# invokermyself/ICP-4DRadar

Measured on AMD Instinct MI355X. Metric: scan-pair registrations/sec (8k-pt clouds, 20 ICP iters) at 1/2/4/8 GPU, higher is better.
Workload: dtype fp32; 1 GPU; C3/C4: 1024 independent pairs per GPU, 8192/8192-pt scans, 20 ICP iterations (fixed) + fitness pass, exact NN (kd-block pruned), PCL numerics (bit-exact float restatement); pairs_per_gpu=1024, points=8192, parallelism=1 GPU

## Files before the change

### icp-4dradar_amd/csrc/icp4r_batch.hpp

```cpp
#pragma once

#include <hip/hip_runtime.h>

#include <vector>

#include "icp4r_host.hpp"
#include "icp4r_internal.hpp"

namespace icp4r_pipe {

struct Plan {
    int q;
    bool packed;
    int splits;
    bool pruned;
    bool lds;
    bool cache;
    int leaf;
    int chunk_sb;
    int chunks;
    bool tile;
    int max_m;
    int tile_run;
    bool solo;
    int64_t blocks;
};

enum PlanOpt : int {
    kOptNnQ, kOptLeaf, kOptChunkSb, kOptNnLds, kOptNnCache, kOptNnTile, kOptTileRun, kOptSolo, kOptXpad,
    kOptPhaseTicks, kOptKd, kOptMortonMwg, kOptPart, kOptSrcOrder, kOptFuseSeed, kOptTileOwn, kOptTileDefer,
    kOptGroups, kOptSearchCuDiv, kOptFuseTest, kOptFuseOrder, kOptSumsTail, kOptWideUpdate, kOptGatherPadded,
    kOptGicpCovBrute, kOptFoldKeys, kOptGicpSpec, kOptGicpGrid, kOptGicpKnnLanes, kOptResUpdate, kOptHeldUpdate,
    kOptFitXform, kOptCounters, kOptStageSel, kOptLazyX, kNumPlanOpts
};
static_assert(kNumPlanOpts <= 64, "icp4r_ctx::plan_set is a 64-bit mask");
extern const char* const kPlanOptNames[kNumPlanOpts];
int opt(const icp4r_ctx* ctx, PlanOpt k, int dflt);

Plan make_plan(const icp4r_ctx* ctx, int npairs, int max_n, int max_m, int nn_mode = ICP4R_NN_AUTO,
               bool allow_lds = true, bool registration = false);
int make_kparams(const icp4r_params* p, icp4r::KParams* kp);
int setup_work(icp4r_ctx* ctx, const Plan& pl, int npairs, int max_n, int max_m, bool corr, hipStream_t st,
               icp4r::WorkArgs& w);
int nn_pass(icp4r_ctx* ctx, const Plan& pl, const icp4r::PairArgs& a, const icp4r::WorkArgs& w, int npairs, int max_n,
            int fitness_pass, int first, hipStream_t st, int ncu = 0, int test_fused = 0, int pass = -1,
            int ordered = 0, int pending = 0);
int next_event(std::vector<icp4r_host::EventPair>& v, size_t& used, icp4r_host::EventPair** out);

}
```

### icp-4dradar_amd/csrc/icp4r_capi.cpp

```cpp
#include <dlfcn.h>
#include <float.h>
#include <hip/hip_runtime.h>
#include <math.h>
#include <stdlib.h>
#include <string.h>

#include <algorithm>
#include <cstdarg>
#include <cstdio>
#include <string>
#include <utility>
#include <vector>

#include "icp4r/icp4r.h"
#include "icp4r_batch.hpp"
#include "icp4r_host.hpp"
#include "icp4r_internal.hpp"

using namespace icp4r;

namespace icp4r_host {

thread_local std::string g_last_error;

int fail(int code, const char* fmt, ...) {
    char buf[512];
    va_list ap;
    va_start(ap, fmt);
    vsnprintf(buf, sizeof(buf), fmt, ap);
    va_end(ap);
    g_last_error = buf;
    return code;
}

int check_cloud(const float* c, int64_t n, int32_t stride, const char* what) {
    if (n < 0) return fail(ICP4R_E_INVALID, "%s: negative point count", what);
    if (n > 0 && !c) return fail(ICP4R_E_INVALID, "%s: NULL cloud with %lld points", what, (long long)n);
    if (stride < 12 || stride % 4) return fail(ICP4R_E_INVALID, "%s: stride %d bytes (need >= 12, multiple of 4)", what, stride);
    return ICP4R_OK;
}

void pack_host(const float* c, int64_t n, int32_t stride_bytes, std::vector<float>& out) {
    out.resize((size_t)(n > 0 ? n : 1) * 4);
    const unsigned char* b = reinterpret_cast<const unsigned char*>(c);
    for (int64_t i = 0; i < n; ++i) {
        const float* p = reinterpret_cast<const float*>(b + (size_t)i * stride_bytes);
        out[4 * (size_t)i + 0] = p[0];
        out[4 * (size_t)i + 1] = p[1];
        out[4 * (size_t)i + 2] = p[2];
        out[4 * (size_t)i + 3] = stride_bytes >= 16 ? p[3] : 0.0f;
    }
}

const RoctxApi& roctx() {
    static const RoctxApi api = [] {
        RoctxApi a;
        void* h = dlopen("librocprofiler-sdk-roctx.so.1", RTLD_NOW | RTLD_LOCAL | RTLD_NOLOAD);
        if (!h) h = dlopen("librocprofiler-sdk-roctx.so.1", RTLD_NOW | RTLD_LOCAL);
        if (h) {
            a.push = reinterpret_cast<int (*)(const char*)>(dlsym(h, "roctxRangePushA"));
            a.pop = reinterpret_cast<int (*)()>(dlsym(h, "roctxRangePop"));
            if (!a.push || !a.pop) a.push = nullptr, a.pop = nullptr;
        }
        return a;
    }();
    return api;
}

}

using icp4r_host::DevBuf;
using icp4r_host::EventPair;
using icp4r_host::check_cloud;
using icp4r_host::fail;
using icp4r_host::pack_host;

namespace icp4r_pipe {

constexpr size_t kCountBytes = (size_t)kCountSlots * kCountStride * sizeof(uint64_t);

constexpr int kNumCounters = 8;
int read_counters(icp4r_ctx* ctx, uint64_t (&out)[kNumCounters]) {
    for (int k = 0; k < kNumCounters; ++k) out[k] = 0;
    HIP_TRY(hipSetDevice(ctx->device));
    HIP_TRY(hipDeviceSynchronize());
    if (!ctx->evals.p) return ICP4R_OK;
    std::vector<uint64_t> v((size_t)kCountSlots * kCountStride);
    HIP_TRY(hipMemcpy(v.data(), ctx->evals.p, kCountBytes, hipMemcpyDeviceToHost));
    for (int s = 0; s < kCountSlots; ++s)
        for (int k = 0; k < kNumCounters; ++k) out[k] += v[(size_t)s * kCountStride + k];
    return ICP4R_OK;
}

const char* const kPlanOptNames[kNumPlanOpts] = {
    "nn_q", "leaf", "chunk_sb", "nn_lds", "nn_cache", "nn_tile", "tile_run", "solo", "xpad",
    "phase_ticks", "kd", "morton_mwg", "part", "src_order", "fuse_seed", "tile_own", "tile_defer",
    "groups", "search_cu_div", "fuse_test", "fuse_order", "sums_tail", "wide_update", "gather_padded",
    "gicp_cov_brute", "fold_keys", "gicp_spec", "gicp_grid", "gicp_knn_lanes", "res_update",
    "held_update", "fit_xform", "counters", "stage_sel", "lazy_x"};

int opt(const icp4r_ctx* ctx, PlanOpt k, int dflt) {
    return (ctx && (ctx->plan_set >> k & 1ull)) ? ctx->plan_val[k] : dflt;
}

Plan make_plan(const icp4r_ctx* ctx, int npairs, int max_n, int max_m, int nn_mode, bool allow_lds,
               bool registration) {
    Plan pl;
    pl.pruned = nn_mode == ICP4R_NN_PRUNED || (nn_mode == ICP4R_NN_AUTO && max_m >= kPrunedMinM);
    pl.packed = false;
    pl.lds = false;
    pl.cache = false;
    pl.splits = 1;
    pl.leaf = 0;
    pl.chunk_sb = 64;
    pl.chunks = 1;
    pl.tile = false;
    pl.tile_run = 64;
    pl.solo = false;
    pl.max_m = max_m;
    const int qcap = opt(ctx, kOptNnQ, pl.pruned ? kDefaultPrunedQ : kDefaultQ);
    pl.q = (qcap == 1 || qcap == 2 || qcap == 4 || qcap == 8 || qcap == 16) ? qcap
                                                                             : (pl.pruned ? kDefaultPrunedQ : kDefaultQ);
    auto qblocks = [&](int q) { return (int64_t)((max_n + kNNWG * q - 1) / (kNNWG * q)); };
    if (pl.pruned) {
        if (pl.q > 4) pl.q = 4;
        const int leaf = opt(ctx, kOptLeaf, kDefaultLeaf);
        pl.leaf = (leaf == 16 || leaf == 32) ? leaf : kDefaultLeaf;
        while (pl.q > 1 && (int64_t)npairs * qblocks(pl.q) * (kNNWG / 64) < 8192) pl.q /= 2;
        pl.blocks = (int64_t)npairs * qblocks(pl.q);
        const int nsb = (((max_m + pl.leaf - 1) / pl.leaf) + kSuper - 1) / kSuper;
        const int64_t waves = pl.blocks * (kNNWG / 64);
        int cs = 64;
        while (cs > 16 && waves * ((nsb + cs - 1) / cs) < 1024) cs /= 2;
        const int cs_env = opt(ctx, kOptChunkSb, 0);
        if (cs_env == 16 || cs_env == 32 || cs_env == 64) cs = cs_env;
        pl.chunk_sb = cs;
        pl.chunks = nsb > 0 ? (nsb + cs - 1) / cs : 1;
        pl.blocks *= pl.chunks;
        const int lds = opt(ctx, kOptNnLds, -1);
        const bool fits = allow_lds && pl.leaf == 16 && max_m <= kLdsMaxTargets && max_n <= kLdsMaxSources;
        pl.lds = fits && (lds == 1 || (lds < 0 && npairs >= kLdsMinPairs));
        if (pl.lds) {
            pl.q = 2;
            pl.blocks = npairs;
            pl.chunks = 1;
            pl.cache = opt(ctx, kOptNnCache, 1) != 0;
        } else {
            pl.tile = pl.leaf == 16 && max_m < (1 << 19) && opt(ctx, kOptNnTile, 1) != 0;
            if (pl.tile) {
                pl.chunks = (max_m + 8191) / 8192;
                const int tr = opt(ctx, kOptTileRun, 0);
                auto parts = [&](int run) { return (int64_t)npairs * ((max_n + 16 * run - 1) / (16 * run)) * pl.chunks; };
                pl.tile_run = 64;
                if (tr == 64 || tr == 32 || tr == 16 || tr == 8)
                    pl.tile_run = tr;
                else
                    while (pl.tile_run > 8 && parts(pl.tile_run) < 256) pl.tile_run /= 2;
                pl.blocks = parts(pl.tile_run);
            }
            const int solo_env = opt(ctx, kOptSolo, -1);
            pl.solo = registration && pl.tile && pl.chunks == 1 && solo_env != 0 &&
                      max_n <= (solo_env == 1 ? kCacheMaxN : kSoloMaxN);
            if (pl.solo) pl.blocks = npairs;
        }
        return pl;
    }
    const int64_t want = 2048;
    while (pl.q > 1 && (int64_t)npairs * qblocks(pl.q) < want) pl.q /= 2;
    while ((int64_t)npairs * qblocks(pl.q) * pl.splits < want && max_m / (pl.splits * 2) >= 256 && pl.splits < 64)
        pl.splits *= 2;
    pl.blocks = (int64_t)npairs * qblocks(pl.q) * pl.splits;
    pl.packed = nn_mode == ICP4R_NN_BRUTE_PACKED && pl.q >= 2;
    return pl;
}

float max_d2_threshold(double max_dist) {
    const double md2 = max_dist * max_dist;
    if (!(md2 < (double)FLT_MAX)) return FLT_MAX;
    float f = (float)md2;
    if ((double)f > md2) f = nextafterf(f, 0.0f);
    return f;
}

int make_kparams(const icp4r_params* p, KParams* kp) {
    icp4r_params d;
    if (!p) {
        icp4r_params_default(&d);
        p = &d;
    }
    if (p->max_iterations < 0) return fail(ICP4R_E_INVALID, "max_iterations must be >= 0");
    if (p->numerics != ICP4R_NUMERICS_PCL && p->numerics != ICP4R_NUMERICS_F64)
        return fail(ICP4R_E_INVALID, "unknown numerics mode %d", p->numerics);
    if (p->nn_mode != ICP4R_NN_AUTO && p->nn_mode != ICP4R_NN_BRUTE && p->nn_mode != ICP4R_NN_BRUTE_PACKED &&
        p->nn_mode != ICP4R_NN_PRUNED)
        return fail(ICP4R_E_INVALID, "unknown nn_mode %d", p->nn_mode);
    if (!(p->huber_delta > 0)) return fail(ICP4R_E_INVALID, "huber_delta must be > 0 (+inf disables)");
    memset(kp, 0, sizeof(*kp));
    kp->conv.max_iterations = p->max_iterations;
    kp->conv.max_similar = p->max_iterations_similar_transforms;
    kp->conv.rot_thr = p->transformation_rotation_epsilon > 0 ? p->transformation_rotation_epsilon
                                                              : 1.0 - p->transformation_epsilon;
    kp->conv.trans_thr = p->transformation_epsilon;
    kp->conv.abs_mse = p->mse_threshold_absolute;
    kp->conv.rel_mse = p->euclidean_fitness_epsilon;
    kp->min_corr = p->min_correspondences;
    kp->numerics = p->numerics;
    kp->compute_fitness = p->compute_fitness;
    kp->max_d2 = max_d2_threshold(p->max_correspondence_distance);
    kp->huber_delta = p->huber_delta;
    kp->fit_max_range = p->fitness_max_range;
    kp->need_mse = (p->mse_threshold_absolute > 0 || p->euclidean_fitness_epsilon > 0) ? 1 : 0;
    if (p->eigen_gebp_mr < 0 || p->eigen_gebp_mr > 64)
        return fail(ICP4R_E_INVALID, "eigen_gebp_mr %d out of range (0: the default 8)", p->eigen_gebp_mr);
    kp->sigma_max_kc = sigma_max_kc(p->eigen_l1_bytes, p->eigen_gebp_mr);
    return ICP4R_OK;
}

int next_event(std::vector<EventPair>& v, size_t& used, EventPair** out) {
    if (used == v.size()) {
        EventPair e;
        HIP_TRY(hipEventCreate(&e.start));
        HIP_TRY(hipEventCreate(&e.stop));
        v.push_back(e);
    }
    *out = &v[used++];
    return ICP4R_OK;
}

int setup_work(icp4r_ctx* ctx, const Plan& pl, int npairs, int max_n, int max_m, bool corr, hipStream_t st,
               WorkArgs& w) {
    const int64_t x_stride = (((max_n > 0 ? max_n : 1) + 3) & ~3) + opt(ctx, kOptXpad, 0);
    const int64_t slots = (int64_t)npairs * x_stride;
    HIP_TRY(ctx->X.ensure((size_t)slots * sizeof(float4)));
    HIP_TRY(ctx->nn_key.ensure((size_t)slots * sizeof(NNKey)));
    HIP_TRY(ctx->state.ensure((size_t)npairs * sizeof(PairState)));
    memset(&w, 0, sizeof(w));
    w.tile_own = opt(ctx, kOptTileOwn, 1) != 0 ? 1 : 0;
    w.X = static_cast<float4*>(ctx->X.p);
    w.nn_key = static_cast<NNKey*>(ctx->nn_key.p);
    w.state = static_cast<PairState*>(ctx->state.p);
    w.x_stride = x_stride;
    w.splits = pl.splits;
    if (!ctx->evals.p) {
        HIP_TRY(ctx->evals.ensure(kCountBytes));
        HIP_TRY(hipMemsetAsync(ctx->evals.p, 0, kCountBytes, st));
    }
    w.evals = (opt(ctx, kOptCounters, 0) != 0 || ctx->kernel_timing) ? static_cast<unsigned long long*>(ctx->evals.p)
                                                                      : nullptr;
    if (opt(ctx, kOptPhaseTicks, 0)) {
        const size_t nt = (size_t)pass_tick_base(npairs) + (size_t)kMaxTickPasses * kPassTickSlots;
        if (ctx->ticks.cap < nt * sizeof(uint64_t)) {
            HIP_TRY(ctx->ticks.ensure(nt * sizeof(uint64_t)));
// ... 90 lines not shown
            w.stage_sel = std::max(0, opt(ctx, kOptStageSel, kDefaultStageSel));
        }
    }
    return ICP4R_OK;
}

int nn_pass(icp4r_ctx* ctx, const Plan& pl, const PairArgs& a, const WorkArgs& w0, int npairs, int max_n,
            int fitness_pass, int first, hipStream_t st, int ncu, int test_fused, int pass, int ordered, int pending) {
    EventPair* ne;
    int r;
    WorkArgs w = w0;
    w.pass_ticks = (w0.ticks && pass >= 0 && pass < kMaxTickPasses)
                       ? w0.ticks + pass_tick_base(npairs) + (int64_t)pass * kPassTickSlots
                       : nullptr;
    const bool kev = ctx->kernel_timing;
    EventPair none;
    none.start = none.stop = nullptr;
    if (kev) {
        if ((r = next_event(ctx->nn_events, ctx->nn_used, &ne))) return r;
    } else {
        ne = &none;
    }
    if (pl.lds) {
        NNLdsEvents ev;
        ev.search_start = ne->start;
        ev.search_stop = ne->stop;
        if (kev && pl.cache && !first && !test_fused) {
            EventPair* te;
            if ((r = next_event(ctx->test_events, ctx->test_used, &te))) return r;
            ev.test_start = te->start;
            ev.test_stop = te->stop;
        }
        HIP_TRY(launch_nn_lds(a, w, npairs, max_n, fitness_pass, first, ncu > 0 ? ncu : ctx->ncu, st, ev, test_fused,
                              ordered, pending));
        return ICP4R_OK;
    }
    if (pl.tile) {
        HIP_TRY(launch_nn_tile(a, w, npairs, max_n, pl.max_m, fitness_pass, first, pl.tile_run, st, ne->start, ne->stop));
        return ICP4R_OK;
    }
    if (kev) HIP_TRY(hipEventRecord(ne->start, st));
    if (pl.pruned) {
        HIP_TRY(launch_nn_pruned(pl.q, pl.chunk_sb, pl.chunks, a, w, npairs, max_n, fitness_pass, first, st));
    } else {
        if (pl.splits > 1) HIP_TRY(hipMemsetAsync(w.nn_key, 0xFF, (size_t)npairs * w.x_stride * sizeof(NNKey), st));
        HIP_TRY(launch_nn(pl.q, pl.packed, a, w, npairs, max_n, fitness_pass, st));
    }
    if (kev) HIP_TRY(hipEventRecord(ne->stop, st));
    return ICP4R_OK;
}

static_assert(sizeof(icp4r_ctx::aux_stream) / sizeof(hipStream_t) == kMaxGroups, "aux streams");

void group_view(const PairArgs& a, const WorkArgs& w, int p0, int g, PairArgs& ag, WorkArgs& wg) {
    ag = a;
    ag.src_off += p0;
    ag.src_n += p0;
    ag.tgt_off += p0;
    ag.tgt_n += p0;
    if (ag.guess) ag.guess += (int64_t)p0 * 16;
    ag.results += p0;
    wg = w;
    const int64_t xs = (int64_t)p0 * w.x_stride;
    wg.X += xs;
    wg.nn_key += xs;
    wg.state += p0;
    if (wg.corr) wg.corr += xs * 2;
    if (wg.tsort) {
        wg.tsort += (int64_t)p0 * w.t_stride;
        wg.tinv += (int64_t)p0 * w.t_stride;
        wg.tbox += (int64_t)p0 * 2 * w.b_stride;
        wg.sbox += (int64_t)p0 * 2 * w.sb_stride;
        wg.sperm += xs;
        if (wg.kdn) wg.kdn += (int64_t)p0 * kKdnStride;
        if (wg.tbb) wg.tbb += (int64_t)p0 * 8;
        if (wg.mo_hist) wg.mo_hist += (int64_t)p0 * w.mo_groups * (1 << 14);
        if (wg.mo_rep) wg.mo_rep += (int64_t)p0 * (1 << 14);
    }
    if (wg.nn_u) {
        wg.nn_u += xs;
        wg.nn_t += xs;
        wg.sq += xs;
        wg.sm += xs;
        wg.need += (int64_t)p0 * w.need_stride;
        wg.miss_cnt += p0;
    }
    if (wg.plist) {
        wg.qv += xs;
        wg.qm += xs;
        wg.plist += (int64_t)p0 * ((w.x_stride + 63) / 64);
        wg.plist_n += 4 * g;
        wg.queue = wg.plist_n + 1;
        wg.owork += p0;
    }
    if (g > 0) wg.ticks = nullptr;
}

int run_pairs(icp4r_ctx* ctx, const PairArgs& a, int npairs, int max_n, int max_m, int max_iterations,
              int nn_mode, hipStream_t st) {
    if (npairs <= 0) return ICP4R_OK;
    const int mn = max_n > 0 ? max_n : 1;
    const bool pcl = a.kp.numerics == kNumericsPCL;
    const Plan pl = make_plan(ctx, npairs, mn, max_m, nn_mode, true, pcl);
    WorkArgs w;
    int rc;
    if ((rc = setup_work(ctx, pl, npairs, max_n, max_m, pcl && !pl.solo, st, w))) return rc;
    w.src_by_tgt = (pl.pruned && pl.lds) ? (opt(ctx, kOptSrcOrder, 1) != 0 ? 1 : 0)
                                         : (pl.pruned && opt(ctx, kOptSrcOrder, 0) != 0 ? 1 : 0);
    w.stage_first = (w.src_by_tgt && (pl.lds || pl.solo) && w.qv && w.qm) ? 1 : 0;
    w.seed_next = (pl.tile && pl.chunks > 1 && pcl && w.corr && opt(ctx, kOptFuseSeed, 1) != 0) ? 1 : 0;
    if (pl.tile && pl.chunks == 1 && !pl.solo && pcl && w.corr && opt(ctx, kOptTileOwn, 1) != 0 &&
        opt(ctx, kOptTileDefer, 1) != 0)
        w.defer_xform = 1;
    EventPair* be;
    if ((rc = next_event(ctx->batch_events, ctx->batch_used, &be))) return rc;
    HIP_TRY(hipEventRecord(be->start, st));
    if (pl.solo) {
        icp4r_host::Range solo_range("icp4r solo registration");
        HIP_TRY(launch_init(a, w, npairs, st));
        HIP_TRY(launch_index(a, w, npairs, st));
        const bool kev = ctx->kernel_timing;
        EventPair* ne = nullptr;
        if (kev) {
            if ((rc = next_event(ctx->nn_events, ctx->nn_used, &ne))) return rc;
            HIP_TRY(hipEventRecord(ne->start, st));
        }
        HIP_TRY(launch_solo(a, w, npairs, max_n, max_iterations > 0 ? max_iterations : 1, st));
        if (kev) HIP_TRY(hipEventRecord(ne->stop, st));
        HIP_TRY(hipEventRecord(be->stop, st));
        return ICP4R_OK;
    }
    int groups = pl.lds ? opt(ctx, kOptGroups, kDefaultGroups) : 1;
    if (groups < 1) groups = 1;
    if (groups > kMaxGroups) groups = kMaxGroups;
    while (groups > 1 && npairs / groups < kLdsMinPairs / 2) --groups;
    PairArgs ag[kMaxGroups];
    WorkArgs wg[kMaxGroups];
    hipStream_t gs[kMaxGroups];
    int gn[kMaxGroups];
    for (int g = 0; g < groups; ++g) {
        const int p0 = (int)((int64_t)npairs * g / groups), p1 = (int)((int64_t)npairs * (g + 1) / groups);
        gn[g] = p1 - p0;
        group_view(a, w, p0, g, ag[g], wg[g]);
        gs[g] = st;
        if (g > 0) {
            if (!ctx->aux_stream[g]) HIP_TRY(hipStreamCreateWithFlags(&ctx->aux_stream[g], hipStreamNonBlocking));
            if (!ctx->fork_ev[g]) HIP_TRY(hipEventCreateWithFlags(&ctx->fork_ev[g], hipEventDisableTiming));
            gs[g] = ctx->aux_stream[g];
        }
    }
    for (int g = 1; g < groups; ++g) HIP_TRY(hipStreamWaitEvent(gs[g], be->start, 0));
    const int cdiv = opt(ctx, kOptSearchCuDiv, groups);
    const int search_cu = cdiv > 1 ? (ctx->ncu + cdiv - 1) / cdiv : 0;
    for (int g = 0; g < groups; ++g) {
        HIP_TRY(launch_init(ag[g], wg[g], gn[g], gs[g]));
        if (pl.pruned) HIP_TRY(launch_index(ag[g], wg[g], gn[g], gs[g]));
    }
    const int iters = max_iterations > 0 ? max_iterations : 1;
    const bool fuse = pl.lds && pl.cache && pcl && opt(ctx, kOptFuseTest, 1) != 0;
    const bool ford = fuse && opt(ctx, kOptFuseOrder, 1) != 0;
    for (int g = 0; g < groups; ++g)
        wg[g].sums_tail = (fuse && a.kp.huber_delta == INFINITY && a.kp.max_d2 >= FLT_MAX && !a.kp.need_mse &&
                           opt(ctx, kOptSumsTail, 0) != 0)
                              ? 1
                              : 0;
    for (int g = 0; g < groups; ++g)
        wg[g].res_update = (fuse && pcl && mn <= kResMaxN && !wg[g].sums_tail && a.kp.huber_delta == INFINITY &&
                             a.kp.max_d2 >= FLT_MAX && opt(ctx, kOptResUpdate, kDefaultResUpdate) != 0)
                                ? 1
                                : 0;
    const bool lazy = fuse && !wg[0].sums_tail && !wg[0].res_update && opt(ctx, kOptLazyX, kDefaultLazyX) != 0;
    for (int g = 0; g < groups; ++g) wg[g].lazy_x = lazy ? 1 : 0;
    auto silent_tail = [&](int it) { return lazy && it >= 0 && it + 1 < iters && ((iters - 2 - it) & 1) != 0; };
    const bool kev = ctx->kernel_timing;
    const bool wide = pcl && !fuse && npairs <= ctx->ncu && opt(ctx, kOptWideUpdate, 1) != 0;
    for (int g = 0; g < groups; ++g)
        wg[g].held_update = (wide && mn <= kHeldMaxN && opt(ctx, kOptHeldUpdate, kDefaultHeldUpdate) != 0) ? 1 : 0;
    if (wide && pl.tile && !pl.lds && w.corr && (pl.chunks > 1 || !w.tile_own) && opt(ctx, kOptFoldKeys, 1) != 0)
        for (int g = 0; g < groups; ++g) wg[g].fold_keys = 1;
    char pass_name[48];
    for (int it = 0; it < iters; ++it) {
        snprintf(pass_name, sizeof(pass_name), "icp4r ICP pass %d", it + 1);
        icp4r_host::Range pass_range(pass_name);
        for (int g = 0; g < groups; ++g) {
            const int ncu_g = search_cu > 0 ? search_cu : ctx->ncu;
            if ((rc = nn_pass(ctx, pl, ag[g], wg[g], gn[g], mn, 0, it == 0, gs[g], search_cu, fuse && it > 0, it,
                              ford && it > 0, silent_tail(it - 1) ? 1 : 0)))
                return rc;
            EventPair* ue = nullptr;
            if (kev) {
                if ((rc = next_event(ctx->upd_events, ctx->upd_used, &ue))) return rc;
                HIP_TRY(hipEventRecord(ue->start, gs[g]));
            }
            HIP_TRY(launch_update(ag[g], wg[g], gn[g], mn, pcl && !pl.pruned, gs[g], fuse && it + 1 < iters,
                                  ford && it + 1 < iters ? ncu_g : 0, wide, silent_tail(it) ? 1 : 0,
                                  silent_tail(it - 1) ? 1 : 0));
            if (kev) HIP_TRY(hipEventRecord(ue->stop, gs[g]));
        }
    }
    icp4r_host::Range fit_range("icp4r fitness pass");
    for (int g = 0; g < groups; ++g) {
        const int ftest = fuse && a.kp.compute_fitness ? 1 : 0;
        wg[g].fit_xform = (a.kp.compute_fitness && pl.tile && !pl.lds && pl.max_m <= kLdsMaxTargets && wg[g].tile_own &&
                           !wg[g].nn_u && !wg[g].seed_next && opt(ctx, kOptFitXform, 1) != 0)
                              ? 1
                              : 0;
        if ((a.kp.compute_fitness || a.aligned) && !wg[g].fit_xform)
            HIP_TRY(launch_fitness_prep(ag[g], wg[g], gn[g], gs[g], ftest));
        if (a.kp.compute_fitness && (rc = nn_pass(ctx, pl, ag[g], wg[g], gn[g], mn, 1, 0, gs[g], search_cu, ftest, iters)))
            return rc;
        HIP_TRY(launch_finish(ag[g], wg[g], gn[g], gs[g]));
    }
    for (int g = 1; g < groups; ++g) {
        HIP_TRY(hipEventRecord(ctx->fork_ev[g], gs[g]));
        HIP_TRY(hipStreamWaitEvent(st, ctx->fork_ev[g], 0));
    }
    HIP_TRY(hipEventRecord(be->stop, st));
    return ICP4R_OK;
}

int nearest_keys(icp4r_ctx* ctx, const float* query, int32_t n, int32_t qstride, const float* tgt, int32_t m,
                 int32_t tstride, const float* T, std::vector<NNKey>& keys) {
    std::vector<float> hq, ht;
    pack_host(query, n, qstride, hq);
    pack_host(tgt, m, tstride, ht);
    hipStream_t st = ctx->stream;
    const int64_t zero64 = 0;
    HIP_TRY(ctx->src.ensure(hq.size() * 4));
    HIP_TRY(ctx->tgt.ensure(ht.size() * 4));
    HIP_TRY(ctx->src_off.ensure(16));
    HIP_TRY(ctx->tgt_off.ensure(16));
    HIP_TRY(ctx->src_n.ensure(16));
    HIP_TRY(ctx->tgt_n.ensure(16));
    HIP_TRY(ctx->guess.ensure(64));
    HIP_TRY(ctx->results.ensure(sizeof(icp4r_result)));
    HIP_TRY(hipMemcpyAsync(ctx->src.p, hq.data(), hq.size() * 4, hipMemcpyHostToDevice, st));
    HIP_TRY(hipMemcpyAsync(ctx->tgt.p, ht.data(), ht.size() * 4, hipMemcpyHostToDevice, st));
    HIP_TRY(hipMemcpyAsync(ctx->src_off.p, &zero64, 8, hipMemcpyHostToDevice, st));
    HIP_TRY(hipMemcpyAsync(ctx->tgt_off.p, &zero64, 8, hipMemcpyHostToDevice, st));
    HIP_TRY(hipMemcpyAsync(ctx->src_n.p, &n, 4, hipMemcpyHostToDevice, st));
    HIP_TRY(hipMemcpyAsync(ctx->tgt_n.p, &m, 4, hipMemcpyHostToDevice, st));
    if (T) HIP_TRY(hipMemcpyAsync(ctx->guess.p, T, 64, hipMemcpyHostToDevice, st));
    PairArgs a;
    memset(&a, 0, sizeof(a));
    a.src = static_cast<const float4*>(ctx->src.p);
    a.tgt = static_cast<const float4*>(ctx->tgt.p);
    a.src_off = static_cast<const int64_t*>(ctx->src_off.p);
    a.tgt_off = static_cast<const int64_t*>(ctx->tgt_off.p);
    a.src_n = static_cast<const int32_t*>(ctx->src_n.p);
    a.tgt_n = static_cast<const int32_t*>(ctx->tgt_n.p);
    a.guess = T ? static_cast<const float*>(ctx->guess.p) : nullptr;
    a.results = static_cast<Result*>(ctx->results.p);
    int rc;
    if ((rc = make_kparams(nullptr, &a.kp))) return rc;
    const Plan pl = make_plan(ctx, 1, n, m, ICP4R_NN_AUTO);
    WorkArgs w;
    if ((rc = setup_work(ctx, pl, 1, n, m, false, st, w))) return rc;
    HIP_TRY(launch_init(a, w, 1, st));
    if (pl.pruned) HIP_TRY(launch_index(a, w, 1, st));
    if ((rc = nn_pass(ctx, pl, a, w, 1, n, 0, 1, st, 0, 0, -1))) return rc;
    PairState ps;
    keys.resize((size_t)n);
    HIP_TRY(hipMemcpyAsync(&ps, w.state, sizeof(ps), hipMemcpyDeviceToHost, st));
    HIP_TRY(hipMemcpyAsync(keys.data(), w.nn_key, (size_t)n * sizeof(NNKey), hipMemcpyDeviceToHost, st));
    HIP_TRY(hipStreamSynchronize(st));
    if (ps.phase == kPhaseInvalid) return fail(ps.status, "non-finite coordinate in the query or target cloud");
    return ICP4R_OK;
}

int events_avg(std::vector<EventPair>& v, size_t used, double* avg_ms) {
    double tot = 0.0;
    for (size_t i = 0; i < used; ++i) {
        HIP_TRY(hipEventSynchronize(v[i].stop));
        float ms = 0.f;
        HIP_TRY(hipEventElapsedTime(&ms, v[i].start, v[i].stop));
        tot += ms;
    }
    *avg_ms = used ? tot / (double)used : 0.0;
    return ICP4R_OK;
}

}

using namespace icp4r_pipe;

extern "C" {

const char* icp4r_version(void) { return "icp4r 0.2.0 (gfx950, HIP)"; }
int icp4r_abi_version(void) { return ICP4R_ABI_VERSION; }
const char* icp4r_last_error(void) { return icp4r_host::g_last_error.c_str(); }

void icp4r_params_default(icp4r_params* p) {
    if (!p) return;
    memset(p, 0, sizeof(*p));
    p->max_iterations = 10;
    p->min_correspondences = 3;
    p->max_correspondence_distance = sqrt(DBL_MAX);
    p->transformation_epsilon = 0.0;
    p->transformation_rotation_epsilon = 0.0;
    p->euclidean_fitness_epsilon = -DBL_MAX;
    p->mse_threshold_absolute = 1e-12;
    p->max_iterations_similar_transforms = 0;
    p->numerics = ICP4R_NUMERICS_PCL;
    p->nn_mode = ICP4R_NN_AUTO;
    p->compute_fitness = 1;
    p->huber_delta = INFINITY;
    p->fitness_max_range = DBL_MAX;
}

int icp4r_device_count(int* count) {
    if (!count) return fail(ICP4R_E_INVALID, "count is NULL");
    HIP_TRY(hipGetDeviceCount(count));
    return ICP4R_OK;
}

int icp4r_create(icp4r_ctx** out, int device) {
    if (!out) return fail(ICP4R_E_INVALID, "out is NULL");
    *out = nullptr;
    if (device == ICP4R_NO_DEVICE) {
        icp4r_ctx* c = new icp4r_ctx();
        c->device = ICP4R_NO_DEVICE;
        *out = c;
        return ICP4R_OK;
    }
    int n = 0;
    HIP_TRY(hipGetDeviceCount(&n));
    if (device < 0 || device >= n) return fail(ICP4R_E_INVALID, "device %d out of range (%d devices)", device, n);
    HIP_TRY(hipSetDevice(device));
    icp4r_ctx* c = new icp4r_ctx();
    c->device = device;
    int ncu = 0;
    if (hipDeviceGetAttribute(&ncu, hipDeviceAttributeMultiprocessorCount, device) == hipSuccess && ncu > 0) c->ncu = ncu;
    hipError_t e = hipStreamCreateWithFlags(&c->stream, hipStreamNonBlocking);
    if (e != hipSuccess) {
        delete c;
        return fail(ICP4R_E_HIP, "hipStreamCreate: %s", hipGetErrorString(e));
    }
    *out = c;
    return ICP4R_OK;
}

int icp4r_destroy(icp4r_ctx* ctx) {
    if (!ctx) return ICP4R_OK;
    for (icp4r_comm* c : ctx->comms) icp4r_host::comm_detach(c);
    if (ctx->device == ICP4R_NO_DEVICE) {
        delete ctx;
        return ICP4R_OK;
    }
    (void)hipSetDevice(ctx->device);
    (void)hipStreamSynchronize(ctx->stream);
    for (int g = 0; g < kMaxGroups; ++g) {
        if (ctx->aux_stream[g]) (void)hipStreamDestroy(ctx->aux_stream[g]);
        if (ctx->fork_ev[g]) (void)hipEventDestroy(ctx->fork_ev[g]);
    }
    for (DevBuf* b : {&ctx->src, &ctx->tgt, &ctx->src_off, &ctx->src_n, &ctx->tgt_off, &ctx->tgt_n, &ctx->guess,
                      &ctx->aligned, &ctx->results, &ctx->T, &ctx->X, &ctx->nn_key,
                      &ctx->state, &ctx->tsort, &ctx->tinv, &ctx->tbox, &ctx->sbox, &ctx->sperm, &ctx->evals, &ctx->corr, &ctx->ticks, &ctx->nn_lu, &ctx->nn_t, &ctx->kdn, &ctx->sq, &ctx->sm, &ctx->qv, &ctx->qm, &ctx->need,
                      &ctx->miss_cnt, &ctx->plist, &ctx->plist_n, &ctx->owork, &ctx->ego_rec, &ctx->ego_off, &ctx->ego_cnt, &ctx->ego_feat,
                      &ctx->ego_pd, &ctx->ego_scores, &ctx->ego_res, &ctx->ego_mask, &ctx->ego_xyzi, &ctx->gicp_gs,
                      &ctx->gicp_cov_src, &ctx->gicp_cov_tgt, &ctx->gicp_mah, &ctx->gicp_active, &ctx->gicp_part, &ctx->gicp_sidx})
        b->release();
    for (auto* v : {&ctx->nn_events, &ctx->test_events, &ctx->upd_events, &ctx->batch_events, &ctx->gicp_events})
// ... 171 lines not shown
    b.tgt_n = static_cast<const int32_t*>(ctx->tgt_n.p);
    b.guess = guess ? static_cast<const float*>(ctx->guess.p) : nullptr;
    b.npairs = npairs;
    b.max_src_n = max_n;
    b.max_tgt_n = max_m;
    int rc = icp4r_align_batch_device(ctx, &b, params, static_cast<icp4r_result*>(ctx->results.p), st);
    if (rc) return rc;
    HIP_TRY(hipMemcpyAsync(results, ctx->results.p, (size_t)npairs * sizeof(icp4r_result), hipMemcpyDeviceToHost, st));
    HIP_TRY(hipStreamSynchronize(st));
    return ICP4R_OK;
}

int icp4r_nearest(icp4r_ctx* ctx, const float* query, int32_t n, int32_t query_stride_bytes, const float* tgt,
                  int32_t m, int32_t tgt_stride_bytes, int32_t* idx_out, float* d2_out) {
    if (!ctx || (n > 0 && (!idx_out || !d2_out))) return fail(ICP4R_E_INVALID, "NULL argument");
    int rc;
    if ((rc = check_cloud(query, n, query_stride_bytes, "query"))) return rc;
    if ((rc = check_cloud(tgt, m, tgt_stride_bytes, "target"))) return rc;
    if (m == 0) return fail(ICP4R_E_EMPTY, "empty target");
    if (n == 0) return ICP4R_OK;
    HIP_TRY(hipSetDevice(ctx->device));
    std::vector<NNKey> keys;
    if ((rc = nearest_keys(ctx, query, n, query_stride_bytes, tgt, m, tgt_stride_bytes, nullptr, keys))) return rc;
    for (int32_t i = 0; i < n; ++i) {
        idx_out[i] = key_idx(keys[i]);
        d2_out[i] = key_d2(keys[i]);
    }
    return ICP4R_OK;
}

int icp4r_fitness(icp4r_ctx* ctx, const float* src, int32_t n, int32_t src_stride_bytes, const float* tgt, int32_t m,
                  int32_t tgt_stride_bytes, const float* T, double max_range, double* fitness) {
    if (!ctx || !T || !fitness) return fail(ICP4R_E_INVALID, "NULL argument");
    int rc;
    if ((rc = check_cloud(src, n, src_stride_bytes, "source"))) return rc;
    if ((rc = check_cloud(tgt, m, tgt_stride_bytes, "target"))) return rc;
    *fitness = DBL_MAX;
    if (m == 0) return fail(ICP4R_E_EMPTY, "empty target");
    if (n == 0) return ICP4R_OK;
    HIP_TRY(hipSetDevice(ctx->device));
    std::vector<NNKey> keys;
    if ((rc = nearest_keys(ctx, src, n, src_stride_bytes, tgt, m, tgt_stride_bytes, T, keys))) return rc;
    double sum = 0.0;
    int nr = 0;
    for (int32_t i = 0; i < n; ++i) {
        const float d2 = key_d2(keys[i]);
        if (d2 <= max_range) {
            sum += d2;
            ++nr;
        }
    }
    *fitness = nr > 0 ? sum / nr : DBL_MAX;
    return ICP4R_OK;
}

int icp4r_synchronize(icp4r_ctx* ctx, void* hip_stream) {
    if (!ctx) return fail(ICP4R_E_INVALID, "ctx is NULL");
    HIP_TRY(hipSetDevice(ctx->device));
    HIP_TRY(hipStreamSynchronize(hip_stream ? static_cast<hipStream_t>(hip_stream) : ctx->stream));
    return ICP4R_OK;
}

int icp4r_kernel_time_ms(icp4r_ctx* ctx, double* avg_ms, int32_t* launches) {
    if (!ctx || !avg_ms) return fail(ICP4R_E_INVALID, "NULL argument");
    HIP_TRY(hipSetDevice(ctx->device));
    int rc = events_avg(ctx->nn_events, ctx->nn_used, avg_ms);
    if (launches) *launches = (int32_t)ctx->nn_used;
    return rc;
}

int icp4r_batch_time_ms(icp4r_ctx* ctx, double* avg_ms, int32_t* calls) {
    if (!ctx || !avg_ms) return fail(ICP4R_E_INVALID, "NULL argument");
    HIP_TRY(hipSetDevice(ctx->device));
    int rc = events_avg(ctx->batch_events, ctx->batch_used, avg_ms);
    if (calls) *calls = (int32_t)ctx->batch_used;
    return rc;
}

int icp4r_stage_time_ms(icp4r_ctx* ctx, int32_t stage, double* avg_ms, int32_t* launches) {
    if (!ctx || !avg_ms) return fail(ICP4R_E_INVALID, "NULL argument");
    std::vector<EventPair>* v;
    size_t used;
    switch (stage) {
        case ICP4R_STAGE_NN: v = &ctx->nn_events; used = ctx->nn_used; break;
        case ICP4R_STAGE_NN_TEST: v = &ctx->test_events; used = ctx->test_used; break;
        case ICP4R_STAGE_UPDATE: v = &ctx->upd_events; used = ctx->upd_used; break;
        case ICP4R_STAGE_BATCH: v = &ctx->batch_events; used = ctx->batch_used; break;
        case ICP4R_STAGE_GICP_COV: v = &ctx->gicp_events; used = ctx->gicp_used; break;
        default: return fail(ICP4R_E_INVALID, "unknown stage %d", stage);
    }
    HIP_TRY(hipSetDevice(ctx->device));
    int rc = events_avg(*v, used, avg_ms);
    if (launches) *launches = (int32_t)used;
    return rc;
}

int icp4r_set_kernel_timing(icp4r_ctx* ctx, int32_t enable) {
    if (!ctx) return fail(ICP4R_E_INVALID, "ctx is NULL");
    ctx->kernel_timing = enable != 0;
    return ICP4R_OK;
}

int icp4r_kernel_time_reset(icp4r_ctx* ctx) {
    if (!ctx) return fail(ICP4R_E_INVALID, "ctx is NULL");
    ctx->nn_used = 0;
    ctx->test_used = 0;
    ctx->upd_used = 0;
    ctx->batch_used = 0;
    ctx->gicp_used = 0;
    if (ctx->evals.p) {
        HIP_TRY(hipSetDevice(ctx->device));
        HIP_TRY(hipDeviceSynchronize());
        HIP_TRY(hipMemset(ctx->evals.p, 0, kCountBytes));
    }
    return ICP4R_OK;
}

namespace {
int plan_opt_index(const char* name) {
    if (!name) return -1;
    for (int k = 0; k < kNumPlanOpts; ++k)
        if (strcmp(name, kPlanOptNames[k]) == 0) return k;
    return -1;
}
}

int icp4r_set_plan_option(icp4r_ctx* ctx, const char* name, int32_t value) {
    if (!ctx) return fail(ICP4R_E_INVALID, "ctx is NULL");
    const int k = plan_opt_index(name);
    if (k < 0) return fail(ICP4R_E_INVALID, "unknown plan option '%s'", name ? name : "(null)");
    if (k == kOptGroups && (value < 1 || value > kMaxGroups))
        return fail(ICP4R_E_INVALID,
                    "plan option groups = %d: 1..%d (a fourth pair group shares a hardware queue with the third, "
                    "and its kernels serialise)",
                    value, kMaxGroups);
    if (k == kOptXpad && (value < 0 || value > 1 << 20)) return fail(ICP4R_E_INVALID, "plan option xpad = %d", value);
    if (k == kOptSearchCuDiv && value < 0) return fail(ICP4R_E_INVALID, "plan option search_cu_div = %d", value);
    ctx->plan_val[k] = value;
    ctx->plan_set |= 1ull << k;
    return ICP4R_OK;
}

int icp4r_get_plan_option(const icp4r_ctx* ctx, const char* name, int32_t* value, int32_t* is_set) {
    if (!ctx || !value) return fail(ICP4R_E_INVALID, "NULL argument");
    const int k = plan_opt_index(name);
    if (k < 0) return fail(ICP4R_E_INVALID, "unknown plan option '%s'", name ? name : "(null)");
    const bool set = (ctx->plan_set >> k) & 1ull;
    *value = set ? ctx->plan_val[k] : INT32_MIN;
    if (!set) {
        static const int32_t dflt[kNumPlanOpts] = {
            0 , kDefaultLeaf, 0 , -1 , 1, 1, 0 ,
            -1 , 0, 0, 3, 1, kDefaultPartSize, -1 , 1, 1, 1, kDefaultGroups,
            0 , 1, 1, 0, 1, 0, 0, 1, kGicpSpec, kGicpGrid,
            0 , kDefaultResUpdate, kDefaultHeldUpdate, 1, 0, kDefaultStageSel, kDefaultLazyX};
        *value = dflt[k];
    }
    if (is_set) *is_set = set ? 1 : 0;
    return ICP4R_OK;
}

int icp4r_reset_plan_options(icp4r_ctx* ctx) {
    if (!ctx) return fail(ICP4R_E_INVALID, "ctx is NULL");
    ctx->plan_set = 0;
    return ICP4R_OK;
}

int icp4r_plan(const icp4r_ctx* ctx, int32_t npairs, int32_t max_src_n, int32_t max_tgt_n, int32_t nn_mode,
               int32_t numerics, icp4r_plan_info* out) {
    if (npairs <= 0 || max_src_n < 0 || max_tgt_n < 0 || !out) return fail(ICP4R_E_INVALID, "bad shape");
    if (nn_mode < ICP4R_NN_AUTO || nn_mode > ICP4R_NN_PRUNED) return fail(ICP4R_E_INVALID, "unknown nn_mode %d", nn_mode);
    if (numerics != ICP4R_NUMERICS_PCL && numerics != ICP4R_NUMERICS_F64)
        return fail(ICP4R_E_INVALID, "unknown numerics mode %d", numerics);
    const bool pcl = numerics == ICP4R_NUMERICS_PCL;
    const Plan pl = make_plan(ctx, npairs, max_src_n > 0 ? max_src_n : 1, max_tgt_n, nn_mode, true, pcl);
    out->pruned = pl.pruned ? 1 : 0;
    out->solo = pl.solo ? 1 : 0;
    const int ncu = ctx ? ctx->ncu : 256;
    const bool fuse = pl.lds && pl.cache && pcl && opt(ctx, kOptFuseTest, 1) != 0;
    out->wide_update = (pcl && !pl.solo && !fuse && npairs <= ncu && opt(ctx, kOptWideUpdate, 1) != 0) ? 1 : 0;
    out->held_update = (out->wide_update && max_src_n <= kHeldMaxN && opt(ctx, kOptHeldUpdate, kDefaultHeldUpdate) != 0) ? 1 : 0;
    out->res_update = (fuse && max_src_n <= kResMaxN && opt(ctx, kOptSumsTail, 0) == 0 && opt(ctx, kOptResUpdate, kDefaultResUpdate) != 0) ? 1 : 0;
    out->q = pl.q;
    out->splits = pl.splits;
    out->leaf = pl.leaf;
    out->lds = pl.lds ? 1 : 0;
    out->cache = pl.cache ? 1 : 0;
    out->nn_blocks = pl.blocks;
    return ICP4R_OK;
}

int icp4r_nn_counters(icp4r_ctx* ctx, uint64_t* evaluations, uint64_t* box_tests) {
    if (!ctx || !evaluations) return fail(ICP4R_E_INVALID, "NULL argument");
    uint64_t v[kNumCounters];
    int rc = read_counters(ctx, v);
    if (rc) return rc;
    *evaluations = v[0];
    if (box_tests) *box_tests = v[1];
    return ICP4R_OK;
}

int icp4r_nn_cache_hits(icp4r_ctx* ctx, uint64_t* hits) {
    if (!ctx || !hits) return fail(ICP4R_E_INVALID, "NULL argument");
    uint64_t v[kNumCounters];
    int rc = read_counters(ctx, v);
    if (rc) return rc;
    *hits = v[2];
    return ICP4R_OK;
}

int icp4r_nn_stats(icp4r_ctx* ctx, icp4r_nn_stats_t* out) {
    if (!ctx || !out) return fail(ICP4R_E_INVALID, "NULL argument");
    uint64_t v[kNumCounters];
    int rc = read_counters(ctx, v);
    if (rc) return rc;
    memset(out, 0, sizeof(*out));
    out->evaluations = v[0];
    out->box_tests = v[1];
    out->cache_hits = v[2];
    out->cache_tested = v[3];
    out->records_written_by_test = v[4];
    out->tested_in_update = v[5];
    out->hits_in_update = v[6];
    out->second_chance_hits = v[7];
    return ICP4R_OK;
}

int icp4r__debug_ticks(icp4r_ctx* ctx, uint64_t* out, int32_t k) {
    if (!ctx || !out || k <= 0 || (size_t)k * sizeof(uint64_t) > ctx->ticks.cap) return fail(ICP4R_E_INVALID, "bad arguments");
    if (!ctx->ticks.p) return fail(ICP4R_E_INVALID, "phase ticks not enabled (plan option phase_ticks = 1)");
    HIP_TRY(hipSetDevice(ctx->device));
    HIP_TRY(hipDeviceSynchronize());
    HIP_TRY(hipMemcpy(out, ctx->ticks.p, (size_t)k * sizeof(uint64_t), hipMemcpyDeviceToHost));
    return ICP4R_OK;
}

int icp4r__test_rot_f32(icp4r_ctx* ctx, const float* sigma, float* R, int32_t k) {
    if (!ctx || !sigma || !R || k <= 0) return fail(ICP4R_E_INVALID, "bad arguments");
    HIP_TRY(hipSetDevice(ctx->device));
    HIP_TRY(ctx->T.ensure((size_t)k * 9 * 4 * 2));
    float* d = static_cast<float*>(ctx->T.p);
    HIP_TRY(hipMemcpyAsync(d, sigma, (size_t)k * 36, hipMemcpyHostToDevice, ctx->stream));
    HIP_TRY(launch_rot_f32(d, d + 9 * (size_t)k, k, ctx->stream));
    HIP_TRY(hipMemcpyAsync(R, d + 9 * (size_t)k, (size_t)k * 36, hipMemcpyDeviceToHost, ctx->stream));
    HIP_TRY(hipStreamSynchronize(ctx->stream));
    return ICP4R_OK;
}

}
```

### icp-4dradar_amd/csrc/icp4r_internal.hpp

```cpp
#pragma once

#include <hip/hip_runtime.h>
#include <stdint.h>

#include "icp4r/icp4r.h"
#include "icp4r/icp4r_ego.h"
#include "icp4r/icp4r_gicp.h"
#include "icp4r_math.hpp"

namespace icp4r {

constexpr int kNNWG = 256;
constexpr int kMaxQ = 16;
constexpr int kDefaultQ = 4;
constexpr int kDefaultPrunedQ = 2;
constexpr int kDefaultLeaf = 16;
constexpr int kMaxGroups = 3;
constexpr int kDefaultGroups = 2;
constexpr int kDefaultStageSel = 32;
constexpr int kDefaultPartSize = 2048;
constexpr int kFoldChunk = 1024;
constexpr int kSuper = 8;
constexpr int kPrunedMinM = 512;
constexpr int kCacheMaxN = 16384;
constexpr int kKdNodes = 2048;
constexpr int kKdnStride = 8 + kKdNodes;
constexpr int kCountSlots = 2048;
constexpr int kCountStride = 16;

constexpr int kNumericsPCL = ICP4R_NUMERICS_PCL;
constexpr int kNumericsF64 = ICP4R_NUMERICS_F64;
constexpr int kStatusEmpty = ICP4R_E_EMPTY;
constexpr int kStatusTooFewCorr = ICP4R_E_TOO_FEW_CORR;
constexpr int kStatusNonFinite = ICP4R_E_NONFINITE;
constexpr int kStatusInvalid = ICP4R_E_INVALID;

constexpr int kPhaseActive = 0;
constexpr int kPhaseConverged = 1;
constexpr int kPhaseFailed = 2;
constexpr int kPhaseInvalid = 3;

using Result = icp4r_result;

struct KParams {
    ConvParams conv;
    int32_t min_corr;
    int32_t numerics;
    int32_t compute_fitness;
    float max_d2;
    double huber_delta;
    double fit_max_range;
    int32_t need_mse;
    int32_t sigma_max_kc;
};

struct PairArgs {
    const float4* src;
    const float4* tgt;
    const int64_t* src_off;
    const int32_t* src_n;
    const int64_t* tgt_off;
    const int32_t* tgt_n;
    const float* guess;
    float4* aligned;
    Result* results;
    KParams kp;
};

struct PairState {
    float T_inc[16];
    float final_T[16];
    double prev_mse;
    int32_t similar;
    int32_t conv_state;
    int32_t iterations;
    int32_t phase;
    int32_t status;
    int32_t ncorr;
    float sum_s[3];
    int32_t sums_ok;
    float T_pend[16];
    int32_t pending;
};

using NNKey = uint64_t;
__host__ __device__ inline float key_d2(NNKey k) {
    union {
        uint32_t u;
        float f;
    } c;
    c.u = (uint32_t)(k >> 32);
    return c.f;
}
__host__ __device__ inline int32_t key_idx(NNKey k) { return (int32_t)(uint32_t)k; }

struct WorkArgs {
    float4* X;
    NNKey* nn_key;
    PairState* state;
    int64_t x_stride;
    int32_t splits;
    int32_t leaf;
    int32_t kd_index;
    int32_t src_by_tgt;
    int32_t stage_first;
    int32_t seed_next;
    float* tbb;
    uint16_t* mo_hist;
    int32_t mo_groups;
    int32_t* mo_rep;
    uint32_t* kdn;
    float4* tsort;
    int32_t* tinv;
    float4* tbox;
    float4* sbox;
    int32_t* sperm;
    int64_t t_stride, b_stride, sb_stride;
    float4* corr;
    float* nn_u;
    int32_t tile_own;
    int32_t defer_xform;
    int32_t sums_tail;
    int32_t fold_keys;
    int32_t res_update;
    int32_t held_update;
    int32_t fit_xform;
    int32_t lazy_x;
    float4* nn_t;
    float4* sq;
    uint2* sm;
    float4* qv;
    uint2* qm;
    uint32_t* need;
    int64_t need_stride;
    int32_t* miss_cnt;
    int32_t* plist;
    int32_t* plist_n;
    int32_t* queue;
    int32_t* owork;
    int32_t part_size;
    int32_t stage_sel;
    unsigned long long* evals;
    uint64_t* ticks;
    uint64_t* pass_ticks;
};
constexpr int kPassTickSlots = 16;
constexpr int kMaxTickPasses = 64;
inline int64_t pass_tick_base(int npairs) { return 32 + 20 * (int64_t)npairs; }

hipError_t launch_init(const PairArgs& a, const WorkArgs& w, int npairs, hipStream_t st);
hipError_t launch_nn(int q, bool packed, const PairArgs& a, const WorkArgs& w, int npairs, int max_n,
                     int fitness_pass, hipStream_t st);
hipError_t launch_index(const PairArgs& a, const WorkArgs& w, int npairs, hipStream_t st);
hipError_t launch_index_cloud(const PairArgs& a, const WorkArgs& w, int npairs, hipStream_t st);
hipError_t launch_nn_pruned(int q, int chunk_sb, int chunks, const PairArgs& a, const WorkArgs& w, int npairs,
                            int max_n, int fitness_pass, int first, hipStream_t st);
hipError_t launch_nn_tile(const PairArgs& a, const WorkArgs& w, int npairs, int max_n, int max_m, int fitness_pass,
                          int first, int qrun, hipStream_t st, hipEvent_t tile_start = nullptr, hipEvent_t tile_stop = nullptr);
struct NNLdsEvents {
    hipEvent_t test_start = nullptr, test_stop = nullptr, search_start = nullptr, search_stop = nullptr;
};
hipError_t launch_nn_lds(const PairArgs& a, const WorkArgs& w, int npairs, int max_n, int fitness_pass, int first,
                         int ncu, hipStream_t st, const NNLdsEvents& ev, int test_fused = 0, int ordered = 0,
                         int pending = 0);
constexpr int kLdsMaxTargets = 8192;
constexpr int kLdsMinPairs = 256;
constexpr int kLdsMaxSources = 1 << 14;
constexpr int kResMaxN = 8192;
constexpr int kDefaultResUpdate = 0;
constexpr int kDefaultLazyX = 1;
constexpr int kHeldMaxN = 10 * 896;
constexpr int kHeldSmallN = 3 * 704;
constexpr int kDefaultHeldUpdate = 1;
constexpr int kSoloMaxN = 1024;
hipError_t launch_update(const PairArgs& a, const WorkArgs& w, int npairs, int max_n, bool need_corr,
                         hipStream_t st, int tail_test = 0,
                         int order_ncu = 0,
                         bool wide = false,
                         int silent = 0,
                         int pending = 0);
hipError_t launch_solo(const PairArgs& a, const WorkArgs& w, int npairs, int max_n, int iters, hipStream_t st);
hipError_t launch_fitness_prep(const PairArgs& a, const WorkArgs& w, int npairs, hipStream_t st, int test = 0);
hipError_t launch_finish(const PairArgs& a, const WorkArgs& w, int npairs, hipStream_t st);
hipError_t launch_rot_f32(const float* sigma, float* R, int k, hipStream_t st);

struct SectorArgs {
    float cx, cy, cz;
    float radius;
    float heading;
};
struct Mat3x4d {
    double R[9];
    double t[3];
};
hipError_t launch_associate(const float4* in, int64_t n, const Mat3x4d& M, float4* out, hipStream_t st);
int64_t sector_blocks(int64_t n);
hipError_t launch_sector(const float4* map, int64_t n, const SectorArgs& a, int32_t* counts, int32_t* offsets,
                         int32_t* total, float4* out, hipStream_t st);

struct EgoArgs {
    const float* rec;
    const int64_t* off;
    const int32_t* cnt;
    int64_t stride;
    float4* feat;
    double4* pd;
    int32_t* scores;
    int32_t max_h;
    int32_t iterations;
    double sigma, dyn;
    uint64_t seed;
    uint8_t* mask;
    icp4r_ego_result* results;
};
hipError_t launch_ego(const EgoArgs& e, int nscans, int max_n, float4* xyzi, hipStream_t st);
hipError_t launch_ego_features(const EgoArgs& e, int nscans, int max_n, float4* xyzi, hipStream_t st);

struct GicpState {
    double R[9], t[3];
    double lambda;
};
constexpr int kGicpSys = 21 + 6 + 1 + 1;
constexpr int kGicpSpec = 2;
constexpr int kGicpMaxSlices = 64;
constexpr int kGicpGrid = 2048;
constexpr int kGicpKnnWaves = 16384;
struct GicpTrial {
    double R[9], t[3];
    double dR[9], dt[3];
    double d[6];
    double lambda;
};
struct GicpCand {
    GicpTrial c[kGicpSpec];
    double lambda0;
    double sys[kGicpSys];
    double R0[9], t0[3];
};
struct GicpArgs {
    GicpState* gs;
    GicpCand* cand;
    double* part_lin;
    double* part_err;
    int32_t* cnt;
    const double* cov_src;
    const double* cov_tgt;
    double* mah;
    int64_t t_stride;
    double max_d2;
    double rot_eps, trans_eps, lm_init;
    int32_t lm_max_iterations, max_iterations;
    int32_t spec;
    int32_t grid;
};
hipError_t launch_gicp_init(const float* guess, GicpState* gs, int npairs, hipStream_t st);
hipError_t launch_gicp_cov(const float4* cloud, const int64_t* off, const int32_t* cnt, int npairs, int max_n,
                           int64_t stride, int k, int reg, double* cov, int lanes, hipStream_t st);
hipError_t launch_gicp_knn_cov(const float4* cloud, const int64_t* off, const int32_t* cnt, const WorkArgs& w,
                               int npairs, int max_n, int64_t stride, int k, int reg, double* cov, int lanes,
                               hipStream_t st);
hipError_t launch_gicp_active(const PairState* st, int npairs, int32_t* out, int64_t* host_out, uint32_t seq,
                              hipStream_t s);
hipError_t launch_gicp_iter(const PairArgs& a, const WorkArgs& w, const GicpArgs& g, int npairs, int max_n, int it,
                            hipStream_t st);

}
```

### icp-4dradar_amd/csrc/icp4r_kernels.hip

```cpp
#include <float.h>
#include <hip/hip_runtime.h>
#include <stdint.h>
#include <stdlib.h>

#include "icp4r_device.hpp"
#include "icp4r_internal.hpp"
#include "icp4r_math.hpp"

namespace icp4r {

template <int Q>
__device__ __forceinline__ void nn_sweep(const float (&x)[Q], const float (&y)[Q], const float (&z)[Q],
                                         const float4* tgt_generic, int j0, int j1, float (&best)[Q],
                                         int (&bi)[Q]) {
    const cv4f_ptr tgt = as_const(tgt_generic);
#pragma unroll
    for (int q = 0; q < Q; ++q) {
        best[q] = INFINITY;
        bi[q] = j0;
    }
    const int last = j1 - 1;
    for (int j = j0; j < j1; j += 4) {
        const v4f c[4] = {tgt[j], tgt[min(j + 1, last)], tgt[min(j + 2, last)], tgt[min(j + 3, last)]};
#pragma unroll
// ... 166 lines not shown
        float4 v[kInitPer];
#pragma unroll
        for (int e = 0; e < kInitPer; ++e) v[e] = src[min(i0 + e * kInitWG + tid, n - 1)];
#pragma unroll
        for (int e = 0; e < kInitPer; ++e) {
            const int i = i0 + e * kInitWG + tid;
            bad |= !(isfinite(v[e].x) && isfinite(v[e].y) && isfinite(v[e].z));
            float4 o = v[e];
            if (!id) xform_pt(Tg, v[e].x, v[e].y, v[e].z, o.x, o.y, o.z);
            big |= fmaxf(fabsf(o.x), fmaxf(fabsf(o.y), fabsf(o.z))) > kBig;
            if (i < nc) X[i] = o;
        }
    }
    if (w.need) {
        uint32_t* gneed = w.need + (int64_t)p * w.need_stride;
        for (int k = tid; k < w.need_stride; k += kInitWG) gneed[k] = 0u;
    }
    if (tid == 0 && w.miss_cnt) w.miss_cnt[p] = 0;
    if (tid < 4 && p == 0 && w.plist_n) w.plist_n[tid] = 0;
    bad = __syncthreads_or(bad);
    big = __syncthreads_or(big);
    if (tid == 0) {
        mat4_identity(st.T_inc);
        st.prev_mse = DBL_MAX;
        st.similar = 0;
        st.conv_state = 0;
        st.iterations = 0;
        st.ncorr = 0;
        st.sums_ok = big ? -1 : 0;
        st.pending = 0;
        const bool too_big = n > w.x_stride || (w.leaf > 0 && m > w.t_stride);
        if (m <= 0 || bad || too_big) {
            mat4_identity(st.final_T);
            st.phase = kPhaseInvalid;
            st.status = too_big ? kStatusInvalid : m <= 0 ? kStatusEmpty : kStatusNonFinite;
        } else {
            for (int k = 0; k < 16; ++k) st.final_T[k] = Tg[k];
            st.phase = kPhaseActive;
            st.status = 0;
        }
    }
}

template <int Q, bool PACKED>
__global__ __launch_bounds__(kNNWG) void nn_kernel(PairArgs a, WorkArgs w, int fitness_pass) {
    const int p = blockIdx.y;
    const int phase = uload(&w.state[p].phase);
    if (fitness_pass ? (phase == kPhaseInvalid) : (phase != kPhaseActive)) return;
    const int n = uload(a.src_n + p), m = uload(a.tgt_n + p);
    const int base = blockIdx.x * (kNNWG * Q);
    if (base >= n) return;
    const int s = blockIdx.z;
    const int j0 = (int)(((int64_t)m * s) / w.splits), j1 = (int)(((int64_t)m * (s + 1)) / w.splits);
    const float4* X = w.X + (int64_t)p * w.x_stride;
    float x[Q], y[Q], z[Q];
#pragma unroll
    for (int q = 0; q < Q; ++q) {
        const int i = base + threadIdx.x + q * kNNWG;
        float4 v = make_float4(0.f, 0.f, 0.f, 0.f);
        if (i < n) v = X[i];
        x[q] = v.x;
        y[q] = v.y;
        z[q] = v.z;
    }
    float best[Q];
    int bi[Q];
    if constexpr (PACKED)
            nn_sweep_packed<Q>(x, y, z, a.tgt + uload(a.tgt_off + p), j0, j1, best, bi);
    else
        nn_sweep<Q>(x, y, z, a.tgt + uload(a.tgt_off + p), j0, j1, best, bi);
    NNKey* key = w.nn_key + (int64_t)p * w.x_stride;
    if (threadIdx.x == 0)
        count_add(w.evals, 0, (unsigned long long)(j1 - j0) * (unsigned long long)min(n - base, kNNWG * Q));
#pragma unroll
    for (int q = 0; q < Q; ++q) {
        const int i = base + threadIdx.x + q * kNNWG;
        if (i < n) {
            const NNKey k = make_key(best[q], (uint32_t)bi[q]);
            if (w.splits > 1)
                atomicMin(reinterpret_cast<unsigned long long*>(key + i), (unsigned long long)k);
            else
                key[i] = k;
        }
    }
}

constexpr int kIdxWG = 512;
constexpr int kIdxWaves = kIdxWG / 64;
constexpr int kCellBins = 1 << 14;
constexpr int kKdMaxN = 8192;
constexpr int kKdPer = kKdMaxN / kIdxWG;

constexpr int kKdBins = 2048;

typedef uint8_t kd_flag_t;
struct KdShared {
    uint16_t L[3][kKdMaxN];
    union {
        uint32_t hist[3][kKdBins];
        struct {
            kd_flag_t left[kKdMaxN + 4];
            uint16_t tpre[3][kIdxWG];
        } p;
        float4 bbox[2 * kKdMaxN / 16];
    } u;
    uint16_t seg_mid[kIdxWG];
    uint8_t seg_ax[kIdxWG];
    alignas(16) uint16_t wsum[3][kIdxWaves];
    float red[kIdxWaves][6];
    float lo[3], sc[3];
};

struct MortonShared {
    uint32_t bins[kCellBins];
    float red[kIdxWaves][6];
    uint32_t wsum[kIdxWaves];
    float lo_s[3], sc_s[3];
};

#ifndef ICP4R_WG_TICKS
#define ICP4R_WG_TICKS 0
#endif

union IndexShared {
    KdShared kd;
    MortonShared mo;
};

__device__ __forceinline__ uint32_t cell_code(float x, float y, float z, const float* lo, const float* sc) {
    const int cx = min(31, max(0, (int)((x - lo[0]) * sc[0])));
    const int cy = min(31, max(0, (int)((y - lo[1]) * sc[1])));
    const int cz = min(15, max(0, (int)((z - lo[2]) * sc[2])));
    uint32_t c = 0;
#pragma unroll
    for (int b = 4; b >= 0; --b) {
        c = (c << 1) | ((cx >> b) & 1);
        c = (c << 1) | ((cy >> b) & 1);
        if (b < 4) c = (c << 1) | ((cz >> b) & 1);
    }
    return c;
}

__device__ __forceinline__ uint32_t ord_key(float f) {
    const uint32_t u = __float_as_uint(f);
    return (u & 0x80000000u) ? ~u : (u | 0x80000000u);
}

__device__ __forceinline__ int kd_split(int S, int leaf) {
    if (S <= leaf) return 0;
    const int unit = S > leaf * kSuper ? leaf * kSuper : leaf;
    return (((S + unit - 1) / unit) >> 1) * unit;
}

template <int KPER, typename Get>
__device__ void kd_order(KdShared& sh, Get pts, int n, int leaf, uint64_t* tk, uint32_t* kdn = nullptr,
                         uint16_t* gk = nullptr) {
    static_assert(KPER % 8 == 0 && KPER <= 16 && KPER * kIdxWG >= kKdMaxN / 2, "list positions per thread");
    const int tid = threadIdx.x, lane = tid & 63, wave = tid >> 6;
    if (tk) tk[0] = __builtin_amdgcn_s_memrealtime();
    float px[kKdPer], py[kKdPer], pz[kKdPer];
#pragma unroll
    for (int k = 0; k < kKdPer; ++k) {
        const float4 v = pts(min(tid + k * kIdxWG, n - 1));
        px[k] = v.x;
        py[k] = v.y;
        pz[k] = v.z;
    }
    float mn[3] = {INFINITY, INFINITY, INFINITY}, mx[3] = {-INFINITY, -INFINITY, -INFINITY};
#pragma unroll
    for (int k = 0; k < kKdPer; ++k) {
        const float4 v = make_float4(px[k], py[k], pz[k], 0.0f);
        mn[0] = fminf(mn[0], v.x); mn[1] = fminf(mn[1], v.y); mn[2] = fminf(mn[2], v.z);
        mx[0] = fmaxf(mx[0], v.x); mx[1] = fmaxf(mx[1], v.y); mx[2] = fmaxf(mx[2], v.z);
    }
#pragma unroll
    for (int k = 0; k < 3; ++k) {
        mn[k] = wave_minf(mn[k]);
        mx[k] = wave_maxf(mx[k]);
    }
    if (lane == 0)
        for (int k = 0; k < 3; ++k) {
            sh.red[wave][k] = mn[k];
            sh.red[wave][3 + k] = mx[k];
        }
    for (int b = tid; b < 3 * kKdBins; b += kIdxWG) (&sh.u.hist[0][0])[b] = 0;
    __syncthreads();
    if (tid < 3) {
        float l = INFINITY, h = -INFINITY;
        for (int v = 0; v < kIdxWaves; ++v) {
            l = fminf(l, sh.red[v][tid]);
            h = fmaxf(h, sh.red[v][3 + tid]);
        }
        sh.lo[tid] = l;
        sh.sc[tid] = h > l ? (float)kKdBins / (h - l) : 0.0f;
        if (kdn) {
            kdn[tid] = __float_as_uint(l);
            kdn[3 + tid] = __float_as_uint(sh.sc[tid]);
        }
    }
    __syncthreads();
    const float lo[3] = {sh.lo[0], sh.lo[1], sh.lo[2]}, sc[3] = {sh.sc[0], sh.sc[1], sh.sc[2]};
    auto bin = [&](float c, int ax) { return min(kKdBins - 1, max(0, (int)((c - lo[ax]) * sc[ax]))); };
#pragma unroll
    for (int k = 0; k < kKdPer; ++k) {
        if (tid + k * kIdxWG >= n) continue;
        const float4 v = make_float4(px[k], py[k], pz[k], 0.0f);
        atomicAdd(&sh.u.hist[0][bin(v.x, 0)], 1u);
        atomicAdd(&sh.u.hist[1][bin(v.y, 1)], 1u);
        atomicAdd(&sh.u.hist[2][bin(v.z, 2)], 1u);
    }
    __syncthreads();
    {
        constexpr int per = 3 * kKdBins / kIdxWG;
        static_assert(3 * kKdBins % kIdxWG == 0, "bins per thread");
        uint32_t* hb = &sh.u.hist[0][0];
        uint32_t loc[per], run = 0;
#pragma unroll
        for (int k = 0; k < per; ++k) {
            const int gb = tid * per + k;
            loc[k] = run;
            run += hb[gb];
        }
        uint32_t incl = run;
        incl = wave_scan_incl(incl);
        if (lane == 63) sh.red[wave][0] = __uint_as_float(incl);
        __syncthreads();
        uint32_t wbase = 0;
        for (int v = 0; v < wave; ++v) wbase += __float_as_uint(sh.red[v][0]);
        const uint32_t tbase = wbase + incl - run;
        __syncthreads();
#pragma unroll
        for (int k = 0; k < per; ++k) {
            const int gb = tid * per + k;
            hb[gb] = tbase + loc[k] - (uint32_t)(gb / kKdBins) * (uint32_t)n;
        }
    }
    __syncthreads();
#pragma unroll
    for (int k = 0; k < kKdPer; ++k) {
        const int i = tid + k * kIdxWG;
        if (i >= n) continue;
        const float4 v = make_float4(px[k], py[k], pz[k], 0.0f);
        const int bx = bin(v.x, 0), by = bin(v.y, 1), bz = bin(v.z, 2);
        if (gk) {
            gk[i] = (uint16_t)bx;
            gk[kKdMaxN + i] = (uint16_t)by;
            gk[2 * kKdMaxN + i] = (uint16_t)bz;
        }
        sh.L[0][atomicAdd(&sh.u.hist[0][bx], 1u)] = (uint16_t)i;
        sh.L[1][atomicAdd(&sh.u.hist[1][by], 1u)] = (uint16_t)i;
        sh.L[2][atomicAdd(&sh.u.hist[2][bz], 1u)] = (uint16_t)i;
    }
    __syncthreads();
    if (tk) tk[1] = __builtin_amdgcn_s_memrealtime();
    const int p0 = tid * KPER;
    int s = 0, e = n, node = 1;
    for (;;) {
        bool any = false;
        if (p0 == s && p0 < n) {
            const int h = kd_split(e - s, leaf);
            uint8_t ax = 3;
            if (h) {
                float ext[3];
                if (gk) {
                    int kf[3], kl[3];
#pragma unroll
                    for (int a = 0; a < 3; ++a) {
                        kf[a] = gk[a * kKdMaxN + sh.L[a][s]];
                        kl[a] = gk[a * kKdMaxN + sh.L[a][e - 1]];
                    }
#pragma unroll
                    for (int a = 0; a < 3; ++a) ext[a] = (float)(kl[a] - kf[a]) / sc[a];
                } else {
                    float4 pf[3], pl[3];
#pragma unroll
                    for (int a = 0; a < 3; ++a) {
                        pf[a] = pts(sh.L[a][s]);
                        pl[a] = pts(sh.L[a][e - 1]);
                    }
                    ext[0] = (float)(bin(pl[0].x, 0) - bin(pf[0].x, 0)) / sc[0];
                    ext[1] = (float)(bin(pl[1].y, 1) - bin(pf[1].y, 1)) / sc[1];
                    ext[2] = (float)(bin(pl[2].z, 2) - bin(pf[2].z, 2)) / sc[2];
                }
                ax = ext[0] >= ext[1] && ext[0] >= ext[2] ? 0 : (ext[1] >= ext[2] ? 1 : 2);
                any = true;
                if (kdn && node < kKdNodes) {
                    uint32_t km;
                    if (gk) {
                        km = gk[ax * kKdMaxN + sh.L[ax][s + h]];
                    } else {
                        const float4 pm = pts(sh.L[ax][s + h]);
                        km = (uint32_t)bin(ax == 0 ? pm.x : (ax == 1 ? pm.y : pm.z), ax);
                    }
                    kdn[8 + node] = 0x80000000u | ((uint32_t)(s + h) << 13) | ((uint32_t)ax << 11) | km;
                }
            }
            sh.seg_mid[tid] = (uint16_t)(s + h);
            sh.seg_ax[tid] = ax;
        }
        if (!__syncthreads_or(any)) {
            if (tk) tk[2] = __builtin_amdgcn_s_memrealtime();
            break;
        }
        int mid = 0, ax = 3;
        if (p0 < n) {
            mid = sh.seg_mid[s / KPER];
            ax = sh.seg_ax[s / KPER];
        }
        uint32_t vp[3][KPER / 2];
        static_assert(KPER % 8 == 0, "whole 16-B reads of the lists");
#pragma unroll
        for (int a = 0; a < 3; ++a)
#pragma unroll
            for (int q8 = 0; q8 < KPER / 8; ++q8) {
                const uint4 r = *reinterpret_cast<const uint4*>(&sh.L[a][p0 + 8 * q8]);
                vp[a][4 * q8] = r.x;
                vp[a][4 * q8 + 1] = r.y;
                vp[a][4 * q8 + 2] = r.z;
                vp[a][4 * q8 + 3] = r.w;
            }
        auto ent = [&](int a, int k) -> uint32_t { return (vp[a][k >> 1] >> (16 * (k & 1))) & 0xffffu; };
        const int nv = min(KPER, n - p0);
        const bool act = nv > 0 && ax < 3;
        if (act) {
            uint32_t va[KPER / 2];
#pragma unroll
            for (int q8 = 0; q8 < KPER / 8; ++q8) {
                const uint4 r = *reinterpret_cast<const uint4*>(&sh.L[ax][p0 + 8 * q8]);
                va[4 * q8] = r.x;
                va[4 * q8 + 1] = r.y;
                va[4 * q8 + 2] = r.z;
                va[4 * q8 + 3] = r.w;
            }
            const uint32_t lf = p0 < mid ? 1u : 0u;
#pragma unroll
            for (int k = 0; k < KPER; ++k) {
                const uint32_t i = (va[k >> 1] >> (16 * (k & 1))) & 0xffffu;
                sh.u.p.left[k < nv ? i : kKdMaxN] = (kd_flag_t)lf;
            }
        }
        __syncthreads();
        uint32_t fb[3] = {0u, 0u, 0u};
        if (act) {
            uint32_t fl[3][KPER];
#pragma unroll
            for (int a = 0; a < 3; ++a)
#pragma unroll
                for (int k = 0; k < KPER; ++k) fl[a][k] = sh.u.p.left[ent(a, k) & (kKdMaxN - 1)];
            const uint32_t vm = nv >= 32 ? ~0u : (1u << nv) - 1u;
#pragma unroll
            for (int a = 0; a < 3; ++a) {
#pragma unroll
                for (int k = 0; k < KPER; ++k) fb[a] |= fl[a][k] << k;
                fb[a] &= vm;
            }
        }
        const int cnt[3] = {__builtin_popcount(fb[0]), __builtin_popcount(fb[1]), __builtin_popcount(fb[2])};
        int incl[3];
#pragma unroll
        for (int a = 0; a < 3; ++a) incl[a] = (int)wave_scan_incl((uint32_t)cnt[a]);
        if (lane == 63)
#pragma unroll
            for (int a = 0; a < 3; ++a) sh.wsum[a][wave] = (uint16_t)incl[a];
#pragma unroll
        for (int a = 0; a < 3; ++a) sh.u.p.tpre[a][tid] = (uint16_t)(incl[a] - cnt[a]);
        __syncthreads();
        const int sw = (s / KPER) >> 6;
        if (act) {
#pragma unroll
            for (int a = 0; a < 3; ++a) {
                if (a == ax) continue;
                static_assert(kIdxWaves % 8 == 0 && kIdxWaves <= 16, "wave totals in whole 16-B reads");
                uint32_t ww[kIdxWaves / 2];
#pragma unroll
                for (int q8 = 0; q8 < kIdxWaves / 8; ++q8) {
                    const uint4 r = *reinterpret_cast<const uint4*>(&sh.wsum[a][8 * q8]);
                    ww[4 * q8] = r.x; ww[4 * q8 + 1] = r.y; ww[4 * q8 + 2] = r.z; ww[4 * q8 + 3] = r.w;
                }
                int bw = 0, bs = 0;
#pragma unroll
                for (int k = 0; k < kIdxWaves; ++k) {
                    const int c = (int)((ww[k >> 1] >> (16 * (k & 1))) & 0xffffu);
                    bw += k < wave ? c : 0;
                    bs += k < sw ? c : 0;
                }
                int ones = (bw + incl[a] - cnt[a]) - (bs + (int)sh.u.p.tpre[a][s / KPER]);
#pragma unroll
                for (int k = 0; k < KPER; ++k) {
                    const int f = (fb[a] >> k) & 1;
                    const int np = f ? s + ones : mid + (p0 + k - s) - ones;
                    ones += f;
                    sh.L[a][np] = (uint16_t)ent(a, k);
                }
            }
            if (p0 < mid) {
                e = mid;
                node = 2 * node;
            } else {
                s = mid;
                node = 2 * node + 1;
            }
        }
        __syncthreads();
    }
}

__device__ void index_boxes(const WorkArgs& w, int p, int n) {
    const int tid = threadIdx.x;
    float4* ts = w.tsort + (int64_t)p * w.t_stride;
    __syncthreads();
    const float4 last = ts[n - 1];
    for (int64_t pos = n + tid; pos < w.t_stride; pos += kIdxWG) ts[pos] = make_float4(INFINITY, INFINITY, INFINITY, last.w);
    const int B = w.leaf;
    const int nb = (n + B - 1) / B;
    float4* tb = w.tbox + (int64_t)p * 2 * w.b_stride;
    constexpr int kHalf = 16;
    for (int b = tid; b < w.b_stride; b += kIdxWG) {
        float4 l = make_float4(INFINITY, INFINITY, INFINITY, 0.f), h = make_float4(-INFINITY, -INFINITY, -INFINITY, 0.f);
        if (b < nb) {
            const int e = min(n, (b + 1) * B) - 1;
            for (int h0 = 0; h0 < B; h0 += kHalf) {
                float vx[kHalf], vy[kHalf], vz[kHalf];
#pragma unroll
                for (int k = 0; k < kHalf; ++k) {
                    const float4 v = ts[min(b * B + h0 + k, e)];
                    vx[k] = v.x;
                    vy[k] = v.y;
                    vz[k] = v.z;
                }
#pragma unroll
                for (int k = 0; k < kHalf; ++k) {
                    l.x = fminf(l.x, vx[k]); l.y = fminf(l.y, vy[k]); l.z = fminf(l.z, vz[k]);
                    h.x = fmaxf(h.x, vx[k]); h.y = fmaxf(h.y, vy[k]); h.z = fmaxf(h.z, vz[k]);
                }
            }
        }
        tb[2 * b] = l;
        tb[2 * b + 1] = h;
    }
    __syncthreads();
    float4* sbx = w.sbox + (int64_t)p * 2 * w.sb_stride;
    for (int s = tid; s < w.sb_stride; s += kIdxWG) {
        float4 l = make_float4(INFINITY, INFINITY, INFINITY, 0.f), h = make_float4(-INFINITY, -INFINITY, -INFINITY, 0.f);
        float4 bb[2 * kSuper];
#pragma unroll
        for (int k = 0; k < 2 * kSuper; ++k) bb[k] = tb[2 * s * kSuper + k];
#pragma unroll
        for (int k = 0; k < kSuper; ++k) {
            const float4 bl = bb[2 * k], bh = bb[2 * k + 1];
            l.x = fminf(l.x, bl.x); l.y = fminf(l.y, bl.y); l.z = fminf(l.z, bl.z);
            h.x = fmaxf(h.x, bh.x); h.y = fmaxf(h.y, bh.y); h.z = fmaxf(h.z, bh.z);
        }
        sbx[2 * s] = l;
        sbx[2 * s + 1] = h;
    }
}

__device__ __forceinline__ bool src_by_tgt_tree(const PairArgs& a, const WorkArgs& w, int p) {
    const int m = a.tgt_n[p];
    return w.src_by_tgt && w.kdn && (w.kd_index & 1) && m > 0 && m <= kKdMaxN && w.t_stride <= kKdMaxN &&
           a.src_n[p] <= kKdMaxN;
}

__device__ __forceinline__ void index_cloud(IndexShared& shu, const PairArgs& a, const WorkArgs& w, int p, bool is_tgt) {
    if (w.state[p].phase == kPhaseInvalid) return;
    const int tid = threadIdx.x, lane = tid & 63, wave = tid >> 6;
    const int n = is_tgt ? a.tgt_n[p] : a.src_n[p];
    if (n <= 0) return;
    const float4* pts = is_tgt ? a.tgt + a.tgt_off[p] : a.src + a.src_off[p];
    if (!is_tgt && src_by_tgt_tree(a, w, p)) return;
    if ((w.kd_index & (is_tgt ? 1 : 2)) && n <= kKdMaxN && (!is_tgt || w.t_stride <= kKdMaxN)) {
#if ICP4R_WG_TICKS
        uint64_t* it = (w.ticks && tid == 0) ? w.ticks + 32 + 12 * (int64_t)gridDim.x + 8 * (int64_t)p + (is_tgt ? 0 : 4) : nullptr;
        if (it) {
            it[0] = __builtin_amdgcn_s_memrealtime();
            it[2] = (uint64_t)(uint32_t)__builtin_amdgcn_s_getreg(4 | (31 << 11)) |
                    ((uint64_t)(uint32_t)__builtin_amdgcn_s_getreg(20 | (31 << 11)) << 32);
        }
#endif
        uint64_t* tk = (w.ticks && p == 0 && is_tgt && tid == 0) ? w.ticks + 12 : nullptr;
        uint32_t* kdn = (is_tgt && w.kdn && w.src_by_tgt) ? w.kdn + (int64_t)p * kKdnStride : nullptr;
        if (kdn)
            for (int k = tid; k < kKdnStride; k += kIdxWG) kdn[k] = 0u;
        uint16_t* gk = (is_tgt && w.qv && (int64_t)w.x_stride * (int64_t)sizeof(float4) >= 3 * kKdMaxN * 2)
                           ? reinterpret_cast<uint16_t*>(w.qv + (int64_t)p * w.x_stride)
                           : nullptr;
        if (n <= kKdMaxN / 2)
            kd_order<8>(shu.kd, [&](int i) { return pts[i]; }, n, is_tgt ? w.leaf : 16, tk, kdn, gk);
        else
            kd_order<16>(shu.kd, [&](int i) { return pts[i]; }, n, is_tgt ? w.leaf : 16, tk, kdn, gk);
        const uint16_t* ord = shu.kd.L[0];
        if (is_tgt) {
            float4* ts = w.tsort + (int64_t)p * w.t_stride;
            int32_t* tinv = w.tinv + (int64_t)p * w.t_stride;
            float4* tb = w.tbox + (int64_t)p * 2 * w.b_stride;
            const float lastw = __uint_as_float((uint32_t)ord[n - 1]);
            const int B = w.leaf;
            uint16_t* inv = shu.kd.L[1];
#pragma unroll
            for (int k = 0; k < kKdPer; ++k) {
                const int pos = tid + k * kIdxWG;
                if (pos < n) inv[ord[pos]] = (uint16_t)pos;
            }
            __syncthreads();
            float px[kKdPer], py[kKdPer], pz[kKdPer];
            uint32_t pos2[kKdPer / 2];
#pragma unroll
            for (int k = 0; k < kKdPer; ++k) {
                const float4 c = pts[min(tid + k * kIdxWG, n - 1)];
                px[k] = c.x;
                py[k] = c.y;
                pz[k] = c.z;
            }
#pragma unroll
            for (int k = 0; k < kKdPer; ++k) {
                const int i = tid + k * kIdxWG;
                const uint32_t ps = i < n ? (uint32_t)inv[i] : 0xffffu;
                if (i < n) tinv[i] = (int32_t)ps;
                if ((k & 1) == 0)
                    pos2[k >> 1] = ps;
                else
                    pos2[k >> 1] |= ps << 16;
            }
            constexpr int kQ = kKdMaxN / 4;
            static_assert(3 * kQ * 4 <= 2 * kKdMaxN * 2, "staging rows in L[1], L[2]");
            float* rx = reinterpret_cast<float*>(&shu.kd.L[1][0]);
            float* ry = rx + kQ;
            float* rz = ry + kQ;
#pragma unroll 1
            for (int q = 0; q < 4; ++q) {
                __syncthreads();
#pragma unroll
                for (int k = 0; k < kKdPer / 2; ++k) asm volatile("" : "+v"(pos2[k]));
#pragma unroll
                for (int k = 0; k < kKdPer; ++k) {
                    const uint32_t r = ((pos2[k >> 1] >> (16 * (k & 1))) & 0xffffu) - (uint32_t)(q * kQ);
                    if (r < (uint32_t)kQ) {
                        rx[r] = px[k];
                        ry[r] = py[k];
                        rz[r] = pz[k];
                    }
                }
                __syncthreads();
#pragma unroll
                for (int kk = 0; kk < kQ / kIdxWG; ++kk) {
                    const int k = q * (kQ / kIdxWG) + kk;
                    const int pos = tid + k * kIdxWG;
                    if (pos < (int)w.t_stride) {
                        float4 v = make_float4(INFINITY, INFINITY, INFINITY, lastw);
                        float4 l = v, h = make_float4(-INFINITY, -INFINITY, -INFINITY, 0.f);
                        if (pos < n) {
                            const int o = pos - q * kQ;
                            v = make_float4(rx[o], ry[o], rz[o], __uint_as_float((uint32_t)ord[pos]));
                            l = v;
                            h = v;
                        }
                        ts[pos] = v;
                        l.x = seg_minf(l.x, B); h.x = seg_maxf(h.x, B);
                        l.y = seg_minf(l.y, B); h.y = seg_maxf(h.y, B);
                        l.z = seg_minf(l.z, B); h.z = seg_maxf(h.z, B);
                        if ((lane & (B - 1)) == 0) {
                            const int b = pos / B;
                            l.w = 0.f;
                            h.w = 0.f;
                            tb[2 * b] = l;
                            tb[2 * b + 1] = h;
                            shu.kd.u.bbox[2 * b] = l;
                            shu.kd.u.bbox[2 * b + 1] = h;
                        }
                    }
                }
            }
            __syncthreads();
            float4* sbx = w.sbox + (int64_t)p * 2 * w.sb_stride;
            for (int sb = tid; sb < w.sb_stride; sb += kIdxWG) {
                float4 l = make_float4(INFINITY, INFINITY, INFINITY, 0.f), h = make_float4(-INFINITY, -INFINITY, -INFINITY, 0.f);
                for (int b = sb * kSuper; b < (sb + 1) * kSuper; ++b) {
                    const float4 bl = shu.kd.u.bbox[2 * b], bh = shu.kd.u.bbox[2 * b + 1];
                    l.x = fminf(l.x, bl.x); l.y = fminf(l.y, bl.y); l.z = fminf(l.z, bl.z);
                    h.x = fmaxf(h.x, bh.x); h.y = fmaxf(h.y, bh.y); h.z = fmaxf(h.z, bh.z);
                }
                sbx[2 * sb] = l;
                sbx[2 * sb + 1] = h;
            }
            if (tk) tk[3] = __builtin_amdgcn_s_memrealtime();
        } else {
            int32_t* sp = w.sperm + (int64_t)p * w.x_stride;
            for (int pos = tid; pos < n; pos += kIdxWG) sp[pos] = ord[pos];
        }
#if ICP4R_WG_TICKS
        __syncthreads();
        if (it) it[1] = __builtin_amdgcn_s_memrealtime();
#endif
        return;
    }
    if (is_tgt && w.mo_hist) return;
    uint32_t* bins = shu.mo.bins;
    float(*red)[6] = shu.mo.red;
    uint32_t* wsum = shu.mo.wsum;
    float* lo_s = shu.mo.lo_s;
    float* sc_s = shu.mo.sc_s;
    constexpr int kMoPer = 16;
    auto sweep = [&](auto&& f) {
        for (int i0 = 0; i0 < n; i0 += kIdxWG * kMoPer) {
            float4 v[kMoPer];
#pragma unroll
            for (int e = 0; e < kMoPer; ++e) v[e] = pts[min(i0 + e * kIdxWG + tid, n - 1)];
#pragma unroll
            for (int e = 0; e < kMoPer; ++e)
                if (i0 + e * kIdxWG + tid < n) f(i0 + e * kIdxWG + tid, v[e]);
        }
    };
    float mn[3] = {INFINITY, INFINITY, INFINITY}, mx[3] = {-INFINITY, -INFINITY, -INFINITY};
    if (is_tgt && w.tbb) {
        for (int k = 0; k < 3; ++k) {
            mn[k] = w.tbb[(int64_t)p * 8 + k];
            mx[k] = w.tbb[(int64_t)p * 8 + 3 + k];
        }
    } else {
        sweep([&](int, const float4& v) {
            mn[0] = fminf(mn[0], v.x); mn[1] = fminf(mn[1], v.y); mn[2] = fminf(mn[2], v.z);
            mx[0] = fmaxf(mx[0], v.x); mx[1] = fmaxf(mx[1], v.y); mx[2] = fmaxf(mx[2], v.z);
        });
    }
#pragma unroll
    for (int k = 0; k < 3; ++k) {
        mn[k] = wave_minf(mn[k]);
        mx[k] = wave_maxf(mx[k]);
    }
    if (lane == 0)
        for (int k = 0; k < 3; ++k) {
            red[wave][k] = mn[k];
            red[wave][3 + k] = mx[k];
        }
    for (int b = tid; b < kCellBins; b += kIdxWG) bins[b] = 0;
    __syncthreads();
    if (tid < 3) {
        float l = INFINITY, h = -INFINITY;
        for (int v = 0; v < kIdxWaves; ++v) {
            l = fminf(l, red[v][tid]);
            h = fmaxf(h, red[v][3 + tid]);
        }
        const float cells = tid == 2 ? 16.0f : 32.0f;
        lo_s[tid] = l;
        sc_s[tid] = h > l ? cells / (h - l) : 0.0f;
    }
    __syncthreads();
    float lo[3] = {lo_s[0], lo_s[1], lo_s[2]}, sc[3] = {sc_s[0], sc_s[1], sc_s[2]};
    sweep([&](int, const float4& v) { atomicAdd(&bins[cell_code(v.x, v.y, v.z, lo, sc)], 1u); });
    __syncthreads();
    constexpr int per = kCellBins / kIdxWG;
    uint32_t loc[per], run = 0;
#pragma unroll
    for (int k = 0; k < per; ++k) {
        loc[k] = run;
        run += bins[tid * per + k];
    }
    uint32_t incl = run;
    incl = wave_scan_incl(incl);
    if (lane == 63) wsum[wave] = incl;
    __syncthreads();
    uint32_t wbase = 0;
    for (int v = 0; v < wave; ++v) wbase += wsum[v];
    const uint32_t tbase = wbase + incl - run;
#pragma unroll
    for (int k = 0; k < per; ++k) bins[tid * per + k] = tbase + loc[k];
    __syncthreads();
    if (is_tgt) {
        float4* ts = w.tsort + (int64_t)p * w.t_stride;
        int32_t* tinv = w.tinv + (int64_t)p * w.t_stride;
        sweep([&](int i, const float4& v) {
            const uint32_t pos = atomicAdd(&bins[cell_code(v.x, v.y, v.z, lo, sc)], 1u);
            ts[pos] = make_float4(v.x, v.y, v.z, __uint_as_float((uint32_t)i));
            tinv[i] = (int32_t)pos;
        });
        index_boxes(w, p, n);
    } else {
        int32_t* sp = w.sperm + (int64_t)p * w.x_stride;
        sweep([&](int i, const float4& v) {
            const uint32_t pos = atomicAdd(&bins[cell_code(v.x, v.y, v.z, lo, sc)], 1u);
            sp[pos] = i;
        });
    }
}


constexpr int kMoChunk = kIdxWG * 16;

__device__ __forceinline__ void mo_quant(const WorkArgs& w, int p, float* lo, float* sc) {
#pragma unroll
    for (int k = 0; k < 3; ++k) {
        const float l = w.tbb[(int64_t)p * 8 + k], h = w.tbb[(int64_t)p * 8 + 3 + k];
        lo[k] = l;
        sc[k] = h > l ? (k == 2 ? 16.0f : 32.0f) / (h - l) : 0.0f;
    }
}

__global__ __launch_bounds__(kIdxWG) void index_mo_hist_kernel(PairArgs a, WorkArgs w) {
    __shared__ uint32_t bins[kCellBins];
    const int g = blockIdx.x, p = blockIdx.y, tid = threadIdx.x;
    const int m = a.tgt_n[p];
    if (w.state[p].phase == kPhaseInvalid || m <= 0 || g * kMoChunk >= m) return;
    const float4* pts = a.tgt + a.tgt_off[p];
    float lo[3], sc[3];
    mo_quant(w, p, lo, sc);
    for (int b = tid; b < kCellBins; b += kIdxWG) bins[b] = 0;
    const int i0 = g * kMoChunk;
    float4 v[kMoChunk / kIdxWG];
#pragma unroll
    for (int e = 0; e < kMoChunk / kIdxWG; ++e) v[e] = pts[min(i0 + e * kIdxWG + tid, m - 1)];
    __syncthreads();
#pragma unroll
    for (int e = 0; e < kMoChunk / kIdxWG; ++e)
        if (i0 + e * kIdxWG + tid < m) atomicAdd(&bins[cell_code(v[e].x, v[e].y, v[e].z, lo, sc)], 1u);
    __syncthreads();
    static_assert(kMoChunk < 65536, "u16 cell counts");
    uint4* row = reinterpret_cast<uint4*>(w.mo_hist + ((int64_t)p * w.mo_groups + g) * kCellBins);
    const uint4* b4 = reinterpret_cast<const uint4*>(bins);
    for (int k = tid; k < kCellBins / 8; k += kIdxWG) {
        const uint4 lo4 = b4[2 * k], hi4 = b4[2 * k + 1];
        row[k] = make_uint4(lo4.x | lo4.y << 16, lo4.z | lo4.w << 16, hi4.x | hi4.y << 16, hi4.z | hi4.w << 16);
    }
}

__global__ __launch_bounds__(kIdxWG) void index_mo_scatter_kernel(PairArgs a, WorkArgs w) {
    __shared__ uint32_t bins[kCellBins];
    __shared__ uint32_t wsum[kIdxWaves];
    const int g = blockIdx.x, p = blockIdx.y, tid = threadIdx.x, lane = tid & 63, wave = tid >> 6;
    const int m = a.tgt_n[p];
    if (w.state[p].phase == kPhaseInvalid || m <= 0 || g * kMoChunk >= m) return;
    const int ng = (m + kMoChunk - 1) / kMoChunk;
    const float4* pts = a.tgt + a.tgt_off[p];
    const int i0 = g * kMoChunk;
    float4 v[kMoChunk / kIdxWG];
#pragma unroll
    for (int e = 0; e < kMoChunk / kIdxWG; ++e) v[e] = pts[min(i0 + e * kIdxWG + tid, m - 1)];
    constexpr int per = kCellBins / kIdxWG;
    constexpr int kMoRows = 3;
    static_assert(per % 8 == 0, "whole 16-B reads of the rows");
    uint32_t tot[per], bef[per];
#pragma unroll
    for (int k = 0; k < per; ++k) tot[k] = bef[k] = 0u;
    const uint16_t* rows = w.mo_hist + (int64_t)p * w.mo_groups * kCellBins + tid * per;
    for (int r0 = 0; r0 < ng; r0 += kMoRows) {
        uint4 c[kMoRows][per / 8];
#pragma unroll
        for (int j = 0; j < kMoRows; ++j) {
            const uint4* rr = reinterpret_cast<const uint4*>(rows + (int64_t)min(r0 + j, ng - 1) * kCellBins);
#pragma unroll
            for (int q = 0; q < per / 8; ++q) c[j][q] = rr[q];
        }
#pragma unroll
        for (int j = 0; j < kMoRows; ++j) {
            const uint32_t use = r0 + j < ng ? 0xffffffffu : 0u, into_bef = r0 + j < g ? 0xffffffffu : 0u;
#pragma unroll
            for (int q = 0; q < per / 8; ++q) {
                const uint32_t u[4] = {c[j][q].x & use, c[j][q].y & use, c[j][q].z & use, c[j][q].w & use};
#pragma unroll
                for (int h = 0; h < 8; ++h) {
                    const uint32_t cnt = (u[h >> 1] >> (16 * (h & 1))) & 0xffffu;
                    tot[8 * q + h] += cnt;
                    bef[8 * q + h] += cnt & into_bef;
                }
            }
        }
    }
    uint32_t run = 0;
#pragma unroll
    for (int k = 0; k < per; ++k) {
        const uint32_t t = tot[k];
        bef[k] += run;
        run += t;
    }
    uint32_t incl = run;
    incl = wave_scan_incl(incl);
    if (lane == 63) wsum[wave] = incl;
    __syncthreads();
    uint32_t tbase = incl - run;
    for (int q = 0; q < wave; ++q) tbase += wsum[q];
    int32_t* rep = w.mo_rep ? w.mo_rep + (int64_t)p * kCellBins : nullptr;
#pragma unroll
    for (int k = 0; k < per; ++k) {
        bins[tid * per + k] = tbase + bef[k];
        if (rep && g == 0 && tot[k] == 0) rep[tid * per + k] = -1;
    }
    __syncthreads();
    float lo[3], sc[3];
    mo_quant(w, p, lo, sc);
    float4* ts = w.tsort + (int64_t)p * w.t_stride;
#pragma unroll
    for (int e = 0; e < kMoChunk / kIdxWG; ++e) {
        const int i = i0 + e * kIdxWG + tid;
        if (i < m) {
            const uint32_t cell = cell_code(v[e].x, v[e].y, v[e].z, lo, sc);
            const uint32_t pos = atomicAdd(&bins[cell], 1u);
            ts[pos] = make_float4(v[e].x, v[e].y, v[e].z, __uint_as_float((uint32_t)i));
            if (rep) rep[cell] = i;
        }
    }
    if (g != ng - 1) return;
    for (int64_t pos = m + tid; pos < w.t_stride; pos += kIdxWG)
        ts[pos] = make_float4(INFINITY, INFINITY, INFINITY, __uint_as_float((uint32_t)(m - 1)));
    const int nb = (m + w.leaf - 1) / w.leaf, nsb = (nb + kSuper - 1) / kSuper;
    const float4 el = make_float4(INFINITY, INFINITY, INFINITY, 0.f), eh = make_float4(-INFINITY, -INFINITY, -INFINITY, 0.f);
    float4* tb = w.tbox + (int64_t)p * 2 * w.b_stride;
    for (int64_t b = nb + tid; b < w.b_stride; b += kIdxWG) {
        tb[2 * b] = el;
        tb[2 * b + 1] = eh;
    }
    float4* sbx = w.sbox + (int64_t)p * 2 * w.sb_stride;
    for (int64_t s = nsb + tid; s < w.sb_stride; s += kIdxWG) {
        sbx[2 * s] = el;
        sbx[2 * s + 1] = eh;
    }
}

constexpr int kSoWG = 512;
constexpr int kNtPosShift = 14;
constexpr int kNtIdxMask = (1 << kNtPosShift) - 1;

struct SoShared {
    uint32_t nodes[kKdNodes];
    uint32_t bins[kKdMaxN / 16];
    uint32_t wsum[kSoWG / 64];
    float qz[6];
    uint32_t sl[kKdMaxN];
};
__device__ void src_order_pair(const PairArgs& a, const WorkArgs& w, int p, SoShared& so) {
    uint32_t* nodes = so.nodes;
    uint32_t* bins = so.bins;
    uint32_t* wsum = so.wsum;
    float* qz = so.qz;
    uint32_t* sl = so.sl;
    if (w.state[p].phase == kPhaseInvalid || !src_by_tgt_tree(a, w, p)) return;
    const int n = a.src_n[p], m = a.tgt_n[p];
    if (n <= 0) return;
    const int tid = threadIdx.x, lane = tid & 63, wave = tid >> 6;
#if ICP4R_WG_TICKS
    uint64_t* it = (w.ticks && tid == 0) ? w.ticks + 32 + 12 * (int64_t)gridDim.x + 8 * (int64_t)p + 4 : nullptr;
    if (it) {
        it[0] = __builtin_amdgcn_s_memrealtime();
        it[2] = (uint64_t)(uint32_t)__builtin_amdgcn_s_getreg(4 | (31 << 11)) |
                ((uint64_t)(uint32_t)__builtin_amdgcn_s_getreg(20 | (31 << 11)) << 32);
    }
#endif
    const int B = w.leaf;
    const int nb = (m + B - 1) / B;
    const uint32_t* kd = w.kdn + (int64_t)p * kKdnStride;
    {
        uint32_t nv[kKdNodes / kSoWG];
#pragma unroll
        for (int k = 0; k < kKdNodes / kSoWG; ++k) nv[k] = kd[8 + tid + k * kSoWG];
#pragma unroll
        for (int k = 0; k < kKdNodes / kSoWG; ++k) nodes[tid + k * kSoWG] = nv[k];
    }
    if (tid < 6) qz[tid] = __uint_as_float(kd[tid]);
    for (int b = tid; b < kKdMaxN / 16; b += kSoWG) bins[b] = 0u;
    __syncthreads();
    const float lo[3] = {qz[0], qz[1], qz[2]}, sc[3] = {qz[3], qz[4], qz[5]};
    const float4* X = w.X + (int64_t)p * w.x_stride;
    constexpr int kSoPer = kKdMaxN / kSoWG, kSoGrp = 8;
    static_assert(kSoPer % kSoGrp == 0 && kSoPer % 2 == 0, "point groups");
    uint32_t lv[kSoPer / 2];
#pragma unroll
    for (int g = 0; g < kSoPer; g += kSoGrp) {
        float4 v[kSoGrp];
#pragma unroll
        for (int e = 0; e < kSoGrp; ++e) v[e] = X[min(tid + (g + e) * kSoWG, n - 1)];
        int key3[kSoGrp][3], node[kSoGrp], sp[kSoGrp];
#pragma unroll
        for (int e = 0; e < kSoGrp; ++e) {
            key3[e][0] = min(kKdBins - 1, max(0, (int)((v[e].x - lo[0]) * sc[0])));
            key3[e][1] = min(kKdBins - 1, max(0, (int)((v[e].y - lo[1]) * sc[1])));
            key3[e][2] = min(kKdBins - 1, max(0, (int)((v[e].z - lo[2]) * sc[2])));
            node[e] = 1;
            sp[e] = 0;
        }
        for (int lvl = 0; lvl < 11; ++lvl) {
            uint32_t nd[kSoGrp];
#pragma unroll
            for (int e = 0; e < kSoGrp; ++e) nd[e] = nodes[min(node[e], kKdNodes - 1)];
#pragma unroll
            for (int e = 0; e < kSoGrp; ++e) {
                const bool inner = node[e] < kKdNodes && (nd[e] >> 31);
                const uint32_t ax = (nd[e] >> 11) & 3u;
                const int k = ax == 0u ? key3[e][0] : (ax == 1u ? key3[e][1] : key3[e][2]);
                const bool right = k >= (int)(nd[e] & 2047u);
                sp[e] = (inner && right) ? (int)((nd[e] >> 13) & 0x3fffu) : sp[e];
                node[e] = inner ? 2 * node[e] + (right ? 1 : 0) : kKdNodes;
            }
        }
#pragma unroll
        for (int e = 0; e < kSoGrp; ++e) {
            const uint32_t leaf = (uint32_t)min(sp[e] / B, nb - 1);
            if (tid + (g + e) * kSoWG < n) atomicAdd(&bins[leaf], 1u);
            if ((e & 1) == 0)
                lv[(g + e) >> 1] = leaf;
            else
                lv[(g + e) >> 1] |= leaf << 16;
        }
    }
    __syncthreads();
#if ICP4R_WG_TICKS
    if (it) it[3] = __builtin_amdgcn_s_memrealtime();
#endif
    {
        constexpr int per = kKdMaxN / 16 / kSoWG;
        uint32_t loc[per], run = 0;
#pragma unroll
        for (int k = 0; k < per; ++k) {
            loc[k] = run;
            run += bins[tid * per + k];
        }
        uint32_t incl = run;
        incl = wave_scan_incl(incl);
        if (lane == 63) wsum[wave] = incl;
        __syncthreads();
        uint32_t base = 0;
        for (int v = 0; v < wave; ++v) base += wsum[v];
        __syncthreads();
#pragma unroll
        for (int k = 0; k < per; ++k) bins[tid * per + k] = base + incl - run + loc[k];
    }
    __syncthreads();
    int32_t* spm = w.sperm + (int64_t)p * w.x_stride;
    NNKey* key = w.nn_key + (int64_t)p * w.x_stride;
    const float4* ts = w.tsort + (int64_t)p * w.t_stride;
    if (w.stage_first) {
        float px[kSoPer], py[kSoPer], pz[kSoPer];
#pragma unroll
        for (int g = 0; g < kSoPer; ++g) {
            const float4 v = X[min(tid + g * kSoWG, n - 1)];
            px[g] = v.x;
            py[g] = v.y;
            pz[g] = v.z;
        }
        uint32_t pos2[kSoPer / 2];
#pragma unroll
        for (int g = 0; g < kSoPer; ++g) {
            const int i = tid + g * kSoWG;
            const uint32_t leaf = (lv[g >> 1] >> (16 * (g & 1))) & 0xffffu;
            const uint32_t ps = i < n ? atomicAdd(&bins[leaf], 1u) : 0xffffu;
            if ((g & 1) == 0)
                pos2[g >> 1] = ps;
            else
                pos2[g >> 1] |= ps << 16;
        }
        constexpr int kQ = kKdMaxN / 4;
        float* rx = reinterpret_cast<float*>(sl);
        float* ry = rx + kQ;
        float* rz = ry + kQ;
        uint32_t* rw = sl + 3 * kQ;
        float4* qv = w.qv + (int64_t)p * w.x_stride;
        uint2* qm = w.qm + (int64_t)p * w.x_stride;
        for (int q0 = 0; q0 < n; q0 += kQ) {
            __syncthreads();
#pragma unroll
            for (int k = 0; k < kSoPer / 2; ++k) asm volatile("" : "+v"(pos2[k]), "+v"(lv[k]));
#pragma unroll
            for (int g = 0; g < kSoPer; ++g) {
                const uint32_t ps = (pos2[g >> 1] >> (16 * (g & 1))) & 0xffffu;
                const uint32_t leaf = (lv[g >> 1] >> (16 * (g & 1))) & 0xffffu;
                const uint32_t r = ps - (uint32_t)q0;
                if (r < (uint32_t)kQ) {
                    rx[r] = px[g];
                    ry[r] = py[g];
                    rz[r] = pz[g];
                    rw[r] = (uint32_t)(tid + g * kSoWG) | (leaf << kNtPosShift);
                }
            }
            __syncthreads();
#pragma unroll
            for (int e = 0; e < kQ / kSoWG; ++e) {
                const int pos = q0 + tid + e * kSoWG;
                if (pos >= n) continue;
                const int o = tid + e * kSoWG;
                const uint32_t e8 = rw[o];
                const uint32_t i = e8 & kNtIdxMask, leaf = e8 >> kNtPosShift;
                spm[pos] = (int32_t)i;
                qv[pos] = make_float4(rx[o], ry[o], rz[o], INFINITY);
                qm[pos] = make_uint2(i | ((uint32_t)pos << kNtPosShift), leaf * (uint32_t)B);
            }
        }
#if ICP4R_WG_TICKS
        __syncthreads();
        if (it) it[1] = __builtin_amdgcn_s_memrealtime();
#endif
        return;
    }
#pragma unroll
    for (int g = 0; g < kSoPer; g += kSoGrp) {
        float sw[kSoGrp];
#pragma unroll
        for (int e = 0; e < kSoGrp; ++e) {
            const uint32_t leaf = (lv[(g + e) >> 1] >> (16 * ((g + e) & 1))) & 0xffffu;
            sw[e] = ts[leaf * B].w;
        }
#pragma unroll
        for (int e = 0; e < kSoGrp; ++e) {
            const int i = tid + (g + e) * kSoWG;
            if (i >= n) continue;
            const uint32_t leaf = (lv[(g + e) >> 1] >> (16 * ((g + e) & 1))) & 0xffffu;
            const uint32_t pos = atomicAdd(&bins[leaf], 1u);
            spm[pos] = i;
            key[i] = make_key(INFINITY, __float_as_uint(sw[e]));
        }
    }
#if ICP4R_WG_TICKS
    __syncthreads();
    if (it) it[1] = __builtin_amdgcn_s_memrealtime();
#endif
}

__global__ __launch_bounds__(kSoWG) void src_order_kernel(PairArgs a, WorkArgs w) {
    __shared__ SoShared so;
    src_order_pair(a, w, xcd_remap(blockIdx.x, gridDim.x), so);
}

static_assert(sizeof(SoShared) <= sizeof(IndexShared) && kSoWG == kIdxWG, "the source order reuses the index build's workgroup");
__global__ __launch_bounds__(kIdxWG, 4) void index_kernel(PairArgs a, WorkArgs w) {
    __shared__ IndexShared shu;
    const int g = xcd_remap(blockIdx.x + gridDim.x * blockIdx.y, gridDim.x * gridDim.y);
    const int p = gridDim.y == 2 ? g >> 1 : g;
    const bool is_tgt = gridDim.y == 2 ? (g & 1) == 0 : true;
    index_cloud(shu, a, w, p, is_tgt);
    if (gridDim.y == 1) {
        __syncthreads();
        src_order_pair(a, w, p, *reinterpret_cast<SoShared*>(&shu));
    }
}

__global__ __launch_bounds__(kIdxWG, 4) void index_cloud_kernel(PairArgs a, WorkArgs w) {
    __shared__ IndexShared shu;
    index_cloud(shu, a, w, xcd_remap(blockIdx.x, gridDim.x), true);
}

__global__ __launch_bounds__(kIdxWG, 4) void index_refine_kernel(PairArgs a, WorkArgs w) {
    __shared__ IndexShared shu;
    const int c = blockIdx.x, p = blockIdx.y;
    if (w.mo_hist && c == (int)gridDim.x - 1) {
        index_cloud(shu, a, w, p, false);
        return;
    }
    if (w.state[p].phase == kPhaseInvalid) return;
    const int m = a.tgt_n[p];
    if (m <= 0 || (m <= kKdMaxN && w.t_stride <= kKdMaxN)) return;
    const int c0 = c * kKdMaxN;
    if (c0 >= m) return;
    const int len = min(kKdMaxN, m - c0);
    const int tid = threadIdx.x, lane = tid & 63;
    float4* ts = w.tsort + (int64_t)p * w.t_stride + c0;
    kd_order<16>(shu.kd, [&](int i) { return ts[i]; }, len, w.leaf, nullptr);
    const uint16_t* ord = shu.kd.L[0];
    float4 v[kKdPer];
#pragma unroll
    for (int k = 0; k < kKdPer; ++k) {
        const int pos = tid + k * kIdxWG;
        v[k] = pos < len ? ts[ord[pos]] : make_float4(INFINITY, INFINITY, INFINITY, 0.f);
    }
    __syncthreads();
    int32_t* tinv = w.tinv + (int64_t)p * w.t_stride;
    float4* tb = w.tbox + (int64_t)p * 2 * w.b_stride;
    const int B = w.leaf;
    const int nbc = (len + B - 1) / B;
#pragma unroll
    for (int k = 0; k < kKdPer; ++k) {
        const int pos = tid + k * kIdxWG;
        const bool real = pos < len;
        if (real) {
            ts[pos] = v[k];
            tinv[__float_as_uint(v[k].w)] = c0 + pos;
        }
        float4 l = real ? v[k] : make_float4(INFINITY, INFINITY, INFINITY, 0.f);
        float4 h = real ? v[k] : make_float4(-INFINITY, -INFINITY, -INFINITY, 0.f);
        l.x = seg_minf(l.x, B); h.x = seg_maxf(h.x, B);
        l.y = seg_minf(l.y, B); h.y = seg_maxf(h.y, B);
        l.z = seg_minf(l.z, B); h.z = seg_maxf(h.z, B);
        if ((lane & (B - 1)) == 0 && pos / B < nbc) {
            const int b = pos / B;
            l.w = 0.f;
            h.w = 0.f;
            tb[2 * (c0 / B + b)] = l;
            tb[2 * (c0 / B + b) + 1] = h;
            shu.kd.u.bbox[2 * b] = l;
            shu.kd.u.bbox[2 * b + 1] = h;
        }
    }
    __syncthreads();
    float4* sbx = w.sbox + (int64_t)p * 2 * w.sb_stride;
    const int nsbc = (nbc + kSuper - 1) / kSuper, sb0 = c0 / (B * kSuper);
    for (int sb = tid; sb < nsbc; sb += kIdxWG) {
        float4 l = make_float4(INFINITY, INFINITY, INFINITY, 0.f), h = make_float4(-INFINITY, -INFINITY, -INFINITY, 0.f);
        for (int b = sb * kSuper; b < min((sb + 1) * kSuper, nbc); ++b) {
            const float4 bl = shu.kd.u.bbox[2 * b], bh = shu.kd.u.bbox[2 * b + 1];
            l.x = fminf(l.x, bl.x); l.y = fminf(l.y, bl.y); l.z = fminf(l.z, bl.z);
            h.x = fmaxf(h.x, bh.x); h.y = fmaxf(h.y, bh.y); h.z = fmaxf(h.z, bh.z);
        }
        sbx[2 * (sb0 + sb)] = l;
        sbx[2 * (sb0 + sb) + 1] = h;
    }
}


__device__ __forceinline__ float rdlane(float v, int l) {
    return __builtin_bit_cast(float, __builtin_amdgcn_readlane(__builtin_bit_cast(int, v), l));
}

template <int Q>
__device__ __forceinline__ bool box_needed(const v4f lo, const v4f hi, const float (&x)[Q], const float (&y)[Q],
                                           const float (&z)[Q], const NNKey (&best)[Q]) {
    bool need = false;
#pragma unroll
    for (int q = 0; q < Q; ++q) {
        const float gx = fmaxf(fmaxf(lo.x - x[q], x[q] - hi.x), 0.0f);
        const float gy = fmaxf(fmaxf(lo.y - y[q], y[q] - hi.y), 0.0f);
        const float gz = fmaxf(fmaxf(lo.z - z[q], z[q] - hi.z), 0.0f);
        const float lb = __builtin_fmaf(gz, gz, __builtin_fmaf(gy, gy, gx * gx));
        need = need || (lb * kLbShrink <= key_d2(best[q]));
    }
    return __any(need);
}

__device__ __forceinline__ bool box_maybe(const v4f lo, const v4f hi, const float (&qlo)[3], const float (&qhi)[3],
                                          float qmax) {
    const float gx = fmaxf(fmaxf(lo.x - qhi[0], qlo[0] - hi.x), 0.0f);
    const float gy = fmaxf(fmaxf(lo.y - qhi[1], qlo[1] - hi.y), 0.0f);
    const float gz = fmaxf(fmaxf(lo.z - qhi[2], qlo[2] - hi.z), 0.0f);
    const float lb = __builtin_fmaf(gz, gz, __builtin_fmaf(gy, gy, gx * gx));
    return lb * kLbShrink <= qmax;
}

template <int Q, int B>
__device__ __forceinline__ void sweep_block(cv4f_ptr blk, const float (&x)[Q], const float (&y)[Q], const float (&z)[Q],
                                            NNKey (&best)[Q]) {
#pragma unroll
    for (int t = 0; t < B; t += 4) {
        const v4f c[4] = {blk[t], blk[t + 1], blk[t + 2], blk[t + 3]};
#pragma unroll
        for (int u = 0; u < 4; ++u) {
            const uint32_t ti = __float_as_uint(c[u].w);
#pragma unroll
            for (int q = 0; q < Q; ++q) {
                const NNKey kn = make_key(l2_simple(x[q], y[q], z[q], c[u].x, c[u].y, c[u].z), ti);
                best[q] = kn < best[q] ? kn : best[q];
            }
        }
    }
}

__global__ __launch_bounds__(256) void nn_seed_kernel(PairArgs a, WorkArgs w, int fitness_pass, int first) {
    const int p = blockIdx.y;
    const int phase = uload(&w.state[p].phase);
    if (fitness_pass ? (phase == kPhaseInvalid) : (phase != kPhaseActive)) return;
    const int n = uload(a.src_n + p), m = uload(a.tgt_n + p);
    const int s = blockIdx.x * 256 + threadIdx.x;
    if (s >= n) return;
    const int o = w.sperm[(int64_t)p * w.x_stride + s];
    const float4 v = w.X[(int64_t)p * w.x_stride + o];
    NNKey* key = w.nn_key + (int64_t)p * w.x_stride;
    const NNKey k0 = key[o];
    const float4* tsg = w.tsort + (int64_t)p * w.t_stride;
    uint32_t j;
    if (first && !seed_key(k0, m)) {
        j = __float_as_uint(tsg[((int64_t)s * m) / n].w);
        if (w.mo_rep) {
            float lo[3], sc[3];
            mo_quant(w, p, lo, sc);
            const int32_t r = w.mo_rep[(int64_t)p * kCellBins + cell_code(v.x, v.y, v.z, lo, sc)];
            if (r >= 0 && r < m) j = (uint32_t)r;
        }
    } else {
        j = min((uint32_t)key_idx(k0), (uint32_t)(m - 1));
    }
    const float4 t = a.tgt[uload(a.tgt_off + p) + j];
    key[o] = make_key(l2_simple(v.x, v.y, v.z, t.x, t.y, t.z), j);
}

template <int Q, int B>
__global__ __launch_bounds__(kNNWG) void nn_pruned_kernel(PairArgs a, WorkArgs w, int fitness_pass, int first, int cs) {
    const int chunks = gridDim.z, c = blockIdx.z;
    const int g = xcd_remap(blockIdx.x + gridDim.x * blockIdx.y, gridDim.x * gridDim.y);
// ... 2297 lines not shown
        if (tid == 0) s.bnd[0] = 0;
        __syncthreads();
        for (int s0 = 0; s0 < S; s0 += kSliceGroup) {
            const int G = min(kSliceGroup, S - s0);
            if (rejected) {
                auto accepted = [&](int i) {
                    float4 r0, r1;
                    rec(i, r0, r1);
                    rec_fix(r0, r1);
                    return !(r1.w > kp.max_d2);
                };
                fold_bounds<WG>(n, kc, S, s0, G, accepted, s.bnd, s.wsum);
            } else {
                if (tid >= 1 && tid <= G) s.bnd[tid] = (s0 + tid >= S) ? n : (s0 + tid) * kc;
                __syncthreads();
            }
            seq([&](int k) { return s.bnd[k]; }, G);
            if (tid == 0) s.bnd[0] = s.bnd[G];
            __syncthreads();
        }
        if (wave == 0 && lane < 9) s.sigmaf[lane] = sig;
        __syncthreads();
        return;
    }

    constexpr int CAP = 9 * ROW;
    auto bufs = [&](int k) -> float* { return &buf[k & 1][0][0]; };
    const bool rejected = cnt < n;
    float sig = 0.0f;
    if (tid == 0) s.bnd[0] = 0;
    __syncthreads();
    if (f.tk) f.tk[18] = __builtin_amdgcn_s_memrealtime();
    for (int s0 = 0; s0 < S; s0 += kSliceGroup) {
        const int G = min(kSliceGroup, S - s0);
        const int R = 9 * G;
        const int FW = (R + 63) / 64;
        const int nF = WG - 64 * FW;
        if (rejected) {
            auto accepted = [&](int i) {
                float4 r0, r1;
                rec(i, r0, r1);
                rec_fix(r0, r1);
                return !(r1.w > kp.max_d2);
            };
            fold_bounds<WG>(n, kc, S, s0, G, accepted, s.bnd, s.wsum);
        }
        auto start = [&](int sl) -> int {
            return rejected ? s.bnd[sl] : min((s0 + sl) * kc, n);
        };
        int maxlen = 0;
        for (int sl = 0; sl < G; ++sl) maxlen = max(maxlen, (s0 + sl + 1 >= S ? n : start(sl + 1)) - start(sl));
        const int stride = (((CAP / R) - 4) & ~7) + 4;
        const int T = stride - 4;
        const float invT = 1.0f / (float)T;
        const int nch = (maxlen + T - 1) / T;
        const int per = (G * T + nF - 1) / nF;
        auto fill = [&](int c) __attribute__((always_inline)) {
            float* b = bufs(c);
            const int me = tid - 64 * FW;
            for (int e0 = 0; e0 < per; e0 += kFillBatch) {
                float4 r[kFillBatch][2];
                int at[kFillBatch];
#pragma unroll
                for (int e = 0; e < kFillBatch; ++e) {
                    const int q = me + (e0 + e) * nF;
                    int sl = (int)((float)q * invT), t = q - sl * T;
                    if (t >= T) { ++sl; t -= T; }
                    if (t < 0) { --sl; t += T; }
                    const int i0 = sl < G ? start(sl) : n;
                    const int i1 = sl < G ? (s0 + sl + 1 >= S ? n : start(sl + 1)) : n;
                    const int i = i0 + c * T + t;
                    at[e] = (e0 + e < per && sl < G && i < i1) ? sl * 9 * stride + t : -1;
                    rec(at[e] >= 0 ? i : 0, r[e][0], r[e][1]);
                }
#pragma unroll
                for (int e = 0; e < kFillBatch; ++e) {
                    if (at[e] < 0) continue;
                    float pr[9];
                    products(r[e][0], r[e][1], pr);
#pragma unroll
                    for (int k = 0; k < 9; ++k) b[at[e] + k * stride] = pr[k];
                }
            }
        };
        float acc = 0.0f;
        const int L = tid;
        const int my_sl = L / 9;
        const int my_len = (wv < FW && L < R) ? ((s0 + my_sl + 1 >= S ? n : start(my_sl + 1)) - start(my_sl)) : 0;
        if (f.tk && s0 == 0) f.tk[0] = __builtin_amdgcn_s_memrealtime();
        if (wv >= FW && nch > 0) fill(0);
        for (int c = 0; c < nch; ++c) {
            __syncthreads();
            if (f.tk && s0 == 0 && c < 2) f.tk[c == 0 ? 1 : 16] = __builtin_amdgcn_s_memrealtime();
            if (wv < FW) {
                const int len = min(T, my_len - c * T);
                if (L < R && len > 0) acc = fold_row(bufs(c) + L * stride, len, acc);
                if (f.tk && s0 == 0 && c < 2) f.tk[15 + 2 * c] = __builtin_amdgcn_s_memrealtime();
            } else if (c + 1 < nch) {
                fill(c + 1);
            }
        }
        __syncthreads();
        if (f.tk && s0 == 0) f.tk[2] = __builtin_amdgcn_s_memrealtime();
        float* cs = bufs(nch);
        if (wv < FW && L < R) cs[L] = acc;
        __syncthreads();
        if (wave == 0 && lane < 9)
            for (int sl = 0; sl < G; ++sl) sig = sig + oon * cs[sl * 9 + lane];
        if (rejected && tid == 0) s.bnd[0] = s.bnd[G];
        __syncthreads();
    }
    if (wave == 0 && lane < 9) s.sigmaf[lane] = sig;
    __syncthreads();
    if (f.tk) f.tk[3] = __builtin_amdgcn_s_memrealtime();
}

template <int WG>
__device__ __forceinline__ void flush_pending(const WorkArgs& w, int p, int n, const float* Tp) {
    float Tq[16];
#pragma unroll
    for (int q = 0; q < 16; ++q) Tq[q] = uload(Tp + q);
    const int64_t xs = (int64_t)p * w.x_stride;
    float4* X = w.X + xs;
    float* uu = w.nn_u + xs;
    constexpr int kPer = 4;
    for (int i0 = 0; i0 < n; i0 += WG * kPer) {
        float4 v[kPer];
        float U[kPer];
#pragma unroll
        for (int e = 0; e < kPer; ++e) {
            const int i = min(i0 + e * WG + (int)threadIdx.x, n - 1);
            v[e] = X[i];
            U[e] = uu[i];
        }
#pragma unroll
        for (int e = 0; e < kPer; ++e) {
            const int i = i0 + e * WG + (int)threadIdx.x;
            if (i >= n) break;
            float4 q = v[e];
            xform_pt(Tq, v[e].x, v[e].y, v[e].z, q.x, q.y, q.z);
            const float2 Lq = move_lu(make_float2(v[e].w, U[e]), v[e].x, v[e].y, v[e].z, q.x, q.y, q.z);
            q.w = Lq.x;
            if (l_flagged(v[e].w)) {
                v[e].w = fabsf(v[e].w);
                X[i] = v[e];
            } else {
                X[i] = q;
                uu[i] = Lq.y;
            }
        }
    }
}

template <bool PEND>
__device__ __forceinline__ int fold_update_pair(const PairArgs& a, const WorkArgs& w, int tail_test, int silent, int p,
                                                FoldShared& sh) {
    PairState& st = w.state[p];
    if (st.phase != kPhaseActive) return 0;
    const int tid = threadIdx.x;
    const int n = a.src_n[p];
    clear_need(w, p, n, tid, kFoldWG);
    const int64_t xs = w.x_stride;
    const KParams& kp = a.kp;
    const float4* C = w.corr ? w.corr + (int64_t)p * xs * 2 : nullptr;
    const float4* Xp = w.X + (int64_t)p * xs;
    const float4* NT = w.nn_t ? w.nn_t + (int64_t)p * xs : nullptr;

    const bool ticks = w.ticks != nullptr && p == 0 && tid == 0;
    if (ticks) w.ticks[0] = __builtin_amdgcn_s_memrealtime();
#if ICP4R_WG_TICKS
    uint64_t* wt = (w.ticks && tid == 0 && st.iterations == 9) ? w.ticks + 32 + 4 * (int64_t)gridDim.x + 8 * (int64_t)p
                                                              : nullptr;
    if (wt) {
        wt[0] = __builtin_amdgcn_s_memrealtime();
        wt[5] = (uint64_t)(uint32_t)__builtin_amdgcn_s_getreg(4 | (31 << 11)) |
                ((uint64_t)(uint32_t)__builtin_amdgcn_s_getreg(20 | (31 << 11)) << 32);
    }
#define WG_TICK(k) \
    if (wt) wt[k] = __builtin_amdgcn_s_memrealtime()
#else
#define WG_TICK(k)
#endif
    const bool lazy = w.lazy_x && w.nn_u && !C && !w.sums_tail;
    const float* Tp = PEND ? st.T_pend : nullptr;
    FoldIn fin{C, Xp, NT, n};
    fin.Tp = Tp;
    const bool sums_tail = w.sums_tail && tail_test && w.nn_u && !C;
    const bool use_sums = sums_tail && uload(&st.sums_ok) == 1;
    fold_pass_a<kFoldWG, kFoldChunkP, kFoldRow>(kp, fin, sh.buf, sh.res, sh.cnt, sh.s, use_sums ? st.sum_s : nullptr);
    if (use_sums && tid == 0) st.sums_ok = 0;
    if (ticks) w.ticks[1] = __builtin_amdgcn_s_memrealtime();
    WG_TICK(1);
    fold_pass_b<kFoldWG, kFoldChunkP, kFoldRow, false>(kp, fin, sh.buf, sh.s);
    if (ticks) w.ticks[2] = __builtin_amdgcn_s_memrealtime();
    WG_TICK(2);
    const bool tail = tail_test && w.nn_u;
    int nwork = 0;
    TailFirst<kTailPer> tf;
    uint32_t* need = reinterpret_cast<uint32_t*>(&sh.buf[0][0][0]);
    if (tail) {
        if (!sums_tail) tail_prefetch<kFoldWG, kTailPer>(w, p, n, tf);
        for (int k = tid; k < ((n + 31) >> 5); k += kFoldWG) need[k] = 0u;
        if (tid == 0) sh.mcount = 0;
    }
    if (tid == 0) solve_pair<kNumericsPCL>(sh.s, st, kp);
    __syncthreads();
    if (ticks) w.ticks[3] = __builtin_amdgcn_s_memrealtime();
    WG_TICK(3);
    if (Tp && !(tail && sh.s.flag == 0)) {
        flush_pending<kFoldWG>(w, p, n, Tp);
        if (tid == 0) st.pending = 0;
    }
    if (sh.s.flag == 1) return 0;
    if (!w.defer_xform) transform_pair<kFoldWG>(w, p, n, sh.s.T_inc, w.seed_next && w.corr);
    if (tail && sh.s.flag == 0) {
        int32_t* pre = reinterpret_cast<int32_t*>(need + kNeedWords);
        float4* lv = reinterpret_cast<float4*>(pre + kNeedWords);
        uint2* lm = reinterpret_cast<uint2*>(lv + (sums_tail ? kFoldRecsSums : kFoldRecs));
        float T[16];
#pragma unroll
        for (int q = 0; q < 16; ++q) T[q] = sh.s.T_inc[q];
#if ICP4R_WG_TICKS
        uint64_t* stamp = wt ? wt + 6 : nullptr;
#else
        uint64_t* stamp = nullptr;
#endif
        if (sums_tail) {
            float* stg = reinterpret_cast<float*>(&sh.buf[0][0][0]) + (2 * 9 * kFoldRow - 2 * kSumBuf);
            nwork = pair_cache_test<kFoldWG, kSumPer, false, true>(
                a, w, p, n, T, need, pre, lv, lm, kFoldRecsSums, &sh.mcount, sh.cnt, false, stamp, nullptr, stg,
                st.sum_s, &st.sums_ok);
        } else {
            const bool quiet = lazy && silent && !Tp;
            nwork = pair_cache_test<kFoldWG, kTailPer, false>(a, w, p, n, T, need, pre, lv, lm, kFoldRecs,
                                                                    &sh.mcount, sh.cnt, false, stamp, &tf, nullptr,
                                                                    nullptr, nullptr, Tp, quiet);
            if (quiet) {
                if (tid < 16) st.T_pend[tid] = sh.s.T_inc[tid];
                if (tid == 0) st.pending = 1;
            } else if (Tp && tid == 0) {
                st.pending = 0;
            }
        }
    }
    if (ticks) w.ticks[4] = __builtin_amdgcn_s_memrealtime();
    WG_TICK(4);
    return nwork;
}

template <bool PEND>
__global__ __launch_bounds__(kFoldWG, 4) void fold_update_kernel(PairArgs a, WorkArgs w, int tail_test, int order_ncu,
                                                                             int silent) {
    __shared__ FoldShared sh;
    __shared__ OrderShared osh;
    __shared__ int32_t last;
    const int p = xcd_remap(blockIdx.x, gridDim.x);
    const int nwork = fold_update_pair<PEND>(a, w, tail_test, silent, p, sh);
    if (order_ncu <= 0) return;
    if (threadIdx.x == 0) {
        __hip_atomic_store(w.owork + p, nwork, __ATOMIC_RELAXED, __HIP_MEMORY_SCOPE_AGENT);
        asm volatile("s_waitcnt vmcnt(0)" ::: "memory");
        const int old = __hip_atomic_fetch_add(w.plist_n + 3, 1, __ATOMIC_RELAXED, __HIP_MEMORY_SCOPE_AGENT);
        last = (old + 1) % (int)gridDim.x == 0 ? 1 : 0;
    }
    __syncthreads();
    if (!last) return;
    order_items<kFoldWG, true>(a, w, (int)gridDim.x, 0, 0, order_ncu, osh);
}

constexpr int kResWG = 256;
constexpr int kResCols = kResMaxN / kResWG;
constexpr int kResRowA = kResWG + kFoldPad;
constexpr int kResStage = 7680;
constexpr int kResRecs = ((kResStage - 2 * kNeedWords) * 4 / 24) & ~15;
static_assert(kResMaxN == kResWG * kResCols && kResCols % 8 == 0 && kResCols <= 32, "columns");
static_assert(2 * 7 * kResRowA <= kResStage, "pass A rows");
struct ResShared {
    float qz[kResMaxN];
    _Float16 L[kResMaxN];
    alignas(16) float stage[kResStage];
    float res[8];
    int32_t cnt[kResWG / 64];
    uint64_t mse_s[kResWG / 64];
    int32_t mse_e[kResWG / 64];
    int32_t mcount;
    SolveShared s;
};

typedef float fcols __attribute__((ext_vector_type(kResCols)));
typedef uint32_t ucols __attribute__((ext_vector_type(kResCols)));
__device__ __forceinline__ int uni(int j) { return __builtin_amdgcn_readfirstlane(j); }

__device__ __forceinline__ _Float16 half_down(float x) {
    _Float16 h = (_Float16)x;
    if ((float)h > x) {
        uint16_t b = __builtin_bit_cast(uint16_t, h);
        b = (b & 0x8000u) ? (uint16_t)(b + 1) : (b == 0 ? (uint16_t)0x8001u : (uint16_t)(b - 1));
        h = __builtin_bit_cast(_Float16, b);
    }
    return h;
}

__device__ __forceinline__ int res_update_pair(const PairArgs& a, const WorkArgs& w, int tail_test, int p,
                                               ResShared& sh) {
    PairState& st = w.state[p];
    if (st.phase != kPhaseActive) return 0;
    const int tid = threadIdx.x, lane = tid & 63, wave = tid >> 6;
    const int n = a.src_n[p];
    clear_need(w, p, n, tid, kResWG);
    const int64_t xs = (int64_t)p * w.x_stride;
    const float4* Xp = w.X + xs;
    const float4* NT = w.nn_t + xs;
    const KParams& kp = a.kp;
    const bool mse = kp.need_mse != 0;
    const int ncol = (n + kResWG - 1) / kResWG;
    float* const buf = sh.stage;
#if ICP4R_WG_TICKS
    uint64_t* wt = (w.ticks && tid == 0 && st.iterations == 9) ? w.ticks + 32 + 4 * (int64_t)gridDim.x + 8 * (int64_t)p
                                                              : nullptr;
#define RES_TICK(k) \
    if (wt) wt[k] = __builtin_amdgcn_s_memrealtime()
    uint64_t* wx = (wt && p == 0) ? w.ticks + 32 + 12 * (int64_t)gridDim.x : nullptr;
#define RES_TICKX(k) \
    if (wx) wx[k] = __builtin_amdgcn_s_memrealtime()
#else
#define RES_TICK(k)
#define RES_TICKX(k)
#endif
    RES_TICK(0);

    fcols px, py, pz, qx, qy;
    constexpr int kLB = 4;
    float4 lv_[kLB], lt_[kLB];
    auto issue = [&](int b) __attribute__((always_inline)) {
#pragma unroll
        for (int e = 0; e < kLB; ++e) {
            const int j = uni(b * kLB + e), i = min(tid + kResWG * j, n - 1);
            if (j < ncol) {
                lv_[e] = Xp[i];
                lt_[e] = NT[i];
            }
        }
    };
    auto extract = [&](int b) __attribute__((always_inline)) {
#pragma unroll
        for (int e = 0; e < kLB; ++e) {
            const int j = uni(b * kLB + e), i = tid + kResWG * j;
            if (j < ncol) {
                px[j] = lv_[e].x;
                py[j] = lv_[e].y;
                pz[j] = lv_[e].z;
                qx[j] = lt_[e].x;
                qy[j] = lt_[e].y;
                sh.qz[i] = lt_[e].z;
                sh.L[i] = half_down(lv_[e].w);
            }
        }
    };
    issue(0);
    extract(0);
    if (ncol > kLB) issue(1);
    RES_TICK(7);

    int cnt = 0;
    uint32_t amask = 0;
    uint64_t ms_s = 0;
    int ms_e = INT_MAX;
    auto stage_col = [&](int j) __attribute__((always_inline)) {
        j = uni(j);
        const int i = tid + kResWG * j;
        if (i >= n) return;
        float* b = buf + (j & 1) * 7 * kResRowA + tid;
        const float z = sh.qz[i];
        const float d2 = l2_simple(px[j], py[j], pz[j], qx[j], qy[j], z);
        const bool ok = !(d2 > kp.max_d2);
        b[0] = ok ? px[j] : -0.0f;
        b[kResRowA] = ok ? py[j] : -0.0f;
        b[2 * kResRowA] = ok ? pz[j] : -0.0f;
        b[3 * kResRowA] = ok ? qx[j] : -0.0f;
        b[4 * kResRowA] = ok ? qy[j] : -0.0f;
        b[5 * kResRowA] = ok ? z : -0.0f;
        b[6 * kResRowA] = ok ? 1.0f : 0.0f;
        cnt += ok ? 1 : 0;
        amask |= ok ? 1u << j : 0u;
        if (mse) lane_exact_add(ok ? (double)d2 : 0.0, ms_s, ms_e);
    };
    float acc = (lane < 6) ? -0.0f : 0.0f;
    if (ncol > 0) stage_col(0);
    for (int K = 0; K < ncol; ++K) {
        __syncthreads();
        if (wave == 0 && lane < 7) {
            fold_prio(true);
            acc = fold_row(buf + ((K & 1) * 7 + lane) * kResRowA, min(kResWG, n - K * kResWG), acc);
            fold_prio(false);
        }
        RES_TICKX(K);
        if ((K + 1) % kLB == 0 && K + 1 < ncol) {
            extract((K + 1) / kLB);
            if (K + 1 + kLB < ncol) issue((K + 1) / kLB + 1);
        }
        if (K + 1 < ncol) stage_col(K + 1);
    }
#pragma unroll
    for (int off = 32; off > 0; off >>= 1) cnt += __shfl_xor(cnt, off, 64);
    if (mse) wave_exact_total(ms_s, ms_e);
    if (lane == 0) {
        sh.cnt[wave] = cnt;
        sh.mse_s[wave] = ms_s;
        sh.mse_e[wave] = ms_e;
    }
    if (wave == 0 && lane < 7) sh.res[lane] = acc;
    __syncthreads();
    if (tid == 0) {
        int total = 0;
        for (int k = 0; k < kResWG / 64; ++k) total += sh.cnt[k];
        sh.s.mom[0] = (double)total;
        const float one_over_n = 1.0f / sh.res[6];
        sh.s.one_over_n = one_over_n;
        for (int k = 0; k < 6; ++k) sh.s.mean[k] = sh.res[k] * one_over_n;
        double msum = 0.0;
// ... 1025 lines not shown
        int flag = 0;
        __syncthreads();
        tick(0);
        for (int it = 0; it < iters && flag == 0; ++it) {
            const int nlist = it > 0 ? solo_cache_test<false>(a, w, p, n, T, sh, tk)
                              : (w.stage_first && src_by_tgt_tree(a, w, p)) ? n : solo_first_list(a, w, p, n, m);
            tick(1);
            search(nlist, false);
            tick(2);
            const FoldIn fin{nullptr, w.X + xs0, w.nn_t + xs0, n};
            fold_pass_a<kSoloWG, kSoloChunk, kSoloRow>(kp, fin, SOLO_F(sh).buf, SOLO_F(sh).res, SOLO_F(sh).cnt, SOLO_F(sh).sv);
            tick(3);
            fold_pass_b<kSoloWG, kSoloChunk, kSoloRow, false>(kp, fin, SOLO_F(sh).buf, SOLO_F(sh).sv);
            tick(4);
            if (tid == 0) solve_pair<kNumericsPCL>(SOLO_F(sh).sv, st, kp);
            __syncthreads();
            tick(5);
            if (tk) tk[9] += 1;
            flag = SOLO_F(sh).sv.flag;
#pragma unroll
            for (int q = 0; q < 16; ++q) T[q] = SOLO_F(sh).sv.T_inc[q];
        }
        if (kp.compute_fitness || a.aligned) {
            __syncthreads();
#pragma unroll
            for (int q = 0; q < 16; ++q) T[q] = st.final_T[q];
            if (kp.compute_fitness) {
                const int nlist = solo_cache_test<true>(a, w, p, n, T, sh);
                tick(6);
                search(nlist, true);
                tick(7);
                if (a.aligned) {
                    __syncthreads();
                    const float4* src = a.src + a.src_off[p];
                    const float4* X = w.X + xs0;
                    for (int i = tid; i < n; i += kSoloWG) {
                        float4 v = X[i];
                        v.w = src[i].w;
                        a.aligned[a.src_off[p] + i] = v;
                    }
                }
            } else {
                const float4* src = a.src + a.src_off[p];
                for (int i = tid; i < n; i += kSoloWG) {
                    const float4 s = src[i];
                    float4 o = s;
                    xform_pt(T, s.x, s.y, s.z, o.x, o.y, o.z);
                    a.aligned[a.src_off[p] + i] = o;
                }
            }
        }
    }
    const bool have = valid && kp.compute_fitness && n > 0;
    double fsum = 0.0;
    int fcnt = 0;
    if (have) {
        const NNKey* key = w.nn_key + xs0;
        const int nch = (n + kSoloFitChunk - 1) / kSoloFitChunk;
        auto fill = [&](int c) {
            const int base = c * kSoloFitChunk, len = min(kSoloFitChunk, n - base);
            for (int o = tid - 64; o < len; o += kSoloWG - 64) {
                const float d2 = key_d2(key[base + o]);
                const bool in = (double)d2 <= kp.fit_max_range;
                SOLO_FIT(sh)[c & 1][o] = in ? (double)d2 : 0.0;
                fcnt += in ? 1 : 0;
            }
        };
        if (wave >= 1) fill(0);
        for (int c = 0; c < nch; ++c) {
            __syncthreads();
            if (wave == 0) {
                if (lane == 0) fsum = fold_seq_d(SOLO_FIT(sh)[c & 1], min(kSoloFitChunk, n - c * kSoloFitChunk), fsum);
            } else if (c + 1 < nch) {
                fill(c + 1);
            }
        }
#pragma unroll
        for (int off = 32; off > 0; off >>= 1) fcnt += __shfl_xor(fcnt, off, 64);
        if (lane == 0) sh.wtot[wave] = fcnt;
        __syncthreads();
        fcnt = 0;
        for (int k = 0; k < kLdsWaves; ++k) fcnt += sh.wtot[k];
    }
    tick(8);
    if (tid == 0) {
        Result r;
        for (int k = 0; k < 16; ++k) r.T[k] = st.final_T[k];
        r.fitness = (have && fcnt > 0) ? fsum / fcnt : DBL_MAX;
        r.iterations = st.iterations;
        r.converged = st.phase == kPhaseConverged ? 1 : 0;
        r.status = st.status;
        r.convergence_state = st.conv_state;
        r.n_correspondences = st.ncorr;
        r.reserved = 0;
        a.results[p] = r;
    }
    if (lane == 0) {
        count_add(w.evals, 0, rs.evals);
        count_add(w.evals, 1, rs.tests);
    }
}

__global__ void rot_f32_kernel(const float* sigma, float* R, int k) {
    const int i = blockIdx.x * 64 + threadIdx.x;
    if (i >= k) return;
    float sg[9], Ri[9];
#pragma unroll
    for (int e = 0; e < 9; ++e) sg[e] = sigma[9 * i + e];
    umeyama_rotation_f32_reg(sg, Ri);
#pragma unroll
    for (int e = 0; e < 9; ++e) R[9 * i + e] = Ri[e];
}

hipError_t launch_rot_f32(const float* sigma, float* R, int k, hipStream_t st) {
    hipLaunchKernelGGL(rot_f32_kernel, dim3((k + 63) / 64), dim3(64), 0, st, sigma, R, k);
    return hipGetLastError();
}

hipError_t launch_init(const PairArgs& a, const WorkArgs& w, int npairs, hipStream_t st) {
    if (npairs < 64)
        hipLaunchKernelGGL(init_kernel<1024>, dim3(npairs), dim3(1024), 0, st, a, w);
    else
        hipLaunchKernelGGL(init_kernel<256>, dim3(npairs), dim3(256), 0, st, a, w);
    return hipGetLastError();
}

hipError_t launch_nn(int q, bool packed, const PairArgs& a, const WorkArgs& w, int npairs, int max_n,
                     int fitness_pass, hipStream_t st) {
    const int per_block = kNNWG * q;
    const dim3 grid((max_n + per_block - 1) / per_block, npairs, w.splits), block(kNNWG);
#define ICP4R_NN_CASE(QQ, PP) hipLaunchKernelGGL((nn_kernel<QQ, PP>), grid, block, 0, st, a, w, fitness_pass)
    if (packed && q >= 2) {
        switch (q) {
            case 2: ICP4R_NN_CASE(2, true); break;
            case 4: ICP4R_NN_CASE(4, true); break;
            case 8: ICP4R_NN_CASE(8, true); break;
            case 16: ICP4R_NN_CASE(16, true); break;
            default: return hipErrorInvalidValue;
        }
    } else {
        switch (q) {
            case 1: ICP4R_NN_CASE(1, false); break;
            case 2: ICP4R_NN_CASE(2, false); break;
            case 4: ICP4R_NN_CASE(4, false); break;
            case 8: ICP4R_NN_CASE(8, false); break;
            case 16: ICP4R_NN_CASE(16, false); break;
            default: return hipErrorInvalidValue;
        }
    }
#undef ICP4R_NN_CASE
    return hipGetLastError();
}

hipError_t launch_index(const PairArgs& a, const WorkArgs& w, int npairs, hipStream_t st) {
    const bool tgt_only = w.src_by_tgt && w.kdn && (w.kd_index & 1) && w.t_stride <= kKdMaxN && w.x_stride <= kKdMaxN;
    const unsigned nch = (unsigned)((w.t_stride + kKdMaxN - 1) / kKdMaxN);
    if (w.mo_hist) {
        if (!(w.tbb && (w.kd_index & 1) && w.t_stride > kKdMaxN && (w.leaf == 16 || w.leaf == 32) &&
              (int64_t)w.mo_groups * kMoChunk >= w.t_stride))
            return hipErrorInvalidValue;
        hipLaunchKernelGGL(index_mo_hist_kernel, dim3(w.mo_groups, npairs), dim3(kIdxWG), 0, st, a, w);
        hipLaunchKernelGGL(index_mo_scatter_kernel, dim3(w.mo_groups, npairs), dim3(kIdxWG), 0, st, a, w);
        hipLaunchKernelGGL(index_refine_kernel, dim3(nch + 1, npairs), dim3(kIdxWG), 0, st, a, w);
        return hipGetLastError();
    }
    hipLaunchKernelGGL(index_kernel, dim3(npairs, tgt_only ? 1 : 2), dim3(kIdxWG), 0, st, a, w);
    if (w.src_by_tgt && w.kdn && !tgt_only)
        hipLaunchKernelGGL(src_order_kernel, dim3(npairs), dim3(kSoWG), 0, st, a, w);
    if ((w.kd_index & 1) && w.t_stride > kKdMaxN && (w.leaf == 16 || w.leaf == 32))
        hipLaunchKernelGGL(index_refine_kernel, dim3(nch, npairs), dim3(kIdxWG), 0, st, a, w);
    return hipGetLastError();
}

hipError_t launch_index_cloud(const PairArgs& a, const WorkArgs& w, int npairs, hipStream_t st) {
    if (w.mo_hist || (w.src_by_tgt && w.kdn)) return hipErrorInvalidValue;
    hipLaunchKernelGGL(index_cloud_kernel, dim3(npairs), dim3(kIdxWG), 0, st, a, w);
    if ((w.kd_index & 1) && w.t_stride > kKdMaxN && (w.leaf == 16 || w.leaf == 32)) {
        const unsigned nch = (unsigned)((w.t_stride + kKdMaxN - 1) / kKdMaxN);
        hipLaunchKernelGGL(index_refine_kernel, dim3(nch, npairs), dim3(kIdxWG), 0, st, a, w);
    }
    return hipGetLastError();
}

hipError_t launch_nn_lds(const PairArgs& a, const WorkArgs& w, int npairs, int max_n, int fitness_pass, int first,
                         int ncu, hipStream_t st, const NNLdsEvents& ev, int test_fused, int ordered, int pending) {
    if (w.leaf != kLdsLeaf || w.t_stride > kLdsTargets || npairs <= 0 || max_n > (1 << kNtPosShift))
        return hipErrorInvalidValue;
    const bool cache = w.nn_u != nullptr;
    if (cache && (max_n > kCacheMaxN || !w.sq || !w.qv || !w.need || !w.miss_cnt || !w.nn_t || !w.defer_xform))
        return hipErrorInvalidValue;
    if (!w.plist || !w.plist_n || !w.queue || !w.qv || !w.qm) return hipErrorInvalidValue;
    hipError_t e;
    if (cache && !first && !test_fused) {
        const int chunks = (max_n + kTestWG * kTestPer - 1) / (kTestWG * kTestPer);
        if (ev.test_start && (e = hipEventRecord(ev.test_start, st)) != hipSuccess) return e;
        hipLaunchKernelGGL(nn_cache_test_kernel, dim3(chunks, npairs), dim3(kTestWG), 0, st, a, w, fitness_pass);
        if (ev.test_stop && (e = hipEventRecord(ev.test_stop, st)) != hipSuccess) return e;
    }
    if (ordered && (first || !cache || fitness_pass || !test_fused)) return hipErrorInvalidValue;
    if (pending && (first || !cache || fitness_pass || !test_fused || !w.lazy_x)) return hipErrorInvalidValue;
    if (!ordered)
        hipLaunchKernelGGL(nn_order_kernel, dim3(1), dim3(kOrderWG), 0, st, a, w, npairs, fitness_pass,
                           (first || !cache) ? 1 : 0, ncu);
    const int grid = npairs < ncu ? npairs : ncu;
    if (ev.search_start && (e = hipEventRecord(ev.search_start, st)) != hipSuccess) return e;
    if (cache)
        hipLaunchKernelGGL((nn_lds_kernel<true>), dim3(grid), dim3(kLdsWG), 0, st, a, w, fitness_pass, first,
                           test_fused && !first ? 1 : 0, pending);
    else
        hipLaunchKernelGGL((nn_lds_kernel<false>), dim3(grid), dim3(kLdsWG), 0, st, a, w, fitness_pass, first, 0, 0);
    if (ev.search_stop && (e = hipEventRecord(ev.search_stop, st)) != hipSuccess) return e;
    return hipGetLastError();
}

hipError_t launch_nn_tile(const PairArgs& a, const WorkArgs& w, int npairs, int max_n, int max_m, int fitness_pass,
                          int first, int qrun, hipStream_t st, hipEvent_t tile_start, hipEvent_t tile_stop) {
    if (w.leaf != kLdsLeaf || !w.tsort || !w.sperm || max_m >= kTileMaxM || npairs <= 0 || max_n <= 0 ||
        (qrun != 64 && qrun != 32 && qrun != 16 && qrun != 8))
        return hipErrorInvalidValue;
    hipError_t e;
    const int qpart = kLdsWaves * qrun;
    const dim3 grid((max_m + kLdsTargets - 1) / kLdsTargets, (max_n + qpart - 1) / qpart, npairs);
    const bool own = grid.x == 1 && w.tile_own != 0;
    if (!own && (first || !w.seed_next))
        hipLaunchKernelGGL(nn_seed_kernel, dim3((max_n + 255) / 256, npairs), dim3(256), 0, st, a, w, fitness_pass,
                           first);
    if (tile_start && (e = hipEventRecord(tile_start, st)) != hipSuccess) return e;
    hipLaunchKernelGGL(nn_tile_kernel, grid, dim3(kLdsWG), 0, st, a, w, fitness_pass, own ? first : -1, qrun);
    if (tile_stop && (e = hipEventRecord(tile_stop, st)) != hipSuccess) return e;
    if (!own && w.corr != nullptr && !fitness_pass && !w.fold_keys)
        hipLaunchKernelGGL(corr_kernel, dim3((max_n + 255) / 256, npairs), dim3(256), 0, st, a, w);
    return hipGetLastError();
}

hipError_t launch_nn_pruned(int q, int chunk_sb, int chunks, const PairArgs& a, const WorkArgs& w, int npairs,
                            int max_n, int fitness_pass, int first, hipStream_t st) {
    const int per_block = kNNWG * q;
    const dim3 grid((max_n + per_block - 1) / per_block, npairs, chunks), block(kNNWG);
    if (chunk_sb < 1 || chunk_sb > 64 || chunks < 1) return hipErrorInvalidValue;
    if (chunks > 1)
        hipLaunchKernelGGL(nn_seed_kernel, dim3((max_n + 255) / 256, npairs), dim3(256), 0, st, a, w, fitness_pass, first);
#define ICP4R_PR_CASE(QQ, BB) \
    hipLaunchKernelGGL((nn_pruned_kernel<QQ, BB>), grid, block, 0, st, a, w, fitness_pass, first, chunk_sb)
    if (w.leaf == 16) {
        switch (q) {
            case 1: ICP4R_PR_CASE(1, 16); break;
            case 2: ICP4R_PR_CASE(2, 16); break;
            case 4: ICP4R_PR_CASE(4, 16); break;
            default: return hipErrorInvalidValue;
        }
    } else if (w.leaf == 32) {
        switch (q) {
            case 1: ICP4R_PR_CASE(1, 32); break;
            case 2: ICP4R_PR_CASE(2, 32); break;
            case 4: ICP4R_PR_CASE(4, 32); break;
            default: return hipErrorInvalidValue;
        }
    } else {
        return hipErrorInvalidValue;
    }
#undef ICP4R_PR_CASE
    if (chunks > 1 && w.corr != nullptr && !fitness_pass)
        hipLaunchKernelGGL(corr_kernel, dim3((max_n + 255) / 256, npairs), dim3(256), 0, st, a, w);
    return hipGetLastError();
}

hipError_t launch_update(const PairArgs& a, const WorkArgs& w, int npairs, int max_n, bool need_corr, hipStream_t st,
                         int tail_test, int order_ncu, bool wide, int silent, int pending) {
    if (silent && pending) return hipErrorInvalidValue;
    if (order_ncu > 0 && (!tail_test || !w.owork || !w.plist || !w.plist_n || !w.nn_u || a.kp.numerics != kNumericsPCL))
        return hipErrorInvalidValue;
    if (w.lazy_x && (wide || need_corr || w.corr || w.res_update || w.sums_tail || !w.nn_u || !w.defer_xform ||
                     a.kp.numerics != kNumericsPCL))
        return hipErrorInvalidValue;
    if (a.kp.numerics == kNumericsPCL) {
        if (need_corr)
            hipLaunchKernelGGL(corr_kernel, dim3((max_n + 255) / 256, npairs), dim3(256), 0, st, a, w);
        if (wide && !tail_test && order_ncu <= 0 && w.held_update && max_n <= kHeldSmallN)
            hipLaunchKernelGGL((fold_update_held_kernel<3, true>), dim3(npairs), dim3(kWideWG), 0, st, a, w);
        else if (wide && !tail_test && order_ncu <= 0 && w.held_update && max_n <= kHeldMaxN)
            hipLaunchKernelGGL((fold_update_held_kernel<10, false>), dim3(npairs), dim3(kWideWG), 0, st, a, w);
        else if (wide && !tail_test && order_ncu <= 0)
            hipLaunchKernelGGL(fold_update_wide_kernel, dim3(npairs), dim3(kWideWG), 0, st, a, w);
        else if (w.res_update && !need_corr && !w.corr && max_n <= kResMaxN && w.nn_t && w.nn_u && w.defer_xform &&
                 a.kp.huber_delta == INFINITY && a.kp.max_d2 >= FLT_MAX &&
                 !w.sums_tail && (!tail_test || (w.sq && w.sm && w.need && w.miss_cnt)))
            hipLaunchKernelGGL(fold_update_res_kernel, dim3(npairs), dim3(kResWG), 0, st, a, w, tail_test, order_ncu);
        else if (w.lazy_x && pending)
            hipLaunchKernelGGL(fold_update_kernel<true>, dim3(npairs), dim3(kFoldWG), 0, st, a, w, tail_test, order_ncu, 0);
        else
            hipLaunchKernelGGL(fold_update_kernel<false>, dim3(npairs), dim3(kFoldWG), 0, st, a, w, tail_test, order_ncu,
                               (w.lazy_x && tail_test && silent) ? 1 : 0);
    } else {
        hipLaunchKernelGGL(update_f64_kernel, dim3(npairs), dim3(kUpdWG), 0, st, a, w);
    }
    return hipGetLastError();
}

hipError_t launch_solo(const PairArgs& a, const WorkArgs& w, int npairs, int max_n, int iters, hipStream_t st) {
    if (a.kp.numerics != kNumericsPCL || w.leaf != kLdsLeaf || w.t_stride > kLdsTargets || max_n > kCacheMaxN ||
        w.x_stride > kCacheMaxN || !w.tsort || !w.tbox || !w.sbox || !w.sperm || !w.nn_u || !w.nn_t || !w.qv ||
        !w.qm || !w.sq || !w.sm || !w.need || !w.miss_cnt || npairs <= 0 || iters <= 0)
        return hipErrorInvalidValue;
    hipLaunchKernelGGL(solo_kernel, dim3(npairs), dim3(kSoloWG), 0, st, a, w, iters);
    return hipGetLastError();
}

hipError_t launch_fitness_prep(const PairArgs& a, const WorkArgs& w, int npairs, hipStream_t st, int test) {
    if (test && (!w.nn_u || !w.need || !w.miss_cnt || !w.nn_t || !w.sq || !w.tsort || w.x_stride > kCacheMaxN))
        return hipErrorInvalidValue;
    hipLaunchKernelGGL(fitness_prep_kernel, dim3(npairs), dim3(kPrepWG), 0, st, a, w, test);
    return hipGetLastError();
}

hipError_t launch_finish(const PairArgs& a, const WorkArgs& w, int npairs, hipStream_t st) {
    hipLaunchKernelGGL(finish_kernel, dim3(npairs), dim3(kFinWG), 0, st, a, w);
    return hipGetLastError();
}

}
```

### icp-4dradar_amd/icp4r/__init__.py

```python
from __future__ import annotations

import ctypes as C
import os
import sys

import numpy as np

__all__ = [
    "ICP4RError", "Params", "Result", "Batch", "Context", "IterativeClosestPoint", "library_path", "load",
    "default_params", "NUMERICS_PCL", "NUMERICS_F64", "status_name", "EXPORTED_SYMBOLS", "Comm", "shard",
    "align_batch_multi",
]

HERE = os.path.dirname(os.path.abspath(__file__))
library_path = os.environ.get("ICP4R_LIBRARY") or os.path.join(HERE, "_lib", "libicp4r.so")

OK, E_INVALID, E_EMPTY, E_TOO_FEW_CORR, E_NONFINITE, E_HIP, E_RCCL, E_NOMEM, E_TOO_LARGE = 0, -1, -2, -3, -4, -5, -6, -7, -8
NUMERICS_PCL, NUMERICS_F64 = 0, 1
NO_DEVICE = -1
NN_AUTO, NN_BRUTE, NN_BRUTE_PACKED, NN_PRUNED = 0, 1, 2, 3
STAGE_NN, STAGE_NN_TEST, STAGE_UPDATE, STAGE_BATCH, STAGE_GICP_COV = 0, 1, 2, 3, 4
DBL_MAX = sys.float_info.max

_STATUS = {OK: "ICP4R_OK", E_INVALID: "ICP4R_E_INVALID", E_EMPTY: "ICP4R_E_EMPTY",
           E_TOO_FEW_CORR: "ICP4R_E_TOO_FEW_CORR", E_NONFINITE: "ICP4R_E_NONFINITE", E_HIP: "ICP4R_E_HIP",
           E_RCCL: "ICP4R_E_RCCL", E_NOMEM: "ICP4R_E_NOMEM", E_TOO_LARGE: "ICP4R_E_TOO_LARGE"}

EXPORTED_SYMBOLS = [
    "icp4r_version", "icp4r_abi_version", "icp4r_last_error", "icp4r_params_default", "icp4r_device_count",
    "icp4r_create", "icp4r_destroy", "icp4r_align", "icp4r_align_batch_device", "icp4r_align_batch_host",
    "icp4r_fitness", "icp4r_nearest", "icp4r_synchronize", "icp4r_kernel_time_ms", "icp4r_batch_time_ms",
    "icp4r_kernel_time_reset", "icp4r_set_kernel_timing", "icp4r_plan", "icp4r_nn_counters", "icp4r_nn_cache_hits", "icp4r_stage_time_ms",
    "icp4r_nn_stats", "icp4r_set_plan_option", "icp4r_get_plan_option", "icp4r_reset_plan_options",
]
PLAN_OPTIONS = (
    "nn_q", "leaf", "chunk_sb", "nn_lds", "nn_cache", "nn_tile", "tile_run", "solo", "xpad", "phase_ticks", "kd",
    "morton_mwg", "part", "src_order", "fuse_seed", "tile_own", "tile_defer", "groups", "search_cu_div",
    "fuse_test", "fuse_order", "sums_tail", "wide_update", "gather_padded", "gicp_cov_brute", "fold_keys", "gicp_spec", "gicp_grid", "gicp_knn_lanes", "res_update", "held_update", "fit_xform", "counters", "stage_sel",
    "lazy_x",
)
EGO_EXPORTED_SYMBOLS = [
    "icp4r_ego_params_default", "icp4r_radar_features", "icp4r_ego_velocity", "icp4r_ego_velocity_batch_device",
]
GICP_EXPORTED_SYMBOLS = [
    "icp4r_gicp_params_default", "icp4r_gicp_align", "icp4r_gicp_align_batch_device", "icp4r_gicp_covariances",
]
MULTI_EXPORTED_SYMBOLS = [
    "icp4r_shard", "icp4r_align_batch_multi", "icp4r_comm_unique_id", "icp4r_comm_create", "icp4r_comm_destroy",
    "icp4r_comm_rank", "icp4r_comm_check", "icp4r_gather_results", "icp4r_align_batch_sharded",
]
MAP_EXPORTED_SYMBOLS = [
    "icp4r_map_create", "icp4r_map_destroy", "icp4r_map_build", "icp4r_map_add_points", "icp4r_map_add_scan",
    "icp4r_map_size", "icp4r_map_sector_search", "icp4r_map_sector_search_device", "icp4r_map_points_device",
    "icp4r_map_time_ms", "icp4r_map_time_reset",
]


def status_name(code: int) -> str:
    return _STATUS.get(code, f"status {code}")


class ICP4RError(RuntimeError):
    def __init__(self, code: int, msg: str):
        super().__init__(f"{status_name(code)}: {msg}")
        self.code = code


class Params(C.Structure):
    _fields_ = [
        ("max_iterations", C.c_int32),
        ("min_correspondences", C.c_int32),
        ("max_correspondence_distance", C.c_double),
        ("transformation_epsilon", C.c_double),
        ("transformation_rotation_epsilon", C.c_double),
        ("euclidean_fitness_epsilon", C.c_double),
        ("mse_threshold_absolute", C.c_double),
        ("max_iterations_similar_transforms", C.c_int32),
        ("numerics", C.c_int32),
        ("nn_mode", C.c_int32),
        ("compute_fitness", C.c_int32),
        ("huber_delta", C.c_double),
        ("fitness_max_range", C.c_double),
        ("eigen_l1_bytes", C.c_int32),
        ("eigen_gebp_mr", C.c_int32),
        ("reserved", C.c_int32 * 6),
    ]


class Result(C.Structure):
    _fields_ = [
        ("T", C.c_float * 16),
        ("fitness", C.c_double),
        ("iterations", C.c_int32),
        ("converged", C.c_int32),
        ("status", C.c_int32),
        ("convergence_state", C.c_int32),
        ("n_correspondences", C.c_int32),
        ("reserved", C.c_int32),
    ]

    def matrix(self) -> np.ndarray:
        return np.array(self.T, np.float32).reshape(4, 4).T.copy()


class Batch(C.Structure):
    _fields_ = [
        ("src", C.c_void_p), ("tgt", C.c_void_p),
        ("src_off", C.c_void_p), ("src_n", C.c_void_p),
        ("tgt_off", C.c_void_p), ("tgt_n", C.c_void_p),
        ("guess", C.c_void_p), ("aligned", C.c_void_p),
        ("npairs", C.c_int32), ("max_src_n", C.c_int32), ("max_tgt_n", C.c_int32), ("reserved", C.c_int32),
    ]


class PlanInfo(C.Structure):
    _fields_ = [("pruned", C.c_int32), ("q", C.c_int32), ("splits", C.c_int32), ("leaf", C.c_int32),
                ("lds", C.c_int32), ("cache", C.c_int32), ("nn_blocks", C.c_int64), ("solo", C.c_int32),
                ("wide_update", C.c_int32), ("res_update", C.c_int32),
                ("held_update", C.c_int32)]


assert C.sizeof(Result) == 96
RESULT_DTYPE = np.dtype([("T", np.float32, 16), ("fitness", np.float64), ("iterations", np.int32),
                         ("converged", np.int32), ("status", np.int32), ("convergence_state", np.int32),
                         ("n_correspondences", np.int32), ("reserved", np.int32)])
assert RESULT_DTYPE.itemsize == 96

_lib = None


def load():
    global _lib
    if _lib is not None:
        return _lib
    if not os.path.exists(library_path):
        raise ICP4RError(E_HIP, f"{library_path} not built (run __graft_entry__.build() or make -C icp-4dradar_amd)")
    L = C.CDLL(library_path)
    vp, i32, i64 = C.c_void_p, C.c_int32, C.c_int64
    sig = {
        "icp4r_version": (C.c_char_p, []),
        "icp4r_abi_version": (C.c_int, []),
        "icp4r_last_error": (C.c_char_p, []),
        "icp4r_params_default": (None, [C.POINTER(Params)]),
        "icp4r_device_count": (C.c_int, [C.POINTER(C.c_int)]),
        "icp4r_create": (C.c_int, [C.POINTER(vp), C.c_int]),
        "icp4r_destroy": (C.c_int, [vp]),
        "icp4r_align": (C.c_int, [vp, vp, i32, i32, vp, i32, i32, vp, C.POINTER(Params), C.POINTER(Result), vp, i32]),
        "icp4r_align_batch_device": (C.c_int, [vp, C.POINTER(Batch), C.POINTER(Params), vp, vp]),
        "icp4r_align_batch_host": (C.c_int, [vp, vp, vp, vp, vp, vp, vp, i32, vp, C.POINTER(Params), vp]),
        "icp4r_fitness": (C.c_int, [vp, vp, i32, i32, vp, i32, i32, vp, C.c_double, C.POINTER(C.c_double)]),
        "icp4r_nearest": (C.c_int, [vp, vp, i32, i32, vp, i32, i32, vp, vp]),
        "icp4r_synchronize": (C.c_int, [vp, vp]),
        "icp4r_kernel_time_ms": (C.c_int, [vp, C.POINTER(C.c_double), C.POINTER(i32)]),
        "icp4r_batch_time_ms": (C.c_int, [vp, C.POINTER(C.c_double), C.POINTER(i32)]),
        "icp4r_kernel_time_reset": (C.c_int, [vp]),
        "icp4r_plan": (C.c_int, [vp, i32, i32, i32, i32, i32, C.POINTER(PlanInfo)]),
        "icp4r_set_plan_option": (C.c_int, [vp, C.c_char_p, i32]),
        "icp4r_get_plan_option": (C.c_int, [vp, C.c_char_p, C.POINTER(i32), C.POINTER(i32)]),
        "icp4r_reset_plan_options": (C.c_int, [vp]),
        "icp4r_nn_counters": (C.c_int, [vp, C.POINTER(C.c_uint64), C.POINTER(C.c_uint64)]),
        "icp4r_nn_cache_hits": (C.c_int, [vp, C.POINTER(C.c_uint64)]),
        "icp4r_stage_time_ms": (C.c_int, [vp, i32, C.POINTER(C.c_double), C.POINTER(i32)]),
        "icp4r_set_kernel_timing": (C.c_int, [vp, i32]),
        "icp4r_nn_stats": (C.c_int, [vp, C.POINTER(C.c_uint64 * 8)]),
        "icp4r_map_create": (C.c_int, [vp, C.POINTER(vp)]),
        "icp4r_map_destroy": (C.c_int, [vp]),
        "icp4r_map_build": (C.c_int, [vp, vp, i64, i32]),
        "icp4r_map_add_points": (C.c_int, [vp, vp, i64, i32, i32]),
        "icp4r_map_add_scan": (C.c_int, [vp, vp, i64, i32, vp, vp, vp]),
        "icp4r_map_size": (C.c_int, [vp, C.POINTER(i64)]),
        "icp4r_map_sector_search": (C.c_int, [vp, vp, C.c_float, C.c_float, vp, i64, C.POINTER(i64)]),
        "icp4r_map_sector_search_device": (C.c_int, [vp, vp, C.c_float, C.c_float, vp, vp, vp]),
        "icp4r_map_points_device": (C.c_int, [vp, C.POINTER(vp), C.POINTER(i64)]),
        "icp4r_map_time_ms": (C.c_int, [vp, C.POINTER(C.c_double), C.POINTER(i32)]),
        "icp4r_map_time_reset": (C.c_int, [vp]),
        "icp4r_shard": (C.c_int, [i32, i32, i32, C.POINTER(i32), C.POINTER(i32)]),
        "icp4r_align_batch_multi": (C.c_int, [C.POINTER(vp), i32, vp, vp, vp, vp, vp, vp, i32, vp, C.POINTER(Params),
                                              vp]),
        "icp4r_comm_unique_id": (C.c_int, [C.c_char_p]),
        "icp4r_comm_create": (C.c_int, [C.POINTER(vp), vp, i32, i32, C.c_char_p]),
        "icp4r_comm_destroy": (C.c_int, [vp]),
        "icp4r_comm_rank": (C.c_int, [vp, C.POINTER(i32), C.POINTER(i32)]),
        "icp4r_comm_check": (C.c_int, [vp]),
        "icp4r_gather_results": (C.c_int, [vp, vp, i32, vp, vp]),
        "icp4r_align_batch_sharded": (C.c_int, [vp, C.POINTER(Batch), i32, C.POINTER(Params), vp, vp, vp]),
    }
    for name, (res, args) in sig.items():
        f = getattr(L, name)
        f.restype = res
        f.argtypes = args
    _lib = L
    return L
# ... 24 lines not shown


class Context:

    def __init__(self, device: int = 0, plan: dict | None = None):
        self._lib = load()
        self._h = C.c_void_p()
        _check(self._lib.icp4r_create(C.byref(self._h), device), "icp4r_create")
        self.device = device
        if plan:
            self.set_plan(**plan)

    def close(self):
        if self._h:
            self._lib.icp4r_destroy(self._h)
            self._h = C.c_void_p()

    def __del__(self):
        try:
            self.close()
        except Exception:
            pass

    @property
    def handle(self):
        return self._h

    def align(self, src, tgt, params: Params | None = None, guess=None, want_aligned: bool = False):
        s, n, ss = _cloud(src)
        t, m, ts = _cloud(tgt)
        p = params if params is not None else default_params()
        r = Result()
        g = None
        if guess is not None:
            g = np.ascontiguousarray(np.asarray(guess, np.float32).T.reshape(16))
        out = np.zeros((n, 4), np.float32) if want_aligned else None
        rc = self._lib.icp4r_align(self._h, _ptr(s), n, ss, _ptr(t), m, ts, _ptr(g) if g is not None else None,
                                   C.byref(p), C.byref(r), _ptr(out) if out is not None else None, 16)
        if rc not in (OK, E_EMPTY, E_TOO_FEW_CORR, E_NONFINITE):
            _check(rc, "icp4r_align")
        return r, out

    def align_batch_host(self, src: np.ndarray, src_off, src_n, tgt: np.ndarray, tgt_off, tgt_n,
                         params: Params | None = None, guess=None) -> np.ndarray:
        src = np.ascontiguousarray(src, np.float32).reshape(-1, 4)
        tgt = np.ascontiguousarray(tgt, np.float32).reshape(-1, 4)
        so = np.ascontiguousarray(src_off, np.int64)
        sn = np.ascontiguousarray(src_n, np.int32)
        to = np.ascontiguousarray(tgt_off, np.int64)
        tn = np.ascontiguousarray(tgt_n, np.int32)
        npairs = len(sn)
        res = np.zeros(npairs, RESULT_DTYPE)
        g = None
        if guess is not None:
            g = np.ascontiguousarray(np.asarray(guess, np.float32).transpose(0, 2, 1).reshape(npairs, 16))
        p = params if params is not None else default_params()
        _check(self._lib.icp4r_align_batch_host(self._h, _ptr(src), _ptr(so), _ptr(sn), _ptr(tgt), _ptr(to), _ptr(tn),
                                                npairs, _ptr(g) if g is not None else None, C.byref(p),
                                                res.ctypes.data), "icp4r_align_batch_host")
        return res

    def align_batch_device(self, batch: Batch, params: Params, results_ptr: int, stream: int | None = None):
        _check(self._lib.icp4r_align_batch_device(self._h, C.byref(batch), C.byref(params), C.c_void_p(results_ptr),
                                                  C.c_void_p(stream) if stream else None), "icp4r_align_batch_device")

    def nearest(self, query, tgt):
        q, n, qs = _cloud(query)
        t, m, ts = _cloud(tgt)
        idx = np.empty(n, np.int32)
        d2 = np.empty(n, np.float32)
        _check(self._lib.icp4r_nearest(self._h, _ptr(q), n, qs, _ptr(t), m, ts, _ptr(idx), _ptr(d2)), "icp4r_nearest")
        return idx, d2

    def fitness(self, src, tgt, T, max_range: float = DBL_MAX) -> float:
        s, n, ss = _cloud(src)
        t, m, ts = _cloud(tgt)
        Tc = np.ascontiguousarray(np.asarray(T, np.float32).T.reshape(16))
        out = C.c_double()
        _check(self._lib.icp4r_fitness(self._h, _ptr(s), n, ss, _ptr(t), m, ts, _ptr(Tc), max_range, C.byref(out)),
               "icp4r_fitness")
        return out.value

    def synchronize(self, stream: int | None = None):
        _check(self._lib.icp4r_synchronize(self._h, C.c_void_p(stream) if stream else None), "icp4r_synchronize")

    def kernel_time_ms(self) -> tuple[float, int]:
        ms, k = C.c_double(), C.c_int32()
        _check(self._lib.icp4r_kernel_time_ms(self._h, C.byref(ms), C.byref(k)), "icp4r_kernel_time_ms")
        return ms.value, k.value

    def batch_time_ms(self) -> tuple[float, int]:
        ms, k = C.c_double(), C.c_int32()
        _check(self._lib.icp4r_batch_time_ms(self._h, C.byref(ms), C.byref(k)), "icp4r_batch_time_ms")
        return ms.value, k.value

    def set_kernel_timing(self, on: bool = True):
        _check(self._lib.icp4r_set_kernel_timing(self._h, 1 if on else 0), "icp4r_set_kernel_timing")

    def set_plan_option(self, name: str, value: int):
        _check(self._lib.icp4r_set_plan_option(self._h, name.encode(), int(value)), f"plan option {name}")

    def set_plan(self, **options):
        for k, v in options.items():
            self.set_plan_option(k, v)

    def get_plan_option(self, name: str) -> tuple[int, bool]:
        v, is_set = C.c_int32(), C.c_int32()
        _check(self._lib.icp4r_get_plan_option(self._h, name.encode(), C.byref(v), C.byref(is_set)), f"plan option {name}")
        return v.value, bool(is_set.value)

    def reset_plan_options(self):
        _check(self._lib.icp4r_reset_plan_options(self._h), "icp4r_reset_plan_options")

    def stage_time_ms(self, stage: int) -> tuple[float, int]:
        ms, k = C.c_double(), C.c_int32()
        _check(self._lib.icp4r_stage_time_ms(self._h, stage, C.byref(ms), C.byref(k)), "icp4r_stage_time_ms")
        return ms.value, k.value

    def reset_timers(self):
        _check(self._lib.icp4r_kernel_time_reset(self._h), "icp4r_kernel_time_reset")

    def nn_counters(self) -> tuple[int, int]:
        v, t = C.c_uint64(), C.c_uint64()
        _check(self._lib.icp4r_nn_counters(self._h, C.byref(v), C.byref(t)), "icp4r_nn_counters")
        return v.value, t.value

    def nn_stats(self) -> dict:
        v = (C.c_uint64 * 8)()
        _check(self._lib.icp4r_nn_stats(self._h, C.byref(v)), "icp4r_nn_stats")
        keys = ("evaluations", "box_tests", "cache_hits", "cache_tested", "records_written_by_test",
                "tested_in_update", "hits_in_update", "second_chance_hits")
        return {k: int(v[i]) for i, k in enumerate(keys)}

    def nn_cache_hits(self) -> int:
        v = C.c_uint64()
        _check(self._lib.icp4r_nn_cache_hits(self._h, C.byref(v)), "icp4r_nn_cache_hits")
        return v.value

    def nn_evaluations(self) -> int:
        return self.nn_counters()[0]


def plan(npairs: int, max_src_n: int, max_tgt_n: int, nn_mode: int = NN_AUTO, numerics: int = NUMERICS_PCL,
         ctx: "Context | None" = None) -> dict:
    info = PlanInfo()
    _check(load().icp4r_plan(ctx.handle if ctx is not None else None, npairs, max_src_n, max_tgt_n, nn_mode, numerics,
                             C.byref(info)), "icp4r_plan")
    out = {"pruned": bool(info.pruned), "lds": bool(info.lds), "cache": bool(info.cache), "q": info.q, "splits": info.splits,
           "leaf": info.leaf, "nn_blocks": info.nn_blocks, "solo": bool(info.solo),
           "wide_update": bool(info.wide_update), "res_update": bool(info.res_update),
           "held_update": bool(info.held_update)}
    octx = ctx if ctx is not None else Context(NO_DEVICE)
    try:
        on = {k: octx.get_plan_option(k)[0] != 0 for k in ("fuse_test", "sums_tail", "lazy_x")}
    finally:
        if ctx is None:
            octx.close()
    out["lazy_x"] = bool(out["lds"] and out["cache"] and numerics == NUMERICS_PCL and on["fuse_test"]
                         and not on["sums_tail"] and not out["res_update"] and on["lazy_x"])
    return out


_default_ctx: Context | None = None


def default_context() -> Context:
    global _default_ctx
    if _default_ctx is None:
        _default_ctx = Context(int(os.environ.get("ICP4R_DEVICE", "0")))
    return _default_ctx


class IterativeClosestPoint:

    def __init__(self, context: Context | None = None):
        self._ctx = context
        self._p = default_params()
        self._src = None
        self._tgt = None
        self._result: Result | None = None

    def setInputSource(self, cloud):
        self._src = np.ascontiguousarray(cloud, np.float32)
        self._result = None

    def setInputTarget(self, cloud):
        self._tgt = np.ascontiguousarray(cloud, np.float32)
        self._result = None

    def setMaximumIterations(self, nr_iterations: int):
        self._p.max_iterations = int(nr_iterations)

    def getMaximumIterations(self) -> int:
        return self._p.max_iterations

    def setMaxCorrespondenceDistance(self, distance_threshold: float):
        self._p.max_correspondence_distance = float(distance_threshold)

    def getMaxCorrespondenceDistance(self) -> float:
        return self._p.max_correspondence_distance

    def setTransformationEpsilon(self, epsilon: float):
        self._p.transformation_epsilon = float(epsilon)

    def setTransformationRotationEpsilon(self, epsilon: float):
        self._p.transformation_rotation_epsilon = float(epsilon)

    def setEuclideanFitnessEpsilon(self, epsilon: float):
        self._p.euclidean_fitness_epsilon = float(epsilon)

    def setHuberDelta(self, delta: float):
        self._p.huber_delta = float(delta)

    def setNumerics(self, numerics: int):
        self._p.numerics = int(numerics)

    def params(self) -> Params:
        return self._p

    def align(self, output=None, guess=None) -> np.ndarray:
        if self._tgt is None:
            raise ICP4RError(E_EMPTY, "No input target dataset was given!")
        if self._src is None:
            raise ICP4RError(E_INVALID, "No input source dataset was given!")
        ctx = self._ctx or default_context()
        r, aligned = ctx.align(self._src, self._tgt, self._p, guess=guess, want_aligned=True)
        self._result = r
        out = self._src.copy()
        out[:, :3] = aligned[:, :3]
        if output is not None:
            output[...] = out
            return output
        return out

    def hasConverged(self) -> bool:
        return bool(self._result is not None and self._result.converged)

    def getFinalTransformation(self) -> np.ndarray:
        if self._result is None:
            return np.eye(4, dtype=np.float32)
        return self._result.matrix()

    def getFitnessScore(self, max_range: float = DBL_MAX) -> float:
        if self._result is None:
            return DBL_MAX
        if max_range == self._p.fitness_max_range:
            return self._result.fitness
        return (self._ctx or default_context()).fitness(self._src, self._tgt, self.getFinalTransformation(), max_range)

    def result(self) -> Result | None:
        return self._result

    def nr_iterations(self) -> int:
        return 0 if self._result is None else self._result.iterations



COMM_ID_BYTES = 128


def shard(npairs: int, nranks: int, rank: int) -> range:
    f, c = C.c_int32(), C.c_int32()
    _check(load().icp4r_shard(npairs, nranks, rank, C.byref(f), C.byref(c)), "icp4r_shard")
    return range(f.value, f.value + c.value)


def align_batch_multi(ctxs, src, src_off, src_n, tgt, tgt_off, tgt_n, params: Params | None = None,
                      guess=None) -> np.ndarray:
    src = np.ascontiguousarray(src, np.float32).reshape(-1, 4)
    tgt = np.ascontiguousarray(tgt, np.float32).reshape(-1, 4)
    so = np.ascontiguousarray(src_off, np.int64)
    sn = np.ascontiguousarray(src_n, np.int32)
    to = np.ascontiguousarray(tgt_off, np.int64)
    tn = np.ascontiguousarray(tgt_n, np.int32)
    npairs = len(sn)
    res = np.zeros(npairs, RESULT_DTYPE)
    g = None
    if guess is not None:
        g = np.ascontiguousarray(np.asarray(guess, np.float32).transpose(0, 2, 1).reshape(npairs, 16))
    handles = (C.c_void_p * len(ctxs))(*[c.handle.value for c in ctxs])
    p = params if params is not None else default_params()
    _check(load().icp4r_align_batch_multi(handles, len(ctxs), _ptr(src), _ptr(so), _ptr(sn), _ptr(tgt), _ptr(to),
                                          _ptr(tn), npairs, _ptr(g) if g is not None else None, C.byref(p),
                                          res.ctypes.data), "icp4r_align_batch_multi")
    return res


class Comm:

    @staticmethod
    def unique_id() -> bytes:
        buf = C.create_string_buffer(COMM_ID_BYTES)
        _check(load().icp4r_comm_unique_id(buf), "icp4r_comm_unique_id")
        return buf.raw

    def __init__(self, ctx: Context, nranks: int, rank: int, uid: bytes):
        if len(uid) != COMM_ID_BYTES:
            raise ICP4RError(E_INVALID, f"unique id must be {COMM_ID_BYTES} bytes")
        self._lib = load()
        self._h = C.c_void_p()
        self.ctx, self.nranks, self.rank = ctx, nranks, rank
        _check(self._lib.icp4r_comm_create(C.byref(self._h), ctx.handle, nranks, rank, uid), "icp4r_comm_create")

    def close(self):
        if self._h:
            self._lib.icp4r_comm_destroy(self._h)
            self._h = C.c_void_p()

    def __del__(self):
        try:
            self.close()
        except Exception:
# ... 26 lines not shown
```

Baseline: 157,500 pairs/s.

## Fuse init into kd index build and optionally fold fitness into last update

```diff
diff --git a/icp-4dradar_amd/csrc/icp4r_batch.hpp b/icp-4dradar_amd/csrc/icp4r_batch.hpp
--- a/icp-4dradar_amd/csrc/icp4r_batch.hpp
+++ b/icp-4dradar_amd/csrc/icp4r_batch.hpp
@@ -31,7 +31,7 @@
     kOptPhaseTicks, kOptKd, kOptMortonMwg, kOptPart, kOptSrcOrder, kOptFuseSeed, kOptTileOwn, kOptTileDefer,
     kOptGroups, kOptSearchCuDiv, kOptFuseTest, kOptFuseOrder, kOptSumsTail, kOptWideUpdate, kOptGatherPadded,
     kOptGicpCovBrute, kOptFoldKeys, kOptGicpSpec, kOptGicpGrid, kOptGicpKnnLanes, kOptResUpdate, kOptHeldUpdate,
-    kOptFitXform, kOptCounters, kOptStageSel, kOptLazyX, kNumPlanOpts
+    kOptFitXform, kOptCounters, kOptStageSel, kOptLazyX, kOptFuseInit, kOptFuseFit, kNumPlanOpts
 };
 static_assert(kNumPlanOpts <= 64, "icp4r_ctx::plan_set is a 64-bit mask");
 extern const char* const kPlanOptNames[kNumPlanOpts];
diff --git a/icp-4dradar_amd/csrc/icp4r_capi.cpp b/icp-4dradar_amd/csrc/icp4r_capi.cpp
--- a/icp-4dradar_amd/csrc/icp4r_capi.cpp
+++ b/icp-4dradar_amd/csrc/icp4r_capi.cpp
@@ -97,7 +97,7 @@
     "phase_ticks", "kd", "morton_mwg", "part", "src_order", "fuse_seed", "tile_own", "tile_defer",
     "groups", "search_cu_div", "fuse_test", "fuse_order", "sums_tail", "wide_update", "gather_padded",
     "gicp_cov_brute", "fold_keys", "gicp_spec", "gicp_grid", "gicp_knn_lanes", "res_update",
-    "held_update", "fit_xform", "counters", "stage_sel", "lazy_x"};
+    "held_update", "fit_xform", "counters", "stage_sel", "lazy_x", "fuse_init", "fuse_fit"};
 
 int opt(const icp4r_ctx* ctx, PlanOpt k, int dflt) {
     return (ctx && (ctx->plan_set >> k & 1ull)) ? ctx->plan_val[k] : dflt;
@@ -494,12 +494,14 @@
     for (int g = 1; g < groups; ++g) HIP_TRY(hipStreamWaitEvent(gs[g], be->start, 0));
     const int cdiv = opt(ctx, kOptSearchCuDiv, groups);
     const int search_cu = cdiv > 1 ? (ctx->ncu + cdiv - 1) / cdiv : 0;
+    const bool fuse = pl.lds && pl.cache && pcl && opt(ctx, kOptFuseTest, 1) != 0;
+    const bool finit = fuse && index_tgt_only(w) && w.stage_first && !w.mo_hist && opt(ctx, kOptFuseInit, kDefaultFuseInit) != 0;
     for (int g = 0; g < groups; ++g) {
-        HIP_TRY(launch_init(ag[g], wg[g], gn[g], gs[g]));
+        wg[g].fuse_init = finit ? 1 : 0;
+        if (!finit) HIP_TRY(launch_init(ag[g], wg[g], gn[g], gs[g]));
         if (pl.pruned) HIP_TRY(launch_index(ag[g], wg[g], gn[g], gs[g]));
     }
     const int iters = max_iterations > 0 ? max_iterations : 1;
-    const bool fuse = pl.lds && pl.cache && pcl && opt(ctx, kOptFuseTest, 1) != 0;
     const bool ford = fuse && opt(ctx, kOptFuseOrder, 1) != 0;
     for (int g = 0; g < groups; ++g)
         wg[g].sums_tail = (fuse && a.kp.huber_delta == INFINITY && a.kp.max_d2 >= FLT_MAX && !a.kp.need_mse &&
@@ -514,6 +516,8 @@
     const bool lazy = fuse && !wg[0].sums_tail && !wg[0].res_update && opt(ctx, kOptLazyX, kDefaultLazyX) != 0;
     for (int g = 0; g < groups; ++g) wg[g].lazy_x = lazy ? 1 : 0;
     auto silent_tail = [&](int it) { return lazy && it >= 0 && it + 1 < iters && ((iters - 2 - it) & 1) != 0; };
+    const bool ffit = fuse && a.kp.compute_fitness && !wg[0].res_update && w.owork &&
+                      opt(ctx, kOptFuseFit, kDefaultFuseFit) != 0;
     const bool kev = ctx->kernel_timing;
     const bool wide = pcl && !fuse && npairs <= ctx->ncu && opt(ctx, kOptWideUpdate, 1) != 0;
     for (int g = 0; g < groups; ++g)
@@ -534,9 +538,10 @@
                 if ((rc = next_event(ctx->upd_events, ctx->upd_used, &ue))) return rc;
                 HIP_TRY(hipEventRecord(ue->start, gs[g]));
             }
+            const bool last_fit = ffit && it + 1 == iters;
             HIP_TRY(launch_update(ag[g], wg[g], gn[g], mn, pcl && !pl.pruned, gs[g], fuse && it + 1 < iters,
-                                  ford && it + 1 < iters ? ncu_g : 0, wide, silent_tail(it) ? 1 : 0,
-                                  silent_tail(it - 1) ? 1 : 0));
+                                  (ford && it + 1 < iters) || last_fit ? ncu_g : 0, wide, silent_tail(it) ? 1 : 0,
+                                  silent_tail(it - 1) ? 1 : 0, last_fit ? 1 : 0));
             if (kev) HIP_TRY(hipEventRecord(ue->stop, gs[g]));
         }
     }
@@ -547,9 +552,10 @@
                            !wg[g].nn_u && !wg[g].seed_next && opt(ctx, kOptFitXform, 1) != 0)
                               ? 1
                               : 0;
-        if ((a.kp.compute_fitness || a.aligned) && !wg[g].fit_xform)
+        if ((a.kp.compute_fitness || a.aligned) && !wg[g].fit_xform && !ffit)
             HIP_TRY(launch_fitness_prep(ag[g], wg[g], gn[g], gs[g], ftest));
-        if (a.kp.compute_fitness && (rc = nn_pass(ctx, pl, ag[g], wg[g], gn[g], mn, 1, 0, gs[g], search_cu, ftest, iters)))
+        if (a.kp.compute_fitness &&
+            (rc = nn_pass(ctx, pl, ag[g], wg[g], gn[g], mn, 1, 0, gs[g], search_cu, ftest, iters, ffit ? 1 : 0, 0)))
             return rc;
         HIP_TRY(launch_finish(ag[g], wg[g], gn[g], gs[g]));
     }
@@ -1027,7 +1033,8 @@
             0 , kDefaultLeaf, 0 , -1 , 1, 1, 0 ,
             -1 , 0, 0, 3, 1, kDefaultPartSize, -1 , 1, 1, 1, kDefaultGroups,
             0 , 1, 1, 0, 1, 0, 0, 1, kGicpSpec, kGicpGrid,
-            0 , kDefaultResUpdate, kDefaultHeldUpdate, 1, 0, kDefaultStageSel, kDefaultLazyX};
+            0 , kDefaultResUpdate, kDefaultHeldUpdate, 1, 0, kDefaultStageSel, kDefaultLazyX,
+            kDefaultFuseInit, kDefaultFuseFit};
         *value = dflt[k];
     }
     if (is_set) *is_set = set ? 1 : 0;
diff --git a/icp-4dradar_amd/csrc/icp4r_internal.hpp b/icp-4dradar_amd/csrc/icp4r_internal.hpp
--- a/icp-4dradar_amd/csrc/icp4r_internal.hpp
+++ b/icp-4dradar_amd/csrc/icp4r_internal.hpp
@@ -125,6 +125,7 @@
     int32_t res_update;
     int32_t held_update;
     int32_t fit_xform;
+    int32_t fuse_init;
     int32_t lazy_x;
     float4* nn_t;
     float4* sq;
@@ -152,6 +153,7 @@
 hipError_t launch_nn(int q, bool packed, const PairArgs& a, const WorkArgs& w, int npairs, int max_n,
                      int fitness_pass, hipStream_t st);
 hipError_t launch_index(const PairArgs& a, const WorkArgs& w, int npairs, hipStream_t st);
+bool index_tgt_only(const WorkArgs& w);
 hipError_t launch_index_cloud(const PairArgs& a, const WorkArgs& w, int npairs, hipStream_t st);
 hipError_t launch_nn_pruned(int q, int chunk_sb, int chunks, const PairArgs& a, const WorkArgs& w, int npairs,
                             int max_n, int fitness_pass, int first, hipStream_t st);
@@ -169,6 +171,8 @@
 constexpr int kResMaxN = 8192;
 constexpr int kDefaultResUpdate = 0;
 constexpr int kDefaultLazyX = 1;
+constexpr int kDefaultFuseInit = 1;
+constexpr int kDefaultFuseFit = 0;
 constexpr int kHeldMaxN = 10 * 896;
 constexpr int kHeldSmallN = 3 * 704;
 constexpr int kDefaultHeldUpdate = 1;
@@ -178,7 +182,8 @@
                          int order_ncu = 0,
                          bool wide = false,
                          int silent = 0,
-                         int pending = 0);
+                         int pending = 0,
+                         int fit = 0);
 hipError_t launch_solo(const PairArgs& a, const WorkArgs& w, int npairs, int max_n, int iters, hipStream_t st);
 hipError_t launch_fitness_prep(const PairArgs& a, const WorkArgs& w, int npairs, hipStream_t st, int test = 0);
 hipError_t launch_finish(const PairArgs& a, const WorkArgs& w, int npairs, hipStream_t st);
diff --git a/icp-4dradar_amd/csrc/icp4r_kernels.hip b/icp-4dradar_amd/csrc/icp4r_kernels.hip
--- a/icp-4dradar_amd/csrc/icp4r_kernels.hip
+++ b/icp-4dradar_amd/csrc/icp4r_kernels.hip
@@ -342,9 +342,11 @@
     return (((S + unit - 1) / unit) >> 1) * unit;
 }
 
-template <int KPER, typename Get>
-__device__ void kd_order(KdShared& sh, Get pts, int n, int leaf, uint64_t* tk, uint32_t* kdn = nullptr,
-                         uint16_t* gk = nullptr) {
+constexpr float kBigCoord = 1e17f;
+constexpr int kInBad = 1, kInBig = 2;
+template <int KPER, bool CHECK = false, typename Get>
+__device__ int kd_order(KdShared& sh, Get pts, int n, int leaf, uint64_t* tk, uint32_t* kdn = nullptr,
+                        uint16_t* gk = nullptr) {
     static_assert(KPER % 8 == 0 && KPER <= 16 && KPER * kIdxWG >= kKdMaxN / 2, "list positions per thread");
     const int tid = threadIdx.x, lane = tid & 63, wave = tid >> 6;
     if (tk) tk[0] = __builtin_amdgcn_s_memrealtime();
@@ -374,7 +376,21 @@
             sh.red[wave][3 + k] = mx[k];
         }
     for (int b = tid; b < 3 * kKdBins; b += kIdxWG) (&sh.u.hist[0][0])[b] = 0;
-    __syncthreads();
+    int chk = 0;
+    if (CHECK) {
+        int bad = 0, big = 0;
+#pragma unroll
+        for (int k = 0; k < kKdPer; ++k) {
+            bad |= !(isfinite(px[k]) && isfinite(py[k]) && isfinite(pz[k]));
+            big |= fmaxf(fabsf(px[k]), fmaxf(fabsf(py[k]), fabsf(pz[k]))) > kBigCoord;
+        }
+        bad = __syncthreads_or(bad);
+        big = __syncthreads_or(big);
+        chk = (bad ? kInBad : 0) | (big ? kInBig : 0);
+        if (bad) return chk;
+    } else {
+        __syncthreads();
+    }
     if (tid < 3) {
         float l = INFINITY, h = -INFINITY;
         for (int v = 0; v < kIdxWaves; ++v) {
@@ -593,6 +609,7 @@
         }
         __syncthreads();
     }
+    return chk;
 }
 
 __device__ void index_boxes(const WorkArgs& w, int p, int n) {
@@ -652,13 +669,14 @@
            a.src_n[p] <= kKdMaxN;
 }
 
-__device__ __forceinline__ void index_cloud(IndexShared& shu, const PairArgs& a, const WorkArgs& w, int p, bool is_tgt) {
-    if (w.state[p].phase == kPhaseInvalid) return;
+template <bool CHECK = false>
+__device__ __forceinline__ int index_cloud(IndexShared& shu, const PairArgs& a, const WorkArgs& w, int p, bool is_tgt) {
+    if (!CHECK && w.state[p].phase == kPhaseInvalid) return 0;
     const int tid = threadIdx.x, lane = tid & 63, wave = tid >> 6;
     const int n = is_tgt ? a.tgt_n[p] : a.src_n[p];
-    if (n <= 0) return;
+    if (n <= 0) return 0;
     const float4* pts = is_tgt ? a.tgt + a.tgt_off[p] : a.src + a.src_off[p];
-    if (!is_tgt && src_by_tgt_tree(a, w, p)) return;
+    if (!is_tgt && src_by_tgt_tree(a, w, p)) return 0;
     if ((w.kd_index & (is_tgt ? 1 : 2)) && n <= kKdMaxN && (!is_tgt || w.t_stride <= kKdMaxN)) {
 #if ICP4R_WG_TICKS
         uint64_t* it = (w.ticks && tid == 0) ? w.ticks + 32 + 12 * (int64_t)gridDim.x + 8 * (int64_t)p + (is_tgt ? 0 : 4) : nullptr;
@@ -675,10 +693,12 @@
         uint16_t* gk = (is_tgt && w.qv && (int64_t)w.x_stride * (int64_t)sizeof(float4) >= 3 * kKdMaxN * 2)
                            ? reinterpret_cast<uint16_t*>(w.qv + (int64_t)p * w.x_stride)
                            : nullptr;
+        int chk;
         if (n <= kKdMaxN / 2)
-            kd_order<8>(shu.kd, [&](int i) { return pts[i]; }, n, is_tgt ? w.leaf : 16, tk, kdn, gk);
+            chk = kd_order<8, CHECK>(shu.kd, [&](int i) { return pts[i]; }, n, is_tgt ? w.leaf : 16, tk, kdn, gk);
         else
-            kd_order<16>(shu.kd, [&](int i) { return pts[i]; }, n, is_tgt ? w.leaf : 16, tk, kdn, gk);
+            chk = kd_order<16, CHECK>(shu.kd, [&](int i) { return pts[i]; }, n, is_tgt ? w.leaf : 16, tk, kdn, gk);
+        if (CHECK && (chk & kInBad)) return chk;
         const uint16_t* ord = shu.kd.L[0];
         if (is_tgt) {
             float4* ts = w.tsort + (int64_t)p * w.t_stride;
@@ -782,9 +802,9 @@
         __syncthreads();
         if (it) it[1] = __builtin_amdgcn_s_memrealtime();
 #endif
-        return;
-    }
-    if (is_tgt && w.mo_hist) return;
+        return chk;
+    }
+    if (is_tgt && w.mo_hist) return 0;
     uint32_t* bins = shu.mo.bins;
     float(*red)[6] = shu.mo.red;
     uint32_t* wsum = shu.mo.wsum;
@@ -872,6 +892,7 @@
             sp[pos] = i;
         });
     }
+    return 0;
 }
 
 
@@ -1016,15 +1037,29 @@
     float qz[6];
     uint32_t sl[kKdMaxN];
 };
-__device__ void src_order_pair(const PairArgs& a, const WorkArgs& w, int p, SoShared& so) {
+template <bool INIT = false>
+__device__ int src_order_pair(const PairArgs& a, const WorkArgs& w, int p, SoShared& so) {
     uint32_t* nodes = so.nodes;
     uint32_t* bins = so.bins;
     uint32_t* wsum = so.wsum;
     float* qz = so.qz;
     uint32_t* sl = so.sl;
-    if (w.state[p].phase == kPhaseInvalid || !src_by_tgt_tree(a, w, p)) return;
+    if ((!INIT && w.state[p].phase == kPhaseInvalid) || !src_by_tgt_tree(a, w, p)) return 0;
     const int n = a.src_n[p], m = a.tgt_n[p];
-    if (n <= 0) return;
+    if (n <= 0) return 0;
+    const float* Gp = (INIT && a.guess) ? a.guess + (int64_t)p * 16 : nullptr;
+    bool id = true;
+    if (INIT && Gp)
+        for (int k = 0; k < 16; ++k) id = id && (uload(Gp + k) == ((k % 5 == 0) ? 1.0f : 0.0f));
+    auto guess_pt = [&](float4& v) {
+        if (id) return;
+        float Tg[16];
+#pragma unroll
+        for (int k = 0; k < 16; ++k) Tg[k] = uload(Gp + k);
+        const float4 s = v;
+        xform_pt(Tg, s.x, s.y, s.z, v.x, v.y, v.z);
+    };
+    int bad = 0, big = 0;
     const int tid = threadIdx.x, lane = tid & 63, wave = tid >> 6;
 #if ICP4R_WG_TICKS
     uint64_t* it = (w.ticks && tid == 0) ? w.ticks + 32 + 12 * (int64_t)gridDim.x + 8 * (int64_t)p + 4 : nullptr;
@@ -1048,7 +1083,7 @@
     for (int b = tid; b < kKdMaxN / 16; b += kSoWG) bins[b] = 0u;
     __syncthreads();
     const float lo[3] = {qz[0], qz[1], qz[2]}, sc[3] = {qz[3], qz[4], qz[5]};
-    const float4* X = w.X + (int64_t)p * w.x_stride;
+    const float4* X = INIT ? a.src + a.src_off[p] : w.X + (int64_t)p * w.x_stride;
     constexpr int kSoPer = kKdMaxN / kSoWG, kSoGrp = 8;
     static_assert(kSoPer % kSoGrp == 0 && kSoPer % 2 == 0, "point groups");
     uint32_t lv[kSoPer / 2];
@@ -1057,6 +1092,17 @@
         float4 v[kSoGrp];
 #pragma unroll
         for (int e = 0; e < kSoGrp; ++e) v[e] = X[min(tid + (g + e) * kSoWG, n - 1)];
+        if (INIT) {
+#pragma unroll
+            for (int e = 0; e < kSoGrp; ++e) {
+                const bool fin = isfinite(v[e].x) && isfinite(v[e].y) && isfinite(v[e].z);
+                bad |= !fin;
+                if (!fin) v[e] = make_float4(0.0f, 0.0f, 0.0f, 0.0f);
+                guess_pt(v[e]);
+                big |= fmaxf(fabsf(v[e].x), fmaxf(fabsf(v[e].y), fabsf(v[e].z))) > kBigCoord;
+            }
+            asm volatile("" : "+v"(bad), "+v"(big));
+        }
         int key3[kSoGrp][3], node[kSoGrp], sp[kSoGrp];
 #pragma unroll
         for (int e = 0; e < kSoGrp; ++e) {
@@ -1090,7 +1136,15 @@
                 lv[(g + e) >> 1] |= leaf << 16;
         }
     }
-    __syncthreads();
+    int chk = 0;
+    if (INIT) {
+        bad = __syncthreads_or(bad);
+        big = __syncthreads_or(big);
+        chk = (bad ? kInBad : 0) | (big ? kInBig : 0);
+        if (bad) return chk;
+    } else {
+        __syncthreads();
+    }
 #if ICP4R_WG_TICKS
     if (it) it[3] = __builtin_amdgcn_s_memrealtime();
 #endif
@@ -1120,7 +1174,8 @@
         float px[kSoPer], py[kSoPer], pz[kSoPer];
 #pragma unroll
         for (int g = 0; g < kSoPer; ++g) {
-            const float4 v = X[min(tid + g * kSoWG, n - 1)];
+            float4 v = X[min(tid + g * kSoWG, n - 1)];
+            if (INIT) guess_pt(v);
             px[g] = v.x;
             py[g] = v.y;
             pz[g] = v.z;
@@ -1176,7 +1231,7 @@
         __syncthreads();
         if (it) it[1] = __builtin_amdgcn_s_memrealtime();
 #endif
-        return;
+        return chk;
     }
 #pragma unroll
     for (int g = 0; g < kSoPer; g += kSoGrp) {
@@ -1200,6 +1255,7 @@
     __syncthreads();
     if (it) it[1] = __builtin_amdgcn_s_memrealtime();
 #endif
+    return chk;
 }
 
 __global__ __launch_bounds__(kSoWG) void src_order_kernel(PairArgs a, WorkArgs w) {
@@ -1217,6 +1273,49 @@
     if (gridDim.y == 1) {
         __syncthreads();
         src_order_pair(a, w, p, *reinterpret_cast<SoShared*>(&shu));
+    }
+}
+
+__global__ __launch_bounds__(kIdxWG, 4) void index_init_kernel(PairArgs a, WorkArgs w) {
+    __shared__ IndexShared shu;
+    const int p = xcd_remap(blockIdx.x, gridDim.x);
+    const int tid = threadIdx.x;
+    const int n = a.src_n[p], m = a.tgt_n[p];
+    if (w.need) {
+        uint32_t* gneed = w.need + (int64_t)p * w.need_stride;
+        for (int k = tid; k < w.need_stride; k += kIdxWG) gneed[k] = 0u;
+    }
+    if (tid == 0 && w.miss_cnt) w.miss_cnt[p] = 0;
+    if (tid < 4 && p == 0 && w.plist_n) w.plist_n[tid] = 0;
+    const bool too_big = n > w.x_stride || m > w.t_stride;
+    int chk = 0;
+    if (!too_big && m > 0) {
+        chk = index_cloud<true>(shu, a, w, p, true);
+        if (!(chk & kInBad)) {
+            __syncthreads();
+            chk |= src_order_pair<true>(a, w, p, *reinterpret_cast<SoShared*>(&shu));
+        }
+    }
+    if (tid == 0) {
+        PairState& st = w.state[p];
+        mat4_identity(st.T_inc);
+        st.prev_mse = DBL_MAX;
+        st.similar = 0;
+        st.conv_state = 0;
+        st.iterations = 0;
+        st.ncorr = 0;
+        st.sums_ok = (chk & kInBig) ? -1 : 0;
+        st.pending = 0;
+        if (m <= 0 || (chk & kInBad) || too_big) {
+            mat4_identity(st.final_T);
+            st.phase = kPhaseInvalid;
+            st.status = too_big ? kStatusInvalid : m <= 0 ? kStatusEmpty : kStatusNonFinite;
+        } else {
+            for (int k = 0; k < 16; ++k)
+                st.final_T[k] = a.guess ? a.guess[(int64_t)p * 16 + k] : ((k % 5 == 0) ? 1.0f : 0.0f);
+            st.phase = kPhaseActive;
+            st.status = 0;
+        }
     }
 }
 
@@ -3820,11 +3919,39 @@
     }
 }
 
-template <bool PEND>
+__device__ __forceinline__ int fit_tail(const PairArgs& a, const WorkArgs& w, int p, int n, FoldShared& sh, bool cleared) {
+    const int tid = threadIdx.x;
+    uint32_t* need = reinterpret_cast<uint32_t*>(&sh.buf[0][0][0]);
+    int32_t* pre = reinterpret_cast<int32_t*>(need + kNeedWords);
+    float4* lv = reinterpret_cast<float4*>(pre + kNeedWords);
+    uint2* lm = reinterpret_cast<uint2*>(lv + kFoldRecs);
+    float* Tf = reinterpret_cast<float*>(sh.s.sigma);
+    static_assert(sizeof(sh.s.sigma) >= 16 * sizeof(float), "final_T staged in SolveShared::sigma");
+    if (!cleared) {
+        for (int k = tid; k < ((n + 31) >> 5); k += kFoldWG) need[k] = 0u;
+        if (tid == 0) sh.mcount = 0;
+    }
+    if (tid < 16) Tf[tid] = w.state[p].final_T[tid];
+    __syncthreads();
+    float T[16];
+#pragma unroll
+    for (int q = 0; q < 16; ++q) T[q] = Tf[q];
+    return pair_cache_test<kFoldWG, kTailPer, true>(a, w, p, n, T, need, pre, lv, lm, kFoldRecs, &sh.mcount, sh.cnt,
+                                                   true);
+}
+
+template <bool PEND, bool FIT = false>
 __device__ __forceinline__ int fold_update_pair(const PairArgs& a, const WorkArgs& w, int tail_test, int silent, int p,
                                                 FoldShared& sh) {
+    static_assert(!(PEND && FIT), "the last update never follows a silent tail");
     PairState& st = w.state[p];
-    if (st.phase != kPhaseActive) return 0;
+    if (FIT) {
+        const int ph = st.phase;
+        if (ph == kPhaseInvalid) return 0;
+        if (ph != kPhaseActive) return fit_tail(a, w, p, a.src_n[p], sh, false);
+    } else if (st.phase != kPhaseActive) {
+        return 0;
+    }
     const int tid = threadIdx.x;
     const int n = a.src_n[p];
     clear_need(w, p, n, tid, kFoldWG);
@@ -3871,10 +3998,19 @@
         for (int k = tid; k < ((n + 31) >> 5); k += kFoldWG) need[k] = 0u;
         if (tid == 0) sh.mcount = 0;
     }
+    if (FIT) {
+        for (int k = tid; k < ((n + 31) >> 5); k += kFoldWG) need[k] = 0u;
+        if (tid == 0) sh.mcount = 0;
+    }
     if (tid == 0) solve_pair<kNumericsPCL>(sh.s, st, kp);
     __syncthreads();
     if (ticks) w.ticks[3] = __builtin_amdgcn_s_memrealtime();
     WG_TICK(3);
+    if (FIT) {
+        nwork = fit_tail(a, w, p, n, sh, true);
+        if (ticks) w.ticks[4] = __builtin_amdgcn_s_memrealtime();
+        return nwork;
+    }
     if (Tp && !(tail && sh.s.flag == 0)) {
         flush_pending<kFoldWG>(w, p, n, Tp);
         if (tid == 0) st.pending = 0;
@@ -3934,6 +4070,23 @@
     __syncthreads();
     if (!last) return;
     order_items<kFoldWG, true>(a, w, (int)gridDim.x, 0, 0, order_ncu, osh);
+}
+
+__global__ __launch_bounds__(kFoldWG, 4) void fold_update_fit_kernel(PairArgs a, WorkArgs w, int order_ncu) {
+    __shared__ FoldShared sh;
+    __shared__ OrderShared osh;
+    __shared__ int32_t last;
+    const int p = xcd_remap(blockIdx.x, gridDim.x);
+    const int nwork = fold_update_pair<false, true>(a, w, 0, 0, p, sh);
+    if (threadIdx.x == 0) {
+        __hip_atomic_store(w.owork + p, nwork, __ATOMIC_RELAXED, __HIP_MEMORY_SCOPE_AGENT);
+        asm volatile("s_waitcnt vmcnt(0)" ::: "memory");
+        const int old = __hip_atomic_fetch_add(w.plist_n + 3, 1, __ATOMIC_RELAXED, __HIP_MEMORY_SCOPE_AGENT);
+        last = (old + 1) % (int)gridDim.x == 0 ? 1 : 0;
+    }
+    __syncthreads();
+    if (!last) return;
+    order_items<kFoldWG, true>(a, w, (int)gridDim.x, 1, 0, order_ncu, osh);
 }
 
 constexpr int kResWG = 256;
@@ -5265,8 +5418,18 @@
     return hipGetLastError();
 }
 
+bool index_tgt_only(const WorkArgs& w) {
+    return w.src_by_tgt && w.kdn && (w.kd_index & 1) && w.t_stride <= kKdMaxN && w.x_stride <= kKdMaxN;
+}
+
 hipError_t launch_index(const PairArgs& a, const WorkArgs& w, int npairs, hipStream_t st) {
-    const bool tgt_only = w.src_by_tgt && w.kdn && (w.kd_index & 1) && w.t_stride <= kKdMaxN && w.x_stride <= kKdMaxN;
+    const bool tgt_only = index_tgt_only(w);
+    if (w.fuse_init) {
+        if (!tgt_only || !w.stage_first || w.mo_hist || !w.qv || !w.qm || !w.nn_u || w.leaf <= 0)
+            return hipErrorInvalidValue;
+        hipLaunchKernelGGL(index_init_kernel, dim3(npairs), dim3(kIdxWG), 0, st, a, w);
+        return hipGetLastError();
+    }
     const unsigned nch = (unsigned)((w.t_stride + kKdMaxN - 1) / kKdMaxN);
     if (w.mo_hist) {
         if (!(w.tbb && (w.kd_index & 1) && w.t_stride > kKdMaxN && (w.leaf == 16 || w.leaf == 32) &&
@@ -5310,7 +5473,7 @@
         hipLaunchKernelGGL(nn_cache_test_kernel, dim3(chunks, npairs), dim3(kTestWG), 0, st, a, w, fitness_pass);
         if (ev.test_stop && (e = hipEventRecord(ev.test_stop, st)) != hipSuccess) return e;
     }
-    if (ordered && (first || !cache || fitness_pass || !test_fused)) return hipErrorInvalidValue;
+    if (ordered && (first || !cache || !test_fused)) return hipErrorInvalidValue;
     if (pending && (first || !cache || fitness_pass || !test_fused || !w.lazy_x)) return hipErrorInvalidValue;
     if (!ordered)
         hipLaunchKernelGGL(nn_order_kernel, dim3(1), dim3(kOrderWG), 0, st, a, w, npairs, fitness_pass,
@@ -5379,9 +5542,13 @@
 }
 
 hipError_t launch_update(const PairArgs& a, const WorkArgs& w, int npairs, int max_n, bool need_corr, hipStream_t st,
-                         int tail_test, int order_ncu, bool wide, int silent, int pending) {
+                         int tail_test, int order_ncu, bool wide, int silent, int pending, int fit) {
     if (silent && pending) return hipErrorInvalidValue;
-    if (order_ncu > 0 && (!tail_test || !w.owork || !w.plist || !w.plist_n || !w.nn_u || a.kp.numerics != kNumericsPCL))
+    if (order_ncu > 0 && (!(tail_test || fit) || !w.owork || !w.plist || !w.plist_n || !w.nn_u || a.kp.numerics != kNumericsPCL))
+        return hipErrorInvalidValue;
+    if (fit && (tail_test || silent || pending || wide || need_corr || w.corr || w.res_update || order_ncu <= 0 ||
+                !a.kp.compute_fitness || !w.nn_u || !w.defer_xform || !w.need || !w.miss_cnt || !w.nn_t || !w.sq ||
+                !w.sm || !w.qv || !w.qm || !w.tsort || w.x_stride > kCacheMaxN || a.kp.numerics != kNumericsPCL))
         return hipErrorInvalidValue;
     if (w.lazy_x && (wide || need_corr || w.corr || w.res_update || w.sums_tail || !w.nn_u || !w.defer_xform ||
                      a.kp.numerics != kNumericsPCL))
@@ -5399,6 +5566,8 @@
                  a.kp.huber_delta == INFINITY && a.kp.max_d2 >= FLT_MAX &&
                  !w.sums_tail && (!tail_test || (w.sq && w.sm && w.need && w.miss_cnt)))
             hipLaunchKernelGGL(fold_update_res_kernel, dim3(npairs), dim3(kResWG), 0, st, a, w, tail_test, order_ncu);
+        else if (fit)
+            hipLaunchKernelGGL(fold_update_fit_kernel, dim3(npairs), dim3(kFoldWG), 0, st, a, w, order_ncu);
         else if (w.lazy_x && pending)
             hipLaunchKernelGGL(fold_update_kernel<true>, dim3(npairs), dim3(kFoldWG), 0, st, a, w, tail_test, order_ncu, 0);
         else
diff --git a/icp-4dradar_amd/icp4r/__init__.py b/icp-4dradar_amd/icp4r/__init__.py
--- a/icp-4dradar_amd/icp4r/__init__.py
+++ b/icp-4dradar_amd/icp4r/__init__.py
@@ -37,7 +37,7 @@
     "nn_q", "leaf", "chunk_sb", "nn_lds", "nn_cache", "nn_tile", "tile_run", "solo", "xpad", "phase_ticks", "kd",
     "morton_mwg", "part", "src_order", "fuse_seed", "tile_own", "tile_defer", "groups", "search_cu_div",
     "fuse_test", "fuse_order", "sums_tail", "wide_update", "gather_padded", "gicp_cov_brute", "fold_keys", "gicp_spec", "gicp_grid", "gicp_knn_lanes", "res_update", "held_update", "fit_xform", "counters", "stage_sel",
-    "lazy_x",
+    "lazy_x", "fuse_init", "fuse_fit",
 )
 EGO_EXPORTED_SYMBOLS = [
     "icp4r_ego_params_default", "icp4r_radar_features", "icp4r_ego_velocity", "icp4r_ego_velocity_batch_device",
@@ -368,12 +368,18 @@
            "held_update": bool(info.held_update)}
     octx = ctx if ctx is not None else Context(NO_DEVICE)
     try:
-        on = {k: octx.get_plan_option(k)[0] != 0 for k in ("fuse_test", "sums_tail", "lazy_x")}
+        on = {k: octx.get_plan_option(k)[0] != 0
+              for k in ("fuse_test", "sums_tail", "lazy_x", "fuse_init", "fuse_fit", "src_order")}
+        kd, xpad = octx.get_plan_option("kd")[0], octx.get_plan_option("xpad")[0]
     finally:
         if ctx is None:
             octx.close()
-    out["lazy_x"] = bool(out["lds"] and out["cache"] and numerics == NUMERICS_PCL and on["fuse_test"]
-                         and not on["sums_tail"] and not out["res_update"] and on["lazy_x"])
+    fuse = bool(out["lds"] and out["cache"] and numerics == NUMERICS_PCL and on["fuse_test"])
+    out["lazy_x"] = bool(fuse and not on["sums_tail"] and not out["res_update"] and on["lazy_x"])
+    x_stride = ((max(max_src_n, 1) + 3) & ~3) + xpad
+    out["fuse_init"] = bool(fuse and on["src_order"] and (kd & 1) and x_stride <= 8192 and max_tgt_n <= 8192
+                            and on["fuse_init"])
+    out["fuse_fit"] = bool(fuse and not out["res_update"] and on["fuse_fit"])
     return out
 
 
```

New measurement: 158,500 pairs/s (median of 6 runs). About the same (+0.6%).
